# ucsdmanorlab/bootstrapper

Measured on AMD Instinct MI355X. Metric: Mvoxels/s predict+segment, 1024^3 vol in 128^3 blocks, higher is better.
Workload: dtype bf16x3

## Files before the change

bootstrapper_amd/_lib.py:

```python
import ctypes as C
import os

import torch

_HERE = os.path.dirname(os.path.abspath(__file__))
LIB_PATH = os.environ.get("BSMI_LIB") or os.path.join(_HERE, "libbsmi.so")

MAX_LEVELS, MAX_CONVS, MAX_HEADS, NAME_LEN = 8, 4, 4, 32
PREC_F32, PREC_BF16, PREC_BF16X3 = 0, 1, 2
RAW_U8, RAW_F32, RAW_U8_UNIT = 0, 1, 2
ERR_INVALID, ERR_HIP, ERR_STATE, ERR_MISSING, ERR_OVERFLOW = -1, -2, -3, -4, -5


class UNetConfig(C.Structure):
    _fields_ = [
        ("in_channels", C.c_int32),
        ("num_fmaps", C.c_int32),
        ("fmap_inc_factor", C.c_int32),
        ("num_levels", C.c_int32),
        ("downsample_factors", (C.c_int32 * 3) * MAX_LEVELS),
        ("n_convs_down", C.c_int32 * MAX_LEVELS),
        ("kernel_size_down", ((C.c_int32 * 3) * MAX_CONVS) * MAX_LEVELS),
        ("n_convs_up", C.c_int32 * MAX_LEVELS),
        ("kernel_size_up", ((C.c_int32 * 3) * MAX_CONVS) * MAX_LEVELS),
        ("num_heads", C.c_int32),
        ("head_name", (C.c_char * NAME_LEN) * MAX_HEADS),
        ("head_dims", C.c_int32 * MAX_HEADS),
        ("num_fmaps_out", C.c_int32),
    ]


class StepInfo(C.Structure):
    _fields_ = [("type", C.c_int32), ("materialised", C.c_int32), ("shape", C.c_int32 * 4), ("conv_index", C.c_int32),
                ("form", C.c_int32), ("flags", C.c_int32), ("bn", C.c_int32), ("ksteps", C.c_int32), ("head", C.c_int32),
                ("factor", C.c_int32 * 3), ("offset", C.c_int32 * 3), ("prefix", C.c_char * 64)]


STEP_TYPES = ("input", "conv", "pool", "up", "head")
CONV_FORMS = ("gather", "raster-halo", "box-halo", "halo-resident", "first-pass", "winograd F(2x2)", "winograd F(4x4)")
STEP_FLAGS = {1: "fused-up", 2: "res-low", 4: "split-k"}


class Codec(C.Structure):
    _fields_ = [("id", C.c_int32), ("level", C.c_int32), ("cname", C.c_int32), ("shuffle", C.c_int32),
                ("typesize", C.c_int32), ("blocksize", C.c_int32)]


class ChunkCopy(C.Structure):
    _fields_ = [("path", C.c_char_p), ("base", C.c_void_p), ("start", C.c_int64 * 4), ("extent", C.c_int64 * 4),
                ("stride", C.c_int64 * 4), ("read_modify_write", C.c_int32), ("reserved", C.c_int32)]


CODEC_RAW, CODEC_ZLIB, CODEC_GZIP, CODEC_ZSTD, CODEC_LZ4, CODEC_BLOSC = range(6)
BLOSC_LZ4, BLOSC_ZLIB, BLOSC_ZSTD = 1, 3, 4
CHUNK_MISSING = 1
MORPH_DILATE, MORPH_ERODE = 0, 1
RESCALE_DOWN, RESCALE_UP = 0, 1


class BsmiError(RuntimeError):
    def __init__(self, code, msg):
        super().__init__(f"libbsmi error {code}: {msg}")
        self.code = code
        self.msg = msg


def _load():
    if not os.path.exists(LIB_PATH):
        raise ImportError(
            f"{LIB_PATH} not found: build it with `python -c 'import __graft_entry__ as g; g.build()'` "
            "(or `make -C bootstrapper_amd/csrc`).  There is no CPU fallback.")
    lib = C.CDLL(LIB_PATH)
    p, i32, i64p, vp = C.c_void_p, C.c_int, C.POINTER(C.c_int64), C.c_void_p
    sigs = {
        "bsmi_last_error": (C.c_char_p, []),
        "bsmi_version": (i32, []),
        "bsmi_unet_create": (i32, [C.POINTER(UNetConfig), i32, C.POINTER(p)]),
        "bsmi_unet_destroy": (i32, [p]),
        "bsmi_unet_load_weight": (i32, [p, C.c_char_p, vp, i64p, i32]),
        "bsmi_unet_finalize": (i32, [p, i32]),
        "bsmi_unet_output_shape": (i32, [p, i64p, i64p]),
        "bsmi_unet_flops": (i32, [p, i64p, C.POINTER(C.c_double)]),
        "bsmi_unet_forward": (i32, [p, i32, vp, i32, i64p, C.POINTER(vp), C.POINTER(vp), vp]),
        "bsmi_unet_debug_activation": (i32, [p, i32, i32, i64p, vp, C.c_uint64]),
        "bsmi_unet_debug_step_info": (i32, [p, i32, C.POINTER(StepInfo), C.POINTER(i32)]),
        "bsmi_unet_profile_enable": (i32, [p, i32]),
        "bsmi_unet_profile_read": (i32, [p, i32, C.POINTER(i32), C.POINTER(C.c_int32), C.POINTER(C.c_double),
                                         C.POINTER(C.c_double)]),
        "bsmi_unet_profile_totals": (i32, [p, C.POINTER(C.c_double), C.POINTER(C.c_double), i64p, i32]),
        "bsmi_extract_block_reflect_u8": (i32, [vp, i64p, i64p, i64p, vp, vp]),
        "bsmi_seg_create": (i32, [i32, i64p, C.POINTER(p)]),
        "bsmi_seg_destroy": (i32, [p]),
        "bsmi_ws_fragments_u8": (i32, [p, vp, i64p, i32, i32, vp, vp, vp]),
        "bsmi_ws_fragments_seeds_u8": (i32, [p, vp, i64p, i32, i32, vp, vp, vp, vp]),
        "bsmi_rag_agglomerate_u8": (i32, [p, vp, vp, i64p, C.c_float, C.c_int, vp]),
        "bsmi_rag_edge_stats": (i32, [p, vp, vp, C.c_uint64, vp]),
        "bsmi_agglomerate_mean_u8": (i32, [p, vp, vp, i64p, C.POINTER(C.c_float), i32, vp, vp]),
        "bsmi_agglomerate_hist_u8": (i32, [p, vp, vp, i64p, C.POINTER(C.c_float), i32, i32, i32, vp, vp]),
        "bsmi_agglomerate_hist_graph": (i32, [C.c_uint32, C.c_uint32, vp, vp, vp, i32, i32, C.POINTER(C.c_float), i32, vp]),
        "bsmi_frag_postprocess_u8": (i32, [p, vp, vp, i64p, C.c_double, C.c_int64, i64p, i64p, C.c_uint64, vp, vp, vp]),
        "bsmi_label_stats": (i32, [p, vp, i64p, C.c_uint64, C.c_uint64, vp, vp, vp]),
        "bsmi_rag_merge_scores_u8": (i32, [p, vp, vp, i64p, C.c_float, C.c_int, vp, vp, C.c_uint64, vp, vp, vp, vp]),
        "bsmi_lut_relabel": (i32, [C.c_int, vp, C.c_uint64, vp, vp, C.c_uint64, vp, vp]),
        "bsmi_lut_relabel_multi": (i32, [i32, vp, C.c_uint64, vp, vp, C.c_uint64, i32, vp, vp]),
        "bsmi_connected_components": (i32, [vp, C.c_uint64, vp, vp, C.c_uint64, C.c_float, vp]),
        "bsmi_connected_components_multi": (i32, [vp, C.c_uint64, vp, vp, C.c_uint64, vp, C.c_int, vp]),
        "bsmi_cc_affs_u8": (i32, [p, vp, i64p, C.c_int, C.c_int64, vp, vp, vp, vp]),
        "bsmi_mws_agglom_f64": (i32, [C.c_int, vp, C.c_int, vp, vp, C.c_uint32, i64p, vp, vp]),
        "bsmi_mws_cluster": (i32, [C.c_uint64, vp, vp, C.c_uint64, vp]),
        "bsmi_frag_pair_affinity_u8": (i32, [C.c_int, vp, C.c_int, vp, vp, i64p, C.c_uint64, vp, vp, vp, vp, vp]),
        "bsmi_label_table_u64": (i32, [p, vp, i64p, C.c_int64, vp, vp, vp, vp, C.c_uint64, vp, vp]),
        "bsmi_seg_status": (i32, [p, vp]),
        "bsmi_seg_set_host_flood": (i32, [p, i32]),
        "bsmi_rag_graph_u8": (i32, [p, vp, vp, i64p, vp, vp, vp, C.c_uint64, vp, vp]),
        "bsmi_rag_merge_scores_host": (i32, [i32, vp, vp, vp, vp, C.c_float, i32, vp, i32]),
        "bsmi_rag_merge_scores_host_rule": (i32, [i32, vp, vp, vp, vp, C.c_float, i32, i32, vp, i32]),
        "bsmi_unet_train_set_arithmetic": (i32, [p, i32]),
        "bsmi_unet_train_set_deterministic": (i32, [p, i32]),
        "bsmi_unet_train_begin": (i32, [p, i64p]),
        "bsmi_unet_train_forward_backward": (i32, [p, vp, C.POINTER(C.c_void_p), C.POINTER(C.c_void_p), C.POINTER(C.c_float), vp]),
        "bsmi_unet_train_num_params": (i32, [p, C.POINTER(C.c_uint64)]),
        "bsmi_unet_train_buffers": (i32, [p, C.POINTER(C.c_void_p), C.POINTER(C.c_void_p)]),
        "bsmi_unet_train_param_info": (i32, [p, C.c_char_p, C.POINTER(C.c_uint64), C.POINTER(C.c_uint64)]),
        "bsmi_unet_train_adam_step": (i32, [p, C.c_float, C.c_float, C.c_float, C.c_float, C.c_float, vp]),
        "bsmi_unet_train_read_param": (i32, [p, C.c_char_p, C.c_int, vp]),
        "bsmi_unet_train_last_loss": (i32, [p, C.POINTER(C.c_float), vp]),
        "bsmi_unet_train_prediction": (i32, [p, i32, C.POINTER(C.c_void_p), C.POINTER(C.c_uint64)]),
        "bsmi_unet_train_grad_groups": (i32, [p, i32, C.POINTER(i32), C.POINTER(C.c_uint64), C.POINTER(C.c_uint64)]),
        "bsmi_unet_train_wait_grad_group": (i32, [p, i32, vp]),
        "bsmi_unet_train_write_param": (i32, [p, C.c_char_p, C.c_int, vp]),
        "bsmi_unet_train_step_count": (i32, [p, C.c_int, C.POINTER(C.c_int)]),
        "bsmi_unet_train_end": (i32, [p]),
        "bsmi_train_affinity_targets": (i32, [C.c_int, vp, vp, i64p, C.POINTER(C.c_int32), C.c_int, C.c_int, C.c_int, C.c_float,
                                              C.c_float, vp, vp, vp]),
        "bsmi_train_lsd_targets": (i32, [C.c_int, vp, vp, i64p, i64p, i64p, C.POINTER(C.c_float), C.POINTER(C.c_float), C.c_int, vp, vp, vp]),
        "bsmi_train_lsd2d_targets": (i32, [C.c_int, vp, vp, C.c_int, i64p, i64p, i64p, C.POINTER(C.c_float), C.POINTER(C.c_float), C.c_int,
                                           vp, vp, vp]),
        "bsmi_train_affinity_targets_roi": (i32, [C.c_int, vp, vp, C.c_int, i64p, i64p, i64p, C.POINTER(C.c_int32), C.c_int, C.c_int,
                                                  C.c_int, C.c_float, C.c_float, vp, vp, vp]),
        "bsmi_train_mask_sat": (i32, [C.c_int, vp, C.c_int, C.c_int, C.c_int, vp, vp]),
        "bsmi_unet_set_persistent_grid": (i32, [p, C.c_int]),
        "bsmi_unet_profile_executed": (i32, [p, C.POINTER(C.c_double), C.c_int]),
        "bsmi_debug_lds_canary": (i32, [i32, i32, i32, vp, vp]),
        "bsmi_debug_check_guards": (i32, []),
        "bsmi_stream_create_cu_mask": (i32, [C.c_int, vp, C.c_int, C.POINTER(C.c_void_p)]),
        "bsmi_stream_destroy": (i32, [C.c_int, vp]),
        "bsmi_eval_create": (i32, [i32, C.c_uint64, C.POINTER(p)]),
        "bsmi_eval_destroy": (i32, [p]),
        "bsmi_eval_aff_errors_u8": (i32, [p, vp, i64p, i64p, vp, i32, i64p, vp, C.POINTER(C.c_int32), i64p, C.c_float, C.c_float,
                                          C.c_int64, vp, vp, vp, vp]),
        "bsmi_eval_lsd_errors_u8": (i32, [p, vp, i64p, i64p, vp, vp, i64p, i64p, i64p, i64p, C.POINTER(C.c_float), C.POINTER(C.c_float),
                                          i32, C.c_float, C.c_float, C.c_int64, C.c_uint64, vp, vp, vp, vp, vp, vp, vp, vp]),
        "bsmi_eval_pairs_u64": (i32, [p, vp, vp, vp, i64p, i32, vp]),
        "bsmi_eval_pairs_read": (i32, [p, vp, vp, vp, C.c_uint64, vp, vp]),
        "bsmi_eval_status": (i32, [p, vp]),
        "bsmi_label_morph_u64": (i32, [i32, vp, i64p, i32, i32, i32, vp, vp, vp]),
        "bsmi_label_fill_holes_scratch_bytes": (C.c_size_t, [i64p, C.c_uint64]),
        "bsmi_label_fill_holes_u64": (i32, [i32, vp, i64p, i32, vp, vp, C.c_size_t, C.c_uint64, C.POINTER(C.c_uint64), vp]),
        "bsmi_mask_closing_work_bytes": (C.c_size_t, [i64p, i32]),
        "bsmi_mask_closing_disk_u8": (i32, [i32, vp, i64p, i32, vp, vp, C.c_size_t, vp]),
        "bsmi_downscale_mean": (i32, [i32, vp, i32, i64p, C.POINTER(C.c_int32), C.POINTER(C.c_int32), vp, i64p, vp]),
        "bsmi_rescale_sample": (i32, [i32, vp, i32, i64p, C.POINTER(C.c_int32), C.POINTER(C.c_int32), i32, vp, i64p, vp]),
        "bsmi_nonzero_bbox": (i32, [i32, vp, i32, i64p, i64p, vp, vp]),
        "bsmi_synth_create": (i32, [i32, i64p, C.POINTER(p)]),
        "bsmi_synth_destroy": (i32, [p]),
        "bsmi_synth_dilate_points": (i32, [p, i64p, vp, i32, vp, vp, vp, vp, vp]),
        "bsmi_synth_label_i32": (i32, [p, vp, i64p, vp, C.POINTER(C.c_uint64), vp]),
        "bsmi_synth_expand_i32": (i32, [p, vp, i64p, i32, C.c_int32, vp, vp]),
        "bsmi_synth_tubes_i32": (i32, [p, vp, i64p, vp, C.POINTER(C.c_uint64), vp]),
        "bsmi_synth_gaussian_f32": (i32, [p, vp, i64p, vp, i32, vp, vp]),
        "bsmi_synth_argmax_filter_f32": (i32, [p, vp, i64p, i32, vp, vp]),
        "bsmi_synth_basins_f32": (i32, [p, vp, vp, vp, i64p, vp, C.POINTER(C.c_uint64), vp]),
        "bsmi_synth_finish_i32": (i32, [p, vp, i64p, i32, i32, i32, vp, vp]),
        "bsmi_synth_grow_boundary_i64": (i32, [i32, vp, i64p, C.c_uint64, i32, vp, vp]),
        "bsmi_synth_merge_i64": (i32, [i32, vp, i64p, C.POINTER(C.c_int32), i32, C.c_int64, C.c_int64, vp]),
        "bsmi_synth_stamp_i64": (i32, [i32, vp, i64p, i32, i32, i32, vp, i32, i32, C.c_int64, vp]),
        "bsmi_synth_present_i64": (i32, [p, vp, C.c_uint64, vp, C.c_uint32, C.POINTER(C.c_uint32), vp]),
        "bsmi_synth_split_i64": (i32, [p, vp, i64p, C.c_int64, i32, C.POINTER(C.c_int32), i32, C.c_int64, C.POINTER(C.c_uint64), vp]),
        "bsmi_codec_bound": (C.c_size_t, [C.POINTER(Codec), C.c_size_t]),
        "bsmi_codec_decode": (i32, [C.POINTER(Codec), vp, C.c_size_t, vp, C.c_size_t, C.POINTER(C.c_size_t)]),
        "bsmi_codec_encode": (i32, [C.POINTER(Codec), vp, C.c_size_t, vp, C.c_size_t, C.POINTER(C.c_size_t)]),
        "bsmi_chunks_read": (i32, [C.POINTER(Codec), i32, C.POINTER(C.c_char_p), C.POINTER(vp), C.POINTER(C.c_size_t),
                                   C.POINTER(C.c_size_t), C.POINTER(i32), i32]),
        "bsmi_chunks_write": (i32, [C.POINTER(Codec), i32, C.POINTER(C.c_char_p), C.POINTER(vp), C.POINTER(C.c_size_t),
                                    C.POINTER(i32), i32]),
        "bsmi_blosc_dev_frame_bound": (C.c_size_t, [C.c_size_t]),
        "bsmi_blosc_dev_scratch_bytes": (C.c_size_t, [i32, C.c_size_t]),
        "bsmi_blosc_encode_dev_u64": (i32, [i32, vp, C.c_int64, C.c_int64, i32, i64p, i64p, i64p, vp, C.c_size_t, vp, C.c_size_t, vp, vp]),
        "bsmi_rag_write_sqlite": (i32, [C.c_char_p, C.c_uint64, vp, vp, vp, C.c_uint64, vp, vp]),
        "bsmi_chunks_read_into": (i32, [C.POINTER(Codec), i32, C.POINTER(ChunkCopy), i64p, i32, vp, C.POINTER(i32), i32]),
        "bsmi_chunks_write_from": (i32, [C.POINTER(Codec), i32, C.POINTER(ChunkCopy), i64p, i32, vp, C.POINTER(i32), i32]),
    }
    for name, (res, args) in sigs.items():
        fn = getattr(lib, name)
        fn.restype = res
        fn.argtypes = args
# ... 14 lines not shown
```

bootstrapper_amd/csrc/seg.hip:

```cpp
#include <atomic>
#include <chrono>
#include <thread>

#include "seg_internal.h"

#include "dev_guard.h"

namespace bsmi {

__global__ __launch_bounds__(256) void fill_list_kernel(FillList L) {
  const size_t stride = (size_t)gridDim.x * blockDim.x, t0 = (size_t)blockIdx.x * blockDim.x + threadIdx.x;
  for (int j = 0; j < L.n; ++j) {
    uint32_t* p = L.p[j];
    const size_t w = L.words[j];
    const uint32_t v = L.value[j];
    size_t head = (size_t)((0 - (uintptr_t)p) >> 2) & 3;
    head = head < w ? head : w;
    if (t0 < head) p[t0] = v;
    uint4* q = (uint4*)(p + head);
    const size_t nv = (w - head) >> 2;
    for (size_t i = t0; i < nv; i += stride) q[i] = make_uint4(v, v, v, v);
    const size_t done = head + 4 * nv;
    if (t0 < w - done) p[done + t0] = v;
  }
}
void Fills::launch(hipStream_t s) const {
  const unsigned grid = (unsigned)std::min<size_t>((most + 255) / 256 + 1, 2048);
  hipLaunchKernelGGL(fill_list_kernel, dim3(grid), dim3(256), 0, s, L);
}

template <typename T>
static int dalloc(bsmi_seg* h, T** p, size_t count) {
  void* q = nullptr;
  BSMI_HIP(hipMalloc(&q, count * sizeof(T) + 16));
  h->allocs.push_back(q);
  *p = (T*)q;
  return BSMI_OK;
}
static uint32_t next_pow2(uint64_t v) {
  uint32_t p = 1;
  while (p < v) p <<= 1;
  return p;
}

int check_seg_shape(bsmi_seg* h, const int64_t shape[3]) {
  if (!h || !shape) BSMI_FAIL(BSMI_ERR_INVALID, "null argument");
  for (int d = 0; d < 3; ++d)
    if (shape[d] < 1) BSMI_FAIL(BSMI_ERR_INVALID, "bad shape");
  if ((size_t)shape[0] * shape[1] * shape[2] > h->max_vox || shape[0] > h->max_shape[0] ||
      shape[1] * shape[2] > h->max_shape[1] * h->max_shape[2])
    BSMI_FAIL(BSMI_ERR_INVALID, "shape (%lld,%lld,%lld) exceeds the handle's max_shape (%lld,%lld,%lld)",
              (long long)shape[0], (long long)shape[1], (long long)shape[2], (long long)h->max_shape[0],
              (long long)h->max_shape[1], (long long)h->max_shape[2]);
  return BSMI_OK;
}

}

using namespace bsmi;

extern "C" {

int bsmi_seg_create(int device, const int64_t max_shape[3], bsmi_seg** out) {
  if (!max_shape || !out) BSMI_FAIL(BSMI_ERR_INVALID, "null argument");
  for (int d = 0; d < 3; ++d)
    if (max_shape[d] < 1 || max_shape[d] > 4096) BSMI_FAIL(BSMI_ERR_INVALID, "bad max_shape");
  BSMI_HIP(hipSetDevice(device));
  bsmi_seg* h = new bsmi_seg;
  h->device = device;
  for (int d = 0; d < 3; ++d) h->max_shape[d] = max_shape[d];
  const size_t nv = (size_t)max_shape[0] * max_shape[1] * max_shape[2];
  const size_t ns = (size_t)max_shape[1] * max_shape[2];
  h->max_vox = nv;
  int rc = 0;
#define A(ptr, cnt) if (!rc) rc = dalloc(h, &(ptr), (cnt))
  A(h->ws.mask, nv); A(h->ws.g, nv); A(h->ws.d2, nv); A(h->ws.mf, nv); A(h->ws.par, nv); A(h->ws.lab, nv);
  A(h->ws.nseeds, (size_t)max_shape[0]); A(h->ws.offs, (size_t)max_shape[0]);
  h->ws.seedlab = nullptr;
  h->flood_spill_stride = ns;
  A(h->flood_spill, nv);
  if (ns >= ((size_t)1 << 20)) A(h->flood_spill_idx, nv);
  AggWs& g = h->agg;
  static std::atomic<int> next_xcd{0};
  g.xcd_hint = next_xcd.fetch_add(1) & 7;
  g.id_cap = (uint32_t)std::min<size_t>(nv + 2, (size_t)1 << 27);
  g.node_cap = (uint32_t)std::min<size_t>(nv / 8 + 1024, (size_t)1 << 24);
  g.hcap = next_pow2(std::max<size_t>(nv / 2, 1024));
  g.edge_cap = g.hcap / 2;
  A(g.rank_of_id, (size_t)g.id_cap); A(g.ids, (size_t)g.node_cap); A(g.counters, 8);
  A(g.hkeys, (size_t)g.hcap); A(g.hvals, (size_t)g.hcap); A(g.hsum, (size_t)g.hcap); A(g.hcnt, (size_t)g.hcap);
  A(g.eu, (size_t)g.edge_cap); A(g.ev, (size_t)g.edge_cap); A(g.ekey0, (size_t)g.edge_cap);
  A(g.esum, (size_t)g.edge_cap); A(g.ecnt, (size_t)g.edge_cap); A(g.enextu, (size_t)g.edge_cap);
  A(g.enextv, (size_t)g.edge_cap); A(g.eflags, (size_t)g.edge_cap);
  A(g.head, (size_t)g.node_cap); A(g.parent, (size_t)g.node_cap);
  A(g.roots, (size_t)g.node_cap * kMaxThresholds); A(g.heap_spill, (size_t)g.edge_cap); A(g.maxid, 1);
  A(g.sticky, 1);
  A(g.escore, (size_t)g.edge_cap); A(g.etime, (size_t)g.edge_cap); A(g.ntime, (size_t)g.node_cap);
  A(h->thr_dev, kMaxThresholds); A(h->status_dev, 4);
  FragWs& f = h->frag;
  f.id_cap = (uint32_t)std::min<size_t>(nv + 2, (size_t)1 << 27);
  A(f.lsum, (size_t)f.id_cap); A(f.lcnt, (size_t)f.id_cap); A(f.rank, nv); A(f.blk, nv / 1024 + 2); A(f.flags, 4);
  f.par = h->ws.par;
  A(h->crop_tmp, nv);
  g.icap = next_pow2((size_t)g.node_cap * 2);
  A(g.idkeys, (size_t)g.icap); A(g.idvals, (size_t)g.icap); A(g.idu, (size_t)g.node_cap);
  A(g.skeys, (size_t)g.hcap); A(g.sslot, (size_t)g.hcap); A(g.iota, (size_t)g.hcap); A(g.qnext, (size_t)g.edge_cap);
  A(g.tnext, (size_t)g.node_cap * 2); A(g.tscore, (size_t)g.node_cap * 2); A(g.cur, (size_t)g.node_cap);
  A(g.ha, (size_t)g.node_cap); A(g.hb, (size_t)g.node_cap); A(h->rag_counts, 4);
  A(g.tcount, (size_t)g.icap); A(g.tzmin, (size_t)g.icap); A(g.tzmax, (size_t)g.icap);
  if (!rc) {
    size_t b = 0;
// ... 136 lines not shown
```

bootstrapper_amd/csrc/seg_graph.hip:

```cpp
#include <new>

#include "seg_internal.h"

#include "dev_guard.h"

namespace bsmi {
void host_agglomerate_hist(uint32_t nn, uint32_t ne, const uint32_t* eu, const uint32_t* ev, uint32_t* hist, int quantile,
                           int init_with_max, const float* thresholds, int nthr, uint32_t* roots_out);

constexpr int AGG_LDS_HEAP = 12288;

__global__ void agg_maxid_kernel(const uint64_t* __restrict__ frags, size_t n, AggWs w) {
  unsigned long long m = 0;
  for (size_t i = (size_t)blockIdx.x * blockDim.x + threadIdx.x; i < n; i += (size_t)gridDim.x * blockDim.x)
    m = frags[i] > m ? frags[i] : m;
  for (int o = 32; o > 0; o >>= 1) {
    const unsigned long long t = __shfl_down(m, o);
    m = t > m ? t : m;
  }
  if ((threadIdx.x & 63) == 0 && m) atomicMax((unsigned long long*)w.maxid, m);
}

__global__ void agg_mark_kernel(const uint64_t* __restrict__ frags, size_t n, AggWs w) {
  const uint64_t maxid = *w.maxid;
  if (maxid >= w.id_cap) {
    if (blockIdx.x == 0 && threadIdx.x == 0) atomicOr(&w.counters[3], 1u);
    return;
  }
  for (size_t i = (size_t)blockIdx.x * blockDim.x + threadIdx.x; i < n; i += (size_t)gridDim.x * blockDim.x) {
    const uint64_t f = frags[i];
    if (f) w.rank_of_id[f] = 1u;
  }
}

__global__ __launch_bounds__(1024) void agg_rank_kernel(AggWs w) {
  __shared__ uint32_t sh[1024];
  if (w.counters[3]) return;
  const uint64_t maxid = *w.maxid;
  const uint32_t n = (uint32_t)maxid + 1;
  const uint32_t chunk = (n + 1023) / 1024;
  const uint32_t c0 = threadIdx.x * chunk, c1 = min(n, c0 + chunk);
  uint32_t cnt = 0;
  for (uint32_t i = c0; i < c1 && i < n; ++i) cnt += w.rank_of_id[i] == 1u;
  sh[threadIdx.x] = cnt;
  __syncthreads();
  if (threadIdx.x == 0) {
    uint32_t acc = 0;
    for (int t = 0; t < 1024; ++t) { const uint32_t c = sh[t]; sh[t] = acc; acc += c; }
    w.counters[0] = acc;
    if (acc > w.node_cap) atomicOr(&w.counters[3], 2u);
  }
  __syncthreads();
  if (w.counters[3]) return;
  uint32_t r = sh[threadIdx.x];
  for (uint32_t i = c0; i < c1 && i < n; ++i) {
    if (w.rank_of_id[i] == 1u) {
      w.rank_of_id[i] = r;
      w.ids[r] = i;
      w.head[r] = NOEDGE;
      w.parent[r] = r;
      ++r;
    } else {
      w.rank_of_id[i] = 0xffffffffu;
    }
  }
}

template <bool HASH>
__device__ __forceinline__ uint32_t agg_rank(const AggWs& w, uint64_t f) {
  if constexpr (!HASH) return w.rank_of_id[f];
  uint32_t s = (uint32_t)mix64(f) & (w.icap - 1);
  for (uint32_t probe = 0; probe < w.icap; ++probe) {
    const uint64_t k = w.idkeys[s];
    if (k == f) return w.idvals[s];
    if (k == HEMPTY) break;
    s = (s + 1) & (w.icap - 1);
  }
  return 0;
}

template <bool HASH>
__global__ void agg_edges_kernel(const uint8_t* __restrict__ affs, const uint64_t* __restrict__ frags, int D, int H,
                                 int W, AggWs w) {
  if (w.counters[3]) return;
  const size_t n = (size_t)D * H * W;
  const size_t hw = (size_t)H * W;
  for (size_t p = (size_t)blockIdx.x * blockDim.x + threadIdx.x; p < n; p += (size_t)gridDim.x * blockDim.x) {
    const uint64_t f1 = frags[p];
    if (!f1) continue;
    const int x = (int)(p % W);
    const int y = (int)((p / W) % H);
    const int z = (int)(p / hw);
    const uint32_t r1 = agg_rank<HASH>(w, f1);
    const bool ok[3] = {z > 0, y > 0, x > 0};
    const size_t st[3] = {hw, (size_t)W, 1};
#pragma unroll
    for (int d = 0; d < 3; ++d) {
      if (!ok[d]) continue;
      const uint64_t f2 = frags[p - st[d]];
      if (!f2 || f2 == f1) continue;
      const uint32_t r2 = agg_rank<HASH>(w, f2);
      const uint32_t u = r1 < r2 ? r1 : r2, v = r1 < r2 ? r2 : r1;
      const uint64_t key = ((uint64_t)u << 32) | v;
      uint32_t slot = (uint32_t)mix64(key) & (w.hcap - 1);
      bool placed = false;
      for (uint32_t probe = 0; probe < w.hcap; ++probe) {
        const unsigned long long old = atomicCAS((unsigned long long*)&w.hkeys[slot], HEMPTY, key);
        if (old == HEMPTY || old == key) { placed = true; break; }
        slot = (slot + 1) & (w.hcap - 1);
      }
      if (!placed) { atomicOr(&w.counters[3], 4u); return; }
      atomicAdd(&w.hsum[slot], (unsigned long long)affs[(size_t)d * n + p]);
      atomicAdd(&w.hcnt[slot], 1u);
    }
  }
}

__global__ void agg_compact_kernel(AggWs w) {
  if (w.counters[3]) return;
  for (uint32_t s = blockIdx.x * blockDim.x + threadIdx.x; s < w.hcap; s += gridDim.x * blockDim.x) {
    const uint64_t key = w.hkeys[s];
    if (key == HEMPTY) continue;
    const uint32_t e = atomicAdd(&w.counters[1], 1u);
    if (e >= w.edge_cap) { atomicOr(&w.counters[3], 8u); continue; }
    const uint32_t u = (uint32_t)(key >> 32), v = (uint32_t)key;
    w.eu[e] = u; w.ev[e] = v; w.ekey0[e] = key;
    w.esum[e] = w.hsum[s]; w.ecnt[e] = w.hcnt[s];
    w.eflags[e] = 0;
    w.hvals[s] = e;
    w.enextu[e] = atomicExch(&w.head[u], e);
    w.enextv[e] = atomicExch(&w.head[v], e);
  }
}

__global__ void agg_hist_kernel(const uint8_t* __restrict__ affs, const uint64_t* __restrict__ frags, int D, int H, int W, AggWs w,
                                uint32_t* __restrict__ hist) {
  if (w.counters[3]) return;
  const size_t n = (size_t)D * H * W;
  const size_t hw = (size_t)H * W;
  for (size_t p = (size_t)blockIdx.x * blockDim.x + threadIdx.x; p < n; p += (size_t)gridDim.x * blockDim.x) {
    const uint64_t f1 = frags[p];
    if (!f1) continue;
    const int x = (int)(p % W);
    const int y = (int)((p / W) % H);
    const int z = (int)(p / hw);
    const uint32_t r1 = w.rank_of_id[f1];
    const bool ok[3] = {z > 0, y > 0, x > 0};
    const size_t st[3] = {hw, (size_t)W, 1};
#pragma unroll
    for (int d = 0; d < 3; ++d) {
      if (!ok[d]) continue;
      const uint64_t f2 = frags[p - st[d]];
      if (!f2 || f2 == f1) continue;
      const uint32_t r2 = w.rank_of_id[f2];
      const uint32_t u = r1 < r2 ? r1 : r2, v = r1 < r2 ? r2 : r1;
      const uint64_t key = ((uint64_t)u << 32) | v;
      uint32_t slot = (uint32_t)mix64(key) & (w.hcap - 1);
      while (w.hkeys[slot] != key) slot = (slot + 1) & (w.hcap - 1);
      atomicAdd(&hist[(size_t)w.hvals[slot] * 256 + affs[(size_t)d * n + p]], 1u);
    }
  }
}

constexpr uint32_t kRankMax = AGG_LDS_HEAP;
__global__ __launch_bounds__(1024) void agg_edge_rank_kernel(AggWs w) {
  extern __shared__ uint64_t rank_keys[];
  if (w.counters[3]) return;
  const uint32_t ne = w.counters[1];
  if (ne > kRankMax || ne > w.edge_cap) return;
  for (uint32_t e = threadIdx.x; e < ne; e += blockDim.x) rank_keys[e] = w.ekey0[e];
  __syncthreads();
  for (uint32_t e = threadIdx.x; e < ne; e += blockDim.x) {
    const uint64_t k = rank_keys[e];
    uint32_t r = 0;
    for (uint32_t j = 0; j < ne; ++j) r += rank_keys[j] < k ? 1u : 0u;
    w.qnext[e] = r;
  }
  if (threadIdx.x == 0) w.counters[7] = 1;
}

__device__ __forceinline__ float agg_score(unsigned long long sum, uint32_t cnt) {
  return 1.0f - (float)((double)sum / (255.0 * (double)cnt));
}

__device__ __forceinline__ bool xcd_claim(uint32_t* claim, int target) {
  __shared__ int sh_run;
  if (threadIdx.x == 0) {
    unsigned xcc;
    asm volatile("s_getreg_b32 %0, hwreg(HW_REG_XCC_ID)" : "=s"(xcc));
    bool run = false;
    if ((int)(xcc & 7) == target) run = atomicCAS(&claim[0], 0u, 1u) == 0u;
    const unsigned arrived = atomicAdd(&claim[1], 1u);
    if (!run && arrived == gridDim.x - 1) run = atomicCAS(&claim[0], 0u, 1u) == 0u;
    sh_run = run ? 1 : 0;
  }
  __syncthreads();
  return sh_run != 0;
}
// ... 152 lines not shown
            bool move_f = true;
            if (gs >= 0) {
              const uint32_t g = w.hvals[gs];
              const unsigned long long sum_f = w.esum[f], sum_g = w.esum[g];
              const uint32_t cnt_f = w.ecnt[f], cnt_g = w.ecnt[g];
              const float st_f = w.escore[f], st_g = w.escore[g];
              const uint8_t gfl = fget(g);
              if (st_f > st_g) {
                w.esum[g] = sum_g + sum_f;
                w.ecnt[g] = cnt_g + cnt_f;
                fset(g, gfl | 2);
                fset(f, ffl | 1);
                move_f = false;
              } else {
                w.esum[f] = sum_f + sum_g;
                w.ecnt[f] = cnt_f + cnt_g;
                fset(g, gfl | 1);
                w.hvals[gs] = f;
              }
            }
            if (move_f) {
              const uint32_t ha = w.head[a];
              if (b_in_u) { w.eu[f] = a; w.enextu[f] = ha; } else { w.ev[f] = a; w.enextv[f] = ha; }
              w.head[a] = f;
              fset(f, ffl | 2);
              if (gs < 0) hput(gkey, f);
            }
          }
          f = nxt;
        }
        if (fail) break;
        {
          const int64_t es = hfind(norm_key(eu, evv));
          if (es >= 0) w.hkeys[es] = HTOMB;
        }
        fset(e, fget(e) | 1);
        w.parent[b] = a;
      }
      sh_dummy = items;
      if (fail) atomicOr(&w.counters[3], 16u);
    }
    __syncthreads();
    for (uint32_t i = lane; i < nn; i += 64) {
      uint32_t r = i;
      for (;;) {
        const uint32_t p = __hip_atomic_load(&w.parent[r], __ATOMIC_RELAXED, __HIP_MEMORY_SCOPE_WORKGROUP);
        if (p == r) break;
        r = p;
      }
      w.roots[(size_t)t * w.node_cap + i] = r;
    }
    __syncthreads();
  }
}

__global__ __launch_bounds__(64) void agg_merge_kernel(AggWs w, const AggThresholds thr_arg, int nthr) {
  __shared__ uint64_t hl[AGG_LDS_HEAP];
  __shared__ uint8_t fl_lds[AGG_LDS_HEAP];
  __shared__ int sh_dummy;
  static_assert(AGG_LDS_HEAP <= 65536, "FAST entries hold 16-bit ranks and edges");
  if (!xcd_claim(&w.counters[5], w.xcd_hint)) return;
  if (w.counters[3]) return;
  const uint32_t nn = w.counters[0];
  const uint32_t ne = min(w.counters[1], w.edge_cap);
  if (ne <= (uint32_t)AGG_LDS_HEAP && w.counters[7] != 0) agg_merge_body<true>(w, thr_arg, nthr, hl, fl_lds, &sh_dummy, nn, ne);
  else agg_merge_body<false>(w, thr_arg, nthr, hl, fl_lds, &sh_dummy, nn, ne);
}

__global__ void agg_relabel_kernel(const uint64_t* __restrict__ frags, size_t n, int nthr, AggWs w,
                                   uint64_t* __restrict__ segs) {
  keep_overflow(w);
  if (w.counters[3]) return;
  for (size_t p = (size_t)blockIdx.x * blockDim.x + threadIdx.x; p < n; p += (size_t)gridDim.x * blockDim.x) {
    const uint64_t f = frags[p];
    if (!f) {
      for (int t = 0; t < nthr; ++t) segs[(size_t)t * n + p] = 0;
      continue;
    }
    const uint32_t r = w.rank_of_id[f];
    for (int t = 0; t < nthr; ++t) segs[(size_t)t * n + p] = w.ids[w.roots[(size_t)t * w.node_cap + r]];
  }
}

__global__ void rag_ids_kernel(const uint64_t* __restrict__ frags, size_t n, int W, AggWs w) {
  for (size_t p = (size_t)blockIdx.x * blockDim.x + threadIdx.x; p < n; p += (size_t)gridDim.x * blockDim.x) {
    const uint64_t f = frags[p];
    if (!f) continue;
    if (p % W != 0 && frags[p - 1] == f) continue;
    if (f >= HTOMB) { atomicOr(&w.counters[3], 1u); continue; }
    uint32_t s = (uint32_t)mix64(f) & (w.icap - 1);
    bool done = false;
    for (uint32_t probe = 0; probe < w.icap; ++probe) {
      const unsigned long long old = atomicCAS((unsigned long long*)&w.idkeys[s], HEMPTY, f);
      if (old == HEMPTY) {
        const uint32_t i = atomicAdd(&w.counters[0], 1u);
        if (i < w.node_cap) {
          w.idu[i] = f;
          w.idvals[s] = i;
        } else {
          atomicOr(&w.counters[3], 2u);
        }
        done = true;
        break;
      }
      if (old == f) { done = true; break; }
      s = (s + 1) & (w.icap - 1);
    }
    if (!done) atomicOr(&w.counters[3], 2u);
  }
}

__global__ void rag_pad_kernel(AggWs w) {
  const uint32_t nn = min(w.counters[0], w.node_cap);
  for (uint32_t i = blockIdx.x * blockDim.x + threadIdx.x; i < w.node_cap; i += gridDim.x * blockDim.x)
    if (i >= nn) w.idu[i] = HEMPTY;
}

__global__ void rag_rank_kernel(AggWs w) {
  if (w.counters[3]) return;
  const uint32_t nn = w.counters[0];
  for (uint32_t r = blockIdx.x * blockDim.x + threadIdx.x; r < nn; r += gridDim.x * blockDim.x) {
    const uint64_t f = w.ids[r];
    uint32_t s = (uint32_t)mix64(f) & (w.icap - 1);
    while (w.idkeys[s] != f) s = (s + 1) & (w.icap - 1);
    w.idvals[s] = r;
    w.head[r] = NOEDGE;
    w.parent[r] = r;
    w.cur[r] = r;
    w.tnext[r] = NOEDGE;
    w.ntime[r] = 0;
  }
}

__global__ void rag_iota_kernel(AggWs w) {
  for (uint32_t i = blockIdx.x * blockDim.x + threadIdx.x; i < w.hcap; i += gridDim.x * blockDim.x) w.iota[i] = i;
}

__global__ void rag_compact_kernel(AggWs w) {
  if (w.counters[3]) return;
  for (uint32_t i = blockIdx.x * blockDim.x + threadIdx.x; i < w.hcap; i += gridDim.x * blockDim.x) {
    const uint64_t key = w.skeys[i];
    if (key == HEMPTY) continue;
    if (i >= w.edge_cap) { atomicOr(&w.counters[3], 8u); continue; }
    const uint32_t e = i, slot = w.sslot[i];
    const uint32_t u = (uint32_t)(key >> 32), v = (uint32_t)key;
    w.eu[e] = u; w.ev[e] = v; w.ekey0[e] = key;
    w.esum[e] = w.hsum[slot]; w.ecnt[e] = w.hcnt[slot];
    w.eflags[e] = 0;
    w.hvals[slot] = e;
    w.enextu[e] = atomicExch(&w.head[u], e);
    w.enextv[e] = atomicExch(&w.head[v], e);
    atomicMax(&w.counters[1], i + 1);
  }
}

__device__ __forceinline__ int64_t agg_hfind(const AggWs& w, uint64_t key) {
  uint32_t s = (uint32_t)mix64(key) & (w.hcap - 1);
  for (uint32_t probe = 0; probe < w.hcap; ++probe) {
    const uint64_t k = w.hkeys[s];
    if (k == key) return (int64_t)s;
    if (k == HEMPTY) return -1;
    s = (s + 1) & (w.hcap - 1);
  }
  return -1;
}

__device__ __forceinline__ bool agg_hput(const AggWs& w, uint64_t key, uint32_t val) {
  uint32_t s = (uint32_t)mix64(key) & (w.hcap - 1);
  uint32_t probe = 0;
  for (; probe < w.hcap; ++probe) {
    const uint64_t k = w.hkeys[s];
    if (k == HEMPTY || k == HTOMB || k == key) break;
    s = (s + 1) & (w.hcap - 1);
  }
  if (probe == w.hcap) return false;
  w.hkeys[s] = key;
  w.hvals[s] = val;
  return true;
}

__device__ __forceinline__ uint64_t agg_norm_key(uint32_t x, uint32_t y) {
  return x < y ? (((uint64_t)x << 32) | y) : (((uint64_t)y << 32) | x);
}

constexpr int kRagFastEdges = 6144, kRagFastNodes = 6144;
template <bool FAST>
struct RagMem {
  const AggWs& w;
  uint16_t *eu16, *ev16, *qn16, *et16, *nt16;
  uint8_t* fl8;
  uint32_t *sum32, *cnt32;
  float* sc32;
// ... 230 lines not shown
    if (e == NOEDGE) break;
    uint32_t a, b;
    if (!agg_contract_wave<FAST>(M, e, lst, sh, a, b)) {
      if (lane == 0) atomicOr(&w.counters[3], 16u);
      break;
    }
    if (lane == 0) {
      const float sc = M.score(e);
      M.set_ntime(a, ++clock);
      const uint32_t t = nn + nm;
      w.tnext[w.cur[a]] = t;
      w.tnext[w.cur[b]] = t;
      w.cur[a] = t;
      w.tnext[t] = NOEDGE;
      w.tscore[t] = sc;
      w.ha[nm] = a;
      w.hb[nm] = b;
      ++nm;
    }
  }
  if (lane == 0) w.counters[4] = nm;
}

__global__ __launch_bounds__(64) void rag_merge_kernel(AggWs w, float threshold, int nbins, int allow_fast) {
  __shared__ uint32_t bhead[kMaxQueueBins], btail[kMaxQueueBins];
  __shared__ uint32_t lst[kSweepCap];
  __shared__ int sh[4];
  __shared__ uint16_t l_eu[kRagFastEdges], l_ev[kRagFastEdges], l_qn[kRagFastEdges], l_et[kRagFastEdges], l_nt[kRagFastNodes];
  __shared__ uint8_t l_fl[kRagFastEdges];
  __shared__ uint32_t l_sum[kRagFastEdges], l_cnt[kRagFastEdges];
  __shared__ float l_sc[kRagFastEdges];
  if (!xcd_claim(&w.counters[5], w.xcd_hint)) return;
  if (w.counters[3]) return;
  for (int b = threadIdx.x; b < nbins; b += 64) bhead[b] = btail[b] = NOEDGE;
  __syncthreads();
  const uint32_t nn = w.counters[0];
  const uint32_t ne = min(w.counters[1], w.edge_cap);
  if (allow_fast && ne <= (uint32_t)kRagFastEdges && nn <= (uint32_t)kRagFastNodes) {
    const RagMem<true> M{w, l_eu, l_ev, l_qn, l_et, l_nt, l_fl, l_sum, l_cnt, l_sc};
    rag_merge_body<true>(M, threshold, nbins, nn, ne, bhead, btail, lst, sh);
  } else {
    const RagMem<false> M{w, nullptr, nullptr, nullptr, nullptr, nullptr, nullptr, nullptr, nullptr, nullptr};
    rag_merge_body<false>(M, threshold, nbins, nn, ne, bhead, btail, lst, sh);
  }
}

__global__ void rag_scores_kernel(AggWs w, uint64_t* __restrict__ edges, float* __restrict__ scores, uint64_t cap,
                                  uint64_t* __restrict__ merges, float* __restrict__ mscores, uint64_t* __restrict__ counts) {
  keep_overflow(w);
  if (w.counters[3]) return;
  const uint32_t nn = w.counters[0];
  const uint32_t ne = min(w.counters[1], w.edge_cap);
  const uint32_t nm = w.counters[4];
  if (ne > cap) {
    if (blockIdx.x == 0 && threadIdx.x == 0) {
      atomicOr(&w.counters[3], 32u);
      atomicOr(w.sticky, 32u);
      counts[0] = ne; counts[1] = nm; counts[2] = nn;
    }
    return;
  }
  if (blockIdx.x == 0 && threadIdx.x == 0) { counts[0] = ne; counts[1] = nm; counts[2] = nn; }
  for (uint32_t e = blockIdx.x * blockDim.x + threadIdx.x; e < ne; e += gridDim.x * blockDim.x) {
    const uint64_t key = w.ekey0[e];
    uint32_t x = (uint32_t)(key >> 32), y = (uint32_t)key;
    edges[2 * (size_t)e] = w.ids[x];
    edges[2 * (size_t)e + 1] = w.ids[y];
    float sc = __uint_as_float(0x7fc00000u);
    for (;;) {
      if (x == y) { sc = w.tscore[x]; break; }
      if (x < y) { const uint32_t nx = w.tnext[x]; if (nx == NOEDGE) break; x = nx; }
      else { const uint32_t ny = w.tnext[y]; if (ny == NOEDGE) break; y = ny; }
    }
    scores[e] = sc;
  }
  if (merges)
    for (uint32_t i = blockIdx.x * blockDim.x + threadIdx.x; i < nm; i += gridDim.x * blockDim.x) {
      merges[2 * (size_t)i] = w.ids[w.ha[i]];
      merges[2 * (size_t)i + 1] = w.ids[w.hb[i]];
      if (mscores) mscores[i] = w.tscore[nn + i];
    }
}

__global__ void rag_graph_hash_out_kernel(AggWs w, uint64_t* __restrict__ edges, uint64_t* __restrict__ sums, uint32_t* __restrict__ cnts,
                                          uint64_t cap, uint64_t* __restrict__ counts) {
  keep_overflow(w);
  if (w.counters[3]) return;
  if (blockIdx.x == 0 && threadIdx.x == 0) counts[2] = w.counters[0];
  for (uint32_t sl = blockIdx.x * blockDim.x + threadIdx.x; sl < w.hcap; sl += gridDim.x * blockDim.x) {
    const uint64_t key = w.hkeys[sl];
    if (key == HEMPTY) continue;
    const unsigned long long e = atomicAdd((unsigned long long*)&counts[0], 1ull);
    if (e >= cap) {
      atomicOr(w.sticky, 32u);
      continue;
    }
    const uint64_t a = w.idu[(uint32_t)(key >> 32)], b = w.idu[(uint32_t)key];
    edges[2 * (size_t)e] = a < b ? a : b;
    edges[2 * (size_t)e + 1] = a < b ? b : a;
    sums[e] = w.hsum[sl];
    cnts[e] = w.hcnt[sl];
  }
}

__global__ void rag_relabel_kernel(uint64_t* __restrict__ frags, size_t n, AggWs w) {
  keep_overflow(w);
  if (w.counters[3]) return;
  for (size_t p = (size_t)blockIdx.x * blockDim.x + threadIdx.x; p < n; p += (size_t)gridDim.x * blockDim.x) {
    const uint64_t f = frags[p];
    if (!f) continue;
    uint32_t r = agg_rank<true>(w, f);
    for (;;) {
      const uint32_t q = w.parent[r];
      if (q == r) break;
      r = q;
    }
    frags[p] = w.ids[r];
  }
}

__global__ void rag_edge_stats_kernel(AggWs w, uint64_t* __restrict__ sums, uint64_t* __restrict__ counts, uint64_t cap) {
  if (w.counters[3]) return;
  const uint32_t ne = min(w.counters[1], w.edge_cap);
  for (uint32_t e = blockIdx.x * blockDim.x + threadIdx.x; e < ne && e < cap; e += gridDim.x * blockDim.x) {
    const uint32_t slot = w.sslot[e];
    sums[e] = w.hsum[slot];
    counts[e] = w.hcnt[slot];
  }
}

__global__ void seg_clear_kernel(AggWs w) {
  const size_t stride = (size_t)gridDim.x * blockDim.x, t0 = (size_t)blockIdx.x * blockDim.x + threadIdx.x;
  for (size_t i = t0; i < w.id_cap; i += stride) w.rank_of_id[i] = 0;
  for (size_t i = t0; i < w.hcap; i += stride) {
    w.hkeys[i] = HEMPTY;
    w.hsum[i] = 0;
    w.hcnt[i] = 0;
  }
}

int seg_scan_grid() {
  static const int g = [] { const char* e = getenv("BSMI_SEG_SCAN_GRID"); const int v = e ? atoi(e) : 32; return v < 1 ? 1 : v; }();
  return g;
}

}

using namespace bsmi;

extern "C" {

static bool agg_fast_enabled() {
  static const bool fast = [] { const char* e = getenv("BSMI_AGG_FAST"); return !(e && e[0] == '0'); }();
  return fast;
}

int bsmi_agglomerate_mean_u8(bsmi_seg* h, const uint8_t* affs_dev, const uint64_t* frags_dev, const int64_t shape[3],
                             const float* thresholds_host, int n_thresholds, uint64_t* segs_dev, void* stream) {
  int rc = check_seg_shape(h, shape);
  if (rc) return rc;
  if (!affs_dev || !frags_dev || !thresholds_host || !segs_dev) BSMI_FAIL(BSMI_ERR_INVALID, "null argument");
  if (n_thresholds < 1 || n_thresholds > kMaxThresholds) BSMI_FAIL(BSMI_ERR_INVALID, "1..%d thresholds supported", kMaxThresholds);
  for (int i = 0; i < n_thresholds; ++i) {
    if (!(thresholds_host[i] >= 0.f)) BSMI_FAIL(BSMI_ERR_INVALID, "thresholds must be >= 0");
    if (i && thresholds_host[i] < thresholds_host[i - 1]) BSMI_FAIL(BSMI_ERR_INVALID, "thresholds must be ascending");
  }
  BSMI_HIP(hipSetDevice(h->device));
  hipStream_t s = (hipStream_t)stream;
  const int D = (int)shape[0], H = (int)shape[1], W = (int)shape[2];
  const size_t n = (size_t)D * H * W;
  AggWs& g = h->agg;
  AggThresholds thr;
  static_assert(kMaxThresholds <= 16, "AggThresholds holds 16 values");
  for (int i = 0; i < 16; ++i) thr.v[i] = i < n_thresholds ? thresholds_host[i] : 0.f;
  BSMI_HIP(hipMemsetAsync(g.counters, 0, 8 * sizeof(uint32_t), s));
  BSMI_HIP(hipMemsetAsync(g.maxid, 0, sizeof(uint64_t), s));
  const int bs = 1024;
  const int grid = (int)std::min<size_t>((n + bs - 1) / bs, (size_t)seg_scan_grid());
  hipLaunchKernelGGL(seg_clear_kernel, dim3(grid), dim3(bs), 0, s, g);
  hipLaunchKernelGGL(agg_maxid_kernel, dim3(grid), dim3(bs), 0, s, frags_dev, n, g);
  hipLaunchKernelGGL(agg_mark_kernel, dim3(grid), dim3(bs), 0, s, frags_dev, n, g);
  hipLaunchKernelGGL(agg_rank_kernel, dim3(1), dim3(1024), 0, s, g);
  hipLaunchKernelGGL(agg_edges_kernel<false>, dim3(grid), dim3(bs), 0, s, affs_dev, frags_dev, D, H, W, g);
  hipLaunchKernelGGL(agg_compact_kernel, dim3(grid), dim3(bs), 0, s, g);
  {
    static DeviceOnce once;
    const bool attr_set = once.run([&]() -> int {
      BSMI_HIP(hipFuncSetAttribute((const void*)agg_edge_rank_kernel, hipFuncAttributeMaxDynamicSharedMemorySize, (int)(kRankMax * sizeof(uint64_t))));
      return BSMI_OK;
    }) == BSMI_OK;
    if (attr_set && agg_fast_enabled()) hipLaunchKernelGGL(agg_edge_rank_kernel, dim3(1), dim3(1024), kRankMax * sizeof(uint64_t), s, g);
  }
  hipLaunchKernelGGL(agg_merge_kernel, dim3(8), dim3(64), 0, s, g, thr, n_thresholds);
  hipLaunchKernelGGL(agg_relabel_kernel, dim3(grid), dim3(bs), 0, s, frags_dev, n, n_thresholds, g, segs_dev);
  BSMI_HIP(hipGetLastError());
  return BSMI_OK;
}

int bsmi_agglomerate_hist_u8(bsmi_seg* h, const uint8_t* affs_dev, const uint64_t* frags_dev, const int64_t shape[3],
                             const float* thresholds_host, int n_thresholds, int quantile, int init_with_max, uint64_t* segs_dev,
                             void* stream) {
  int rc = check_seg_shape(h, shape);
  if (rc) return rc;
  if (!affs_dev || !frags_dev || !thresholds_host || !segs_dev) BSMI_FAIL(BSMI_ERR_INVALID, "null argument");
  if (n_thresholds < 1 || n_thresholds > kMaxThresholds) BSMI_FAIL(BSMI_ERR_INVALID, "1..%d thresholds supported", kMaxThresholds);
  if (quantile < 0 || quantile > 100) BSMI_FAIL(BSMI_ERR_INVALID, "quantile %d outside 0..100", quantile);
  for (int i = 0; i < n_thresholds; ++i) {
    if (!(thresholds_host[i] >= 0.f)) BSMI_FAIL(BSMI_ERR_INVALID, "thresholds must be >= 0");
    if (i && thresholds_host[i] < thresholds_host[i - 1]) BSMI_FAIL(BSMI_ERR_INVALID, "thresholds must be ascending");
  }
  BSMI_HIP(hipSetDevice(h->device));
  hipStream_t s = (hipStream_t)stream;
  const int D = (int)shape[0], H = (int)shape[1], W = (int)shape[2];
  const size_t n = (size_t)D * H * W;
  AggWs& g = h->agg;
  BSMI_HIP(hipMemsetAsync(g.counters, 0, 8 * sizeof(uint32_t), s));
  BSMI_HIP(hipMemsetAsync(g.maxid, 0, sizeof(uint64_t), s));
  const int bs = 1024;
  const int grid = (int)std::min<size_t>((n + bs - 1) / bs, (size_t)seg_scan_grid());
  hipLaunchKernelGGL(seg_clear_kernel, dim3(grid), dim3(bs), 0, s, g);
  hipLaunchKernelGGL(agg_maxid_kernel, dim3(grid), dim3(bs), 0, s, frags_dev, n, g);
// ... 153 lines not shown
```

bootstrapper_amd/csrc/seg_internal.h:

```cpp
#pragma once
#include <vector>

#include "common.h"
#include "u64_table.h"

namespace bsmi {

constexpr uint64_t HEMPTY = 0xffffffffffffffffull;
constexpr uint64_t HTOMB = 0xfffffffffffffffeull;
constexpr uint32_t NOEDGE = 0xffffffffu;
constexpr int kMaxThresholds = 16;

__device__ __forceinline__ int reflect_dup(int i, int n) {
  const int p = 2 * n;
  i %= p;
  if (i < 0) i += p;
  return i < n ? i : p - 1 - i;
}
__device__ __forceinline__ int reflect_near(int i, int n) { return i < 0 ? -i - 1 : (i >= n ? 2 * n - 1 - i : i); }

struct WsScratch {
  uint8_t* mask;
  int32_t* g;
  int32_t* d2;
// ... 20 lines not shown
  uint32_t* eu; uint32_t* ev; uint64_t* ekey0; unsigned long long* esum; uint32_t* ecnt;
  uint32_t* enextu; uint32_t* enextv; uint8_t* eflags;
  uint32_t edge_cap;
  uint32_t* head;
  uint32_t* parent;
  uint32_t* roots;
  uint64_t* heap_spill;
  uint64_t* maxid;
  uint64_t* idkeys;
  uint32_t* idvals;
  uint32_t icap;
  uint64_t* idu;
  uint64_t* skeys;
  uint32_t* sslot;
  uint32_t* iota;
  uint32_t* qnext;
  uint32_t* tnext;
  float* tscore;
  uint32_t* cur;
  uint32_t* ha; uint32_t* hb;
  float* escore;
  uint32_t* etime;
  uint32_t* ntime;
  int xcd_hint;
  unsigned long long* tcount;
  int* tzmin; int* tzmax;
};

__device__ __forceinline__ void keep_overflow(const AggWs& w) {
  if (blockIdx.x == 0 && threadIdx.x == 0) {
    const uint32_t f = w.counters[3];
    if (f) atomicOr(w.sticky, f);
  }
}

struct FragWs {
  unsigned long long* lsum;
  uint32_t* lcnt;
  uint32_t id_cap;
  int32_t* par;
  int32_t* rank;
  uint32_t* blk;
  uint32_t* flags;
};

__device__ __forceinline__ int cc_find(int32_t* par, int a) {
  int p = __hip_atomic_load(&par[a], __ATOMIC_RELAXED, __HIP_MEMORY_SCOPE_AGENT);
  while (p != a) {
    a = p;
    p = __hip_atomic_load(&par[a], __ATOMIC_RELAXED, __HIP_MEMORY_SCOPE_AGENT);
  }
  return a;
}
__device__ __forceinline__ void cc_unite(int32_t* par, int a, int b) {
  for (;;) {
    a = cc_find(par, a);
    b = cc_find(par, b);
    if (a == b) break;
    const int hi = a < b ? b : a, lo = a < b ? a : b;
    const int old = atomicMin(&par[hi], lo);
    if (old == hi) break;
    a = old;
    b = lo;
  }
}

constexpr int kMaxFills = 6;
struct FillList {
  uint32_t* p[kMaxFills];
  size_t words[kMaxFills];
  uint32_t value[kMaxFills];
  int n;
};
struct Fills {
  FillList L{};
  size_t most = 0;
  void add(void* p, size_t bytes, uint32_t value = 0) {
    L.p[L.n] = (uint32_t*)p; L.words[L.n] = bytes / 4; L.value[L.n] = value; ++L.n;
    most = std::max(most, bytes / 16);
  }
  void launch(hipStream_t s) const;
};

}

struct bsmi_seg {
  int device = 0;
  int64_t max_shape[3] = {0, 0, 0};
  size_t max_vox = 0;
  std::vector<void*> allocs;
  bsmi::WsScratch ws{};
  uint64_t* flood_spill = nullptr;
  size_t flood_spill_stride = 0;
  uint32_t* flood_spill_idx = nullptr;
  bsmi::AggWs agg{};
  bsmi::FragWs frag{};
  uint64_t* crop_tmp = nullptr;
  void* sort_tmp = nullptr;
  size_t sort_tmp_bytes = 0;
  int32_t* seedlab = nullptr;
  uint64_t* rag_counts = nullptr;
  float* thr_dev = nullptr;
  int* status_dev = nullptr;
  bool host_flood3 = false;
};

namespace bsmi {

int check_seg_shape(bsmi_seg* h, const int64_t shape[3]);

int fragments_3d(bsmi_seg* h, const uint8_t* affs_dev, int D, int H, int W, int min_seed_distance, uint64_t* frags_dev,
                 uint64_t* max_id_dev, uint64_t* seeds_dev, hipStream_t s);

void cc_rank_roots(size_t n, const FragWs& f, uint64_t* num_out, hipStream_t s);

hipError_t seg_sort_tmp_bytes(int n_keys, int n_pairs, size_t* bytes);
hipError_t seg_sort_keys_u64(void* tmp, size_t tmp_bytes, const uint64_t* keys_in, uint64_t* keys_out, int n, hipStream_t s);
hipError_t seg_sort_pairs_u64_u32(void* tmp, size_t tmp_bytes, const uint64_t* keys_in, uint64_t* keys_out, const uint32_t* vals_in,
                                  uint32_t* vals_out, int n, hipStream_t s);

}
```

bootstrapper_amd/csrc/seg_labels.hip:

```cpp
#include "seg_internal.h"

#include "dev_guard.h"

namespace bsmi {

__global__ void lut_relabel_kernel(const uint64_t* __restrict__ in, size_t n, const uint64_t* __restrict__ keys,
                                   const uint64_t* __restrict__ vals, uint64_t m, uint64_t* __restrict__ out) {
  for (size_t p = (size_t)blockIdx.x * blockDim.x + threadIdx.x; p < n; p += (size_t)gridDim.x * blockDim.x) {
    const uint64_t f = in[p];
    uint64_t r = f;
    if (f && m) {
      uint64_t lo = 0, hi = m;
      while (lo < hi) {
        const uint64_t mid = (lo + hi) >> 1;
        if (keys[mid] < f) lo = mid + 1; else hi = mid;
      }
      if (lo < m && keys[lo] == f) r = vals[lo];
    }
    out[p] = r;
  }
}

constexpr int kLutMaxColumns = 8;
struct LutColumns {
  const uint64_t* vals[kLutMaxColumns];
  uint64_t* out[kLutMaxColumns];
};
__global__ void lut_relabel_multi_kernel(const uint64_t* __restrict__ in, size_t n, const uint64_t* __restrict__ keys, uint64_t m, int T,
                                         LutColumns c) {
  constexpr int RUN = 8;
  const size_t nruns = (n + RUN - 1) / RUN;
  for (size_t r0 = (size_t)blockIdx.x * blockDim.x + threadIdx.x; r0 < nruns; r0 += (size_t)gridDim.x * blockDim.x) {
    uint64_t last = 0, idx = m;
    const size_t p0 = r0 * RUN, p1 = p0 + RUN < n ? p0 + RUN : n;
    for (size_t p = p0; p < p1; ++p) {
      const uint64_t f = in[p];
      if (f != last) {
        last = f;
        idx = m;
        if (f && m) {
          uint64_t lo = 0, hi = m;
          while (lo < hi) {
            const uint64_t mid = (lo + hi) >> 1;
            if (keys[mid] < f) lo = mid + 1; else hi = mid;
          }
          if (lo < m && keys[lo] == f) idx = lo;
        }
      }
      for (int t = 0; t < T; ++t) c.out[t][p] = idx < m ? c.vals[t][idx] : f;
    }
  }
}

__global__ void frag_stats_kernel(const uint8_t* __restrict__ affs, const uint64_t* __restrict__ frags, size_t n, FragWs w) {
  for (size_t p = (size_t)blockIdx.x * blockDim.x + threadIdx.x; p < n; p += (size_t)gridDim.x * blockDim.x) {
    const uint64_t f = frags[p];
    if (!f) continue;
    if (f >= w.id_cap) { atomicOr(w.flags, 1u); continue; }
    atomicAdd(&w.lsum[f], (unsigned long long)((uint32_t)affs[p] + affs[n + p] + affs[2 * n + p]));
    atomicAdd(&w.lcnt[f], 1u);
  }
}

__global__ void frag_decide_kernel(const uint8_t* __restrict__ affs, const uint64_t* __restrict__ frags, size_t n, FragWs w,
                                   double filter_value, long long min_size) {
  for (uint32_t f = blockIdx.x * blockDim.x + threadIdx.x; f < w.id_cap; f += gridDim.x * blockDim.x) {
    const uint32_t c = w.lcnt[f];
    if (!c || !f) continue;
    bool drop = false;
    if (filter_value > 0.0) {
      double mean = (double)w.lsum[f] / (765.0 * (double)c);
      if (fabs(mean - filter_value) <= 1e-9) {
        double sum = 0.0;
        for (size_t p = 0; p < n; ++p)
          if (frags[p] == f)
            sum += (((double)affs[p] / 255.0 + (double)affs[n + p] / 255.0) + (double)affs[2 * n + p] / 255.0) / 3.0;
        mean = sum / (double)c;
      }
      drop = mean < filter_value;
    }
    if (min_size > 0) drop = drop || (long long)c < min_size;
    if (drop) w.lcnt[f] = c | 0x80000000u;
  }
}

__global__ void frag_filter_kernel(uint64_t* __restrict__ frags, size_t n, FragWs w) {
  for (size_t p = (size_t)blockIdx.x * blockDim.x + threadIdx.x; p < n; p += (size_t)gridDim.x * blockDim.x) {
    const uint64_t f = frags[p];
    if (!f || f >= w.id_cap) continue;
    if (w.lcnt[f] & 0x80000000u) frags[p] = 0;
  }
}

__global__ void crop_u64_kernel(const uint64_t* __restrict__ in, int H, int W, int oz, int oy, int ox, int cd, int ch,
                                int cw, uint64_t* __restrict__ out) {
  const size_t n = (size_t)cd * ch * cw;
  for (size_t i = (size_t)blockIdx.x * blockDim.x + threadIdx.x; i < n; i += (size_t)gridDim.x * blockDim.x) {
    const int x = (int)(i % cw);
    const int y = (int)((i / cw) % ch);
    const int z = (int)(i / ((size_t)cw * ch));
    out[i] = in[((size_t)(z + oz) * H + (y + oy)) * W + (x + ox)];
  }
}

__global__ void cc26_init_kernel(const uint64_t* __restrict__ x, size_t n, FragWs w) {
  for (size_t p = (size_t)blockIdx.x * blockDim.x + threadIdx.x; p < n; p += (size_t)gridDim.x * blockDim.x)
    w.par[p] = x[p] ? (int32_t)p : -1;
}

__global__ void cc26_union_kernel(const uint64_t* __restrict__ x, int D, int H, int W, FragWs w) {
  const size_t n = (size_t)D * H * W;
  for (size_t p = (size_t)blockIdx.x * blockDim.x + threadIdx.x; p < n; p += (size_t)gridDim.x * blockDim.x) {
    const uint64_t v = x[p];
    if (!v) continue;
    const int xx = (int)(p % W);
    const int y = (int)((p / W) % H);
    const int z = (int)(p / ((size_t)W * H));
    for (int dz = -1; dz <= 0; ++dz)
      for (int dy = -1; dy <= 1; ++dy)
        for (int dx = -1; dx <= 1; ++dx) {
          if (dz == 0 && (dy > 0 || (dy == 0 && dx >= 0))) continue;
          const int zz = z + dz, yy = y + dy, x2 = xx + dx;
          if (zz < 0 || yy < 0 || yy >= H || x2 < 0 || x2 >= W) continue;
          const size_t q = ((size_t)zz * H + yy) * W + x2;
          if (x[q] != v) continue;
          cc_unite(w.par, (int)p, (int)q);
        }
  }
}

__global__ __launch_bounds__(1024) void cc26_count_kernel(size_t n, FragWs w) {
  __shared__ uint32_t cnt;
  if (threadIdx.x == 0) cnt = 0;
  __syncthreads();
  const size_t p = (size_t)blockIdx.x * 1024 + threadIdx.x;
  if (p < n && w.par[p] == (int32_t)p) atomicAdd(&cnt, 1u);
  __syncthreads();
  if (threadIdx.x == 0) w.blk[blockIdx.x] = cnt;
}

__global__ __launch_bounds__(1024) void cc26_scan_kernel(uint32_t nblk, FragWs w, uint64_t* num_out) {
  __shared__ uint32_t sh[1024];
  const uint32_t chunk = (nblk + 1023) / 1024;
  const uint32_t c0 = threadIdx.x * chunk, c1 = min(nblk, c0 + chunk);
  uint32_t s = 0;
  for (uint32_t i = c0; i < c1; ++i) s += w.blk[i];
  sh[threadIdx.x] = s;
  __syncthreads();
  if (threadIdx.x == 0) {
    uint32_t acc = 0;
    for (int t = 0; t < 1024; ++t) { const uint32_t c = sh[t]; sh[t] = acc; acc += c; }
    *num_out = acc;
  }
  __syncthreads();
  uint32_t acc = sh[threadIdx.x];
  for (uint32_t i = c0; i < c1; ++i) { const uint32_t c = w.blk[i]; w.blk[i] = acc; acc += c; }
}

__global__ __launch_bounds__(1024) void cc26_rank_kernel(size_t n, FragWs w) {
  __shared__ uint32_t sh[1024];
  const size_t p = (size_t)blockIdx.x * 1024 + threadIdx.x;
  const uint32_t flag = (p < n && w.par[p] == (int32_t)p) ? 1u : 0u;
  sh[threadIdx.x] = flag;
  __syncthreads();
  for (int o = 1; o < 1024; o <<= 1) {
    const uint32_t v = threadIdx.x >= (unsigned)o ? sh[threadIdx.x - o] : 0u;
    __syncthreads();
    sh[threadIdx.x] += v;
    __syncthreads();
  }
  if (flag) w.rank[p] = (int32_t)(w.blk[blockIdx.x] + sh[threadIdx.x]);
}

void cc_rank_roots(size_t n, const FragWs& f, uint64_t* num_out, hipStream_t s) {
  const uint32_t nblk = (uint32_t)((n + 1023) / 1024);
  hipLaunchKernelGGL(cc26_count_kernel, dim3(nblk), dim3(1024), 0, s, n, f);
  hipLaunchKernelGGL(cc26_scan_kernel, dim3(1), dim3(1024), 0, s, nblk, f, num_out);
  hipLaunchKernelGGL(cc26_rank_kernel, dim3(nblk), dim3(1024), 0, s, n, f);
}

__global__ void cc26_write_kernel(const uint64_t* __restrict__ x, size_t n, FragWs w, uint64_t id_offset, uint64_t* __restrict__ out) {
  for (size_t p = (size_t)blockIdx.x * blockDim.x + threadIdx.x; p < n; p += (size_t)gridDim.x * blockDim.x) {
    if (!x[p]) { out[p] = 0; continue; }
    out[p] = id_offset + (uint64_t)w.rank[cc_find(w.par, (int)p)];
  }
}

__global__ void ccaff_init_kernel(size_t n, FragWs w, uint64_t* __restrict__ touched) {
  for (size_t p = (size_t)blockIdx.x * blockDim.x + threadIdx.x; p < n; p += (size_t)gridDim.x * blockDim.x) {
    w.par[p] = (int32_t)p;
    touched[p] = 0;
  }
}

__global__ void ccaff_union_kernel(const uint8_t* __restrict__ affs, int D, int H, int W, int cut, FragWs w, uint64_t* __restrict__ touched) {
  const size_t n = (size_t)D * H * W, hw = (size_t)H * W;
  for (size_t p = (size_t)blockIdx.x * blockDim.x + threadIdx.x; p < n; p += (size_t)gridDim.x * blockDim.x) {
    const int x = (int)(p % W), y = (int)((p / W) % H), z = (int)(p / hw);
    const bool ok[3] = {z + 1 < D, y + 1 < H, x + 1 < W};
    const size_t st[3] = {hw, (size_t)W, 1};
#pragma unroll
    for (int d = 0; d < 3; ++d) {
      if ((int)affs[(size_t)d * n + p] <= cut) continue;
      touched[p] = 1;
      if (!ok[d]) continue;
      const size_t q = p + st[d];
      touched[q] = 1;
      cc_unite(w.par, (int)p, (int)q);
    }
  }
}

__global__ void ccaff_finalize_kernel(size_t n, FragWs w, const uint64_t* __restrict__ touched) {
  for (size_t p = (size_t)blockIdx.x * blockDim.x + threadIdx.x; p < n; p += (size_t)gridDim.x * blockDim.x)
    if (!touched[p]) w.par[p] = -1;
}

__global__ void ltab_clear_kernel(AggWs w) {
  for (size_t i = (size_t)blockIdx.x * blockDim.x + threadIdx.x; i < w.icap; i += (size_t)gridDim.x * blockDim.x) {
    w.idkeys[i] = HEMPTY;
    w.tcount[i] = 0;
    w.tzmin[i] = 0x7fffffff;
    w.tzmax[i] = -0x7fffffff;
  }
}

__global__ void ltab_scan_kernel(const uint64_t* __restrict__ lab, int D, int H, int W, int z0, AggWs w) {
  const size_t nrows = (size_t)D * H;
  for (size_t row = (size_t)blockIdx.x * blockDim.x + threadIdx.x; row < nrows; row += (size_t)gridDim.x * blockDim.x) {
    const int z = (int)(row / H);
    const uint64_t* p = lab + row * W;
    int x = 0;
    while (x < W) {
      const uint64_t f = p[x];
      int len = 1;
      while (x + len < W && p[x + len] == f) ++len;
      x += len;
      if (!f) continue;
      if (f >= HTOMB) { atomicOr(&w.counters[3], 1u); continue; }
      uint32_t s = (uint32_t)mix64(f) & (w.icap - 1);
      bool ok = false;
      for (uint32_t probe = 0; probe < w.icap; ++probe) {
        const unsigned long long old = atomicCAS((unsigned long long*)&w.idkeys[s], HEMPTY, f);
        if (old == HEMPTY) {
          if (atomicAdd(&w.counters[0], 1u) >= w.node_cap) atomicOr(&w.counters[3], 2u);
          ok = true;
          break;
        }
        if (old == f) { ok = true; break; }
        s = (s + 1) & (w.icap - 1);
      }
      if (!ok) { atomicOr(&w.counters[3], 2u); continue; }
      atomicAdd(&w.tcount[s], (unsigned long long)len);
      atomicMin(&w.tzmin[s], z0 + z);
      atomicMax(&w.tzmax[s], z0 + z);
    }
  }
}

__global__ void ltab_compact_kernel(AggWs w) {
  if (w.counters[3]) return;
  for (uint32_t s = blockIdx.x * blockDim.x + threadIdx.x; s < w.icap; s += gridDim.x * blockDim.x) {
    if (w.idkeys[s] == HEMPTY) continue;
    const uint32_t i = atomicAdd(&w.counters[1], 1u);
    if (i < w.node_cap) {
      w.idu[i] = w.idkeys[s];
      w.ha[i] = s;
    }
  }
}

__global__ void ltab_pad_kernel(AggWs w) {
  const uint32_t nn = min(w.counters[0], w.node_cap);
  for (uint32_t i = blockIdx.x * blockDim.x + threadIdx.x; i < w.node_cap; i += gridDim.x * blockDim.x)
    if (i >= nn) { w.idu[i] = HEMPTY; w.ha[i] = 0; }
}

__global__ void ltab_gather_kernel(AggWs w, uint64_t* __restrict__ ids, uint64_t* __restrict__ counts, int32_t* __restrict__ zmin,
                                   int32_t* __restrict__ zmax, uint64_t cap, uint64_t* __restrict__ n_out) {
  keep_overflow(w);
  if (w.counters[3]) return;
  const uint32_t nn = w.counters[0];
  if (nn > cap) {
    if (blockIdx.x == 0 && threadIdx.x == 0) { atomicOr(&w.counters[3], 32u); atomicOr(w.sticky, 32u); }
    return;
  }
  if (blockIdx.x == 0 && threadIdx.x == 0) *n_out = nn;
  for (uint32_t i = blockIdx.x * blockDim.x + threadIdx.x; i < nn; i += gridDim.x * blockDim.x) {
    const uint32_t s = w.hb[i];
    ids[i] = w.ids[i];
    counts[i] = w.tcount[s];
    zmin[i] = w.tzmin[s];
    zmax[i] = w.tzmax[s];
  }
}

__global__ void label_stats_kernel(const uint64_t* __restrict__ lab, int D, int H, int W, uint64_t id_offset, uint64_t num,
                                   unsigned long long* __restrict__ size, unsigned long long* __restrict__ sums) {
  const size_t n = (size_t)D * H * W;
  for (size_t p = (size_t)blockIdx.x * blockDim.x + threadIdx.x; p < n; p += (size_t)gridDim.x * blockDim.x) {
    const uint64_t l = lab[p];
    if (l <= id_offset || l - id_offset > num) continue;
    const uint64_t k = l - id_offset - 1;
    atomicAdd(&size[k], 1ull);
    atomicAdd(&sums[3 * k + 0], (unsigned long long)(p / ((size_t)W * H)));
    atomicAdd(&sums[3 * k + 1], (unsigned long long)((p / W) % H));
    atomicAdd(&sums[3 * k + 2], (unsigned long long)(p % W));
  }
}

}

using namespace bsmi;

extern "C" {

int bsmi_frag_postprocess_u8(bsmi_seg* h, const uint8_t* affs_dev, uint64_t* frags_dev, const int64_t shape[3],
                             double filter_value, int64_t min_size, const int64_t crop_offset[3],
                             const int64_t crop_shape[3], uint64_t id_offset, uint64_t* out_dev, uint64_t* num_labels_dev,
                             void* stream) {
  int rc = check_seg_shape(h, shape);
  if (rc) return rc;
  if (!affs_dev || !frags_dev || !crop_offset || !crop_shape || !out_dev || !num_labels_dev) BSMI_FAIL(BSMI_ERR_INVALID, "null argument");
  for (int d = 0; d < 3; ++d)
    if (crop_offset[d] < 0 || crop_shape[d] < 1 || crop_offset[d] + crop_shape[d] > shape[d])
      BSMI_FAIL(BSMI_ERR_INVALID, "crop outside the fragment volume");
  BSMI_HIP(hipSetDevice(h->device));
  hipStream_t s = (hipStream_t)stream;
  const size_t n = (size_t)shape[0] * shape[1] * shape[2];
  const size_t nc = (size_t)crop_shape[0] * crop_shape[1] * crop_shape[2];
  FragWs& f = h->frag;
  const int bs = 256;
  const int grid = (int)std::min<size_t>((n + bs - 1) / bs, 4096);
  const int gridc = (int)std::min<size_t>((nc + bs - 1) / bs, 4096);
  {
    Fills fl;
    fl.add(f.flags, 4 * sizeof(uint32_t));
    if (filter_value > 0.0 || min_size > 0) {
      fl.add(f.lsum, (size_t)f.id_cap * sizeof(unsigned long long));
      fl.add(f.lcnt, (size_t)f.id_cap * sizeof(uint32_t));
    }
    fl.launch(s);
  }
  if (filter_value > 0.0 || min_size > 0) {
    hipLaunchKernelGGL(frag_stats_kernel, dim3(grid), dim3(bs), 0, s, affs_dev, (const uint64_t*)frags_dev, n, f);
    hipLaunchKernelGGL(frag_decide_kernel, dim3(grid), dim3(bs), 0, s, affs_dev, (const uint64_t*)frags_dev, n, f, filter_value,
                       (long long)min_size);
    hipLaunchKernelGGL(frag_filter_kernel, dim3(grid), dim3(bs), 0, s, frags_dev, n, f);
  }
  hipLaunchKernelGGL(crop_u64_kernel, dim3(gridc), dim3(bs), 0, s, (const uint64_t*)frags_dev, (int)shape[1], (int)shape[2],
                     (int)crop_offset[0], (int)crop_offset[1], (int)crop_offset[2], (int)crop_shape[0], (int)crop_shape[1],
                     (int)crop_shape[2], h->crop_tmp);
  hipLaunchKernelGGL(cc26_init_kernel, dim3(gridc), dim3(bs), 0, s, (const uint64_t*)h->crop_tmp, nc, f);
  hipLaunchKernelGGL(cc26_union_kernel, dim3(gridc), dim3(bs), 0, s, (const uint64_t*)h->crop_tmp, (int)crop_shape[0],
                     (int)crop_shape[1], (int)crop_shape[2], f);
  cc_rank_roots(nc, f, num_labels_dev, s);
  hipLaunchKernelGGL(cc26_write_kernel, dim3(gridc), dim3(bs), 0, s, (const uint64_t*)h->crop_tmp, nc, f, id_offset, out_dev);
  BSMI_HIP(hipGetLastError());
  return BSMI_OK;
}

int bsmi_label_stats(bsmi_seg* h, const uint64_t* labels_dev, const int64_t shape[3], uint64_t id_offset, uint64_t num,
                     uint64_t* size_dev, uint64_t* sums_dev, void* stream) {
  int rc = check_seg_shape(h, shape);
  if (rc) return rc;
  if (!labels_dev || !size_dev || !sums_dev) BSMI_FAIL(BSMI_ERR_INVALID, "null argument");
  BSMI_HIP(hipSetDevice(h->device));
  hipStream_t s = (hipStream_t)stream;
  const size_t n = (size_t)shape[0] * shape[1] * shape[2];
  {
    Fills fl;
    fl.add(size_dev, num * sizeof(uint64_t));
    fl.add(sums_dev, 3 * num * sizeof(uint64_t));
    fl.launch(s);
  }
  const int bs = 256;
  hipLaunchKernelGGL(label_stats_kernel, dim3((int)std::min<size_t>((n + bs - 1) / bs, 4096)), dim3(bs), 0, s, labels_dev,
                     (int)shape[0], (int)shape[1], (int)shape[2], id_offset, num, (unsigned long long*)size_dev,
                     (unsigned long long*)sums_dev);
  BSMI_HIP(hipGetLastError());
  return BSMI_OK;
}

int bsmi_lut_relabel(int device, const uint64_t* in_dev, uint64_t n, const uint64_t* keys_dev, const uint64_t* vals_dev, uint64_t m,
                     uint64_t* out_dev, void* stream) {
  if (!in_dev || !out_dev || (m && (!keys_dev || !vals_dev))) BSMI_FAIL(BSMI_ERR_INVALID, "null argument");
  BSMI_HIP(hipSetDevice(device));
  if (!n) return BSMI_OK;
  const int bs = 256;
  hipLaunchKernelGGL(lut_relabel_kernel, dim3((int)std::min<uint64_t>((n + bs - 1) / bs, 8192)), dim3(bs), 0, (hipStream_t)stream,
                     in_dev, (size_t)n, keys_dev, vals_dev, m, out_dev);
// ... 79 lines not shown
```

bootstrapper_amd/csrc/seg_ws.hip:

```cpp
#include "seg_internal.h"

#include "dev_guard.h"

namespace bsmi {

constexpr int WS_T = 1024;
#ifndef BSMI_FLOOD_WAVES
#define BSMI_FLOOD_WAVES 8
#endif
constexpr int FLOOD_WAVES = BSMI_FLOOD_WAVES;
constexpr int FLOOD_LDS_HEAP = 1024;

template <bool LDS>
__global__ __launch_bounds__(WS_T) void ws_seeds_kernel(const uint8_t* __restrict__ affs, int D, int H, int W,
                                                        int msd, WsScratch s, int compact) {
  extern __shared__ __attribute__((aligned(16))) char ws_smem[];
  const int z = blockIdx.x;
  const int n = H * W;
  const size_t vol = (size_t)D * n;
  const uint8_t* ay = affs + vol + (size_t)z * n;
  const uint8_t* ax = affs + 2 * vol + (size_t)z * n;
  uint8_t* mask = s.mask + (size_t)z * n;
  int32_t* g = s.g + (size_t)z * n;
  int32_t* d2 = s.d2 + (size_t)z * n;
  int32_t* mf = s.mf + (size_t)z * n;
  int32_t* par = s.par + (size_t)z * n;
  int32_t* lab = s.lab + (size_t)z * n;
  const int tid = threadIdx.x;
  __shared__ int sh_any_bg;
  __shared__ int sh_wave[WS_T / 64];
  const bool near = msd <= H && msd <= W;
  if (tid == 0) sh_any_bg = 0;
  __syncthreads();
  uint8_t* smask = nullptr;
  uint8_t* sflag = nullptr;
  const uint16_t* sd2_lds = nullptr;
  if constexpr (!LDS) compact = 0;
  if constexpr (LDS) {
    const size_t o_sd2 = ((size_t)H * (W + 2) * 2 + 15) & ~(size_t)15;
    sd2_lds = (const uint16_t*)(ws_smem + o_sd2);
    const size_t o_mask = (o_sd2 + (size_t)n * 2 + 15) & ~(size_t)15;
    smask = (uint8_t*)(ws_smem + o_mask);
    sflag = smask + (((size_t)n + 15) & ~(size_t)15);
  }
  int bg = 0;
  for (int i = tid; i < n; i += WS_T) {
    const int m = (int)ay[i] + (int)ax[i] >= 256;
    if (!compact) mask[i] = (uint8_t)m;
    if constexpr (LDS) smask[i] = (uint8_t)m;
    bg |= !m;
  }
  if (bg) sh_any_bg = 1;
  __syncthreads();
  const int any_bg = sh_any_bg;
  constexpr int INF = 1 << 28;
  if constexpr (LDS) {
    const int Wp = W + 2;
    uint16_t* sg = (uint16_t*)ws_smem;
    uint16_t* sd2 = (uint16_t*)(ws_smem + (((size_t)H * Wp * 2 + 15) & ~(size_t)15));
    constexpr int GINF = 0xffff;
    if (any_bg) {
      for (int y = tid; y < H; y += WS_T) {
        int last = -INF;
        for (int x = 0; x < W; ++x) {
          if (!smask[y * W + x]) last = x;
          sg[y * Wp + x] = (uint16_t)(last <= -INF ? GINF : x - last);
        }
        last = INF;
        for (int x = W - 1; x >= 0; --x) {
          if (!smask[y * W + x]) last = x;
          const int d = last >= INF ? GINF : last - x;
          if (d < (int)sg[y * Wp + x]) sg[y * Wp + x] = (uint16_t)d;
        }
      }
      __syncthreads();
      for (int i = tid; i < n; i += WS_T) {
        const int y = i / W, x = i - y * W;
        const int g0 = sg[y * Wp + x];
        int best = g0 == GINF ? INF : g0 * g0;
        for (int k = 1; k < H && k * k < best; ++k) {
          if (y - k >= 0) {
            const int gg = sg[(y - k) * Wp + x];
            const int v = gg == GINF ? INF : gg * gg + k * k;
            best = v < best ? v : best;
          }
          if (y + k < H) {
            const int gg = sg[(y + k) * Wp + x];
            const int v = gg == GINF ? INF : gg * gg + k * k;
            best = v < best ? v : best;
          }
        }
        sd2[i] = (uint16_t)best;
        if (!compact) d2[i] = best;
      }
    } else {
      for (int i = tid; i < n; i += WS_T) {
        const int y = i / W, x = i - y * W;
        const int v = (y + 1) * (y + 1) + x * x;
// ... 117 lines not shown
      }
    }
  }
  __syncthreads();
  auto find = [&](int a) {
    int p = par[a];
    while (p != a) {
      a = p;
      p = __hip_atomic_load(&par[a], __ATOMIC_RELAXED, __HIP_MEMORY_SCOPE_WORKGROUP);
    }
    return a;
  };
  auto unite = [&](int a, int b) {
    for (;;) {
      a = find(a);
      b = find(b);
      if (a == b) return;
      if (a < b) { const int t = a; a = b; b = t; }
      const int old = atomicMin(&par[a], b);
      if (old == a) return;
      a = old;
    }
  };
  for (int i = tid; i < n; i += WS_T) {
    if (i < W || par[i] < 0 || par[i - W] < 0) continue;
    const int x = i % W;
    if (x > 0 && par[i - 1] >= 0 && par[i - W - 1] >= 0) continue;
    unite(i, i - W);
  }
  __syncthreads();
  if constexpr (LDS) {
    for (int i = tid; i < n; i += WS_T) sflag[i] = (uint8_t)(par[i] == i);
    __syncthreads();
  }
  const int chunk = (n + WS_T - 1) / WS_T;
  const int c0 = tid * chunk, c1 = min(n, c0 + chunk);
  int cnt = 0;
  for (int i = c0; i < c1; ++i) {
    if constexpr (LDS) cnt += sflag[i];
    else cnt += (par[i] == i);
  }
  const int lane = tid & 63, wave = tid >> 6;
  int incl = cnt;
  for (int o = 1; o < 64; o <<= 1) {
    const int t = __shfl_up(incl, o);
    if (lane >= o) incl += t;
  }
  if (lane == 63) sh_wave[wave] = incl;
  __syncthreads();
  if (wave == 0) {
    int w = lane < WS_T / 64 ? sh_wave[lane] : 0;
    for (int o = 1; o < WS_T / 64; o <<= 1) {
      const int t = __shfl_up(w, o);
      if (lane >= o) w += t;
    }
    if (lane < WS_T / 64) sh_wave[lane] = w;
  }
  __syncthreads();
  int id = (wave ? sh_wave[wave - 1] : 0) + incl - cnt;
  if (tid == WS_T - 1) s.nseeds[z] = id + cnt;
  for (int i = c0; i < c1; ++i) {
    bool root;
    if constexpr (LDS) root = sflag[i] != 0;
    else root = par[i] == i;
    if (root) g[i] = ++id;
  }
  __syncthreads();
  for (int i = tid; i < n; i += WS_T) {
    int l = 0;
    if (par[i] >= 0) {
      const int sl = g[find(i)];
      if (s.seedlab) s.seedlab[(size_t)z * n + i] = sl;
      bool inside;
      if constexpr (LDS) inside = smask[i] != 0;
      else inside = mask[i] != 0;
      if (inside) l = sl;
    } else if (s.seedlab) {
      s.seedlab[(size_t)z * n + i] = 0;
    }
    if (compact) ((uint32_t*)lab)[i] = (uint32_t)l | ((uint32_t)sd2_lds[i] << 16);
    else lab[i] = l;
  }
}

__global__ void ws_offsets_kernel(int D, WsScratch s, uint64_t* max_id) {
  if (threadIdx.x == 0 && blockIdx.x == 0) {
    uint64_t acc = 0;
    for (int z = 0; z < D; ++z) { s.offs[z] = acc; acc += (uint64_t)s.nseeds[z]; }
    *max_id = acc;
  }
}

__device__ __forceinline__ uint64_t bcast0(uint64_t v) {
  const uint32_t lo = __builtin_amdgcn_readfirstlane((uint32_t)v), hi = __builtin_amdgcn_readfirstlane((uint32_t)(v >> 32));
  return ((uint64_t)hi << 32) | lo;
}

__device__ __forceinline__ bool flood_smaller(uint64_t a, uint64_t b) { return (int64_t)((a >> 20) - (b >> 20)) < 0; }

template <bool COMPACT>
__global__ __launch_bounds__(64 * FLOOD_WAVES) void ws_flood_kernel(int D, int H, int W, WsScratch s, uint64_t* heap_spill,
                                                     size_t spill_stride, uint64_t* __restrict__ frags, int* status) {
  __shared__ uint64_t hl_all[FLOOD_WAVES][FLOOD_LDS_HEAP];
  const int lane = threadIdx.x & 63;
  const int wave = __builtin_amdgcn_readfirstlane(threadIdx.x >> 6);
  const int z = blockIdx.x * FLOOD_WAVES + wave;
  if (z >= D) return;
  uint64_t* hl = hl_all[wave];
  const int n = H * W;
  const uint8_t* mask = s.mask + (size_t)z * n;
  const int32_t* d2 = s.d2 + (size_t)z * n;
  int32_t* lab = s.lab + (size_t)z * n;
  uint64_t* hg = heap_spill + (size_t)z * spill_stride;
  {
    constexpr uint64_t MAXD2 = (1u << 24) - 1;
    auto uni = [](int v) { return __builtin_amdgcn_readfirstlane(v); };
    auto entry = [](uint64_t dd, uint32_t age_, uint64_t q_, uint32_t lbl_) -> uint64_t {
      return COMPACT ? ((65535ull - dd) << 48) | ((uint64_t)age_ << 32) | ((uint64_t)lbl_ << 16) | q_
                     : ((MAXD2 - dd) << 40) | ((uint64_t)age_ << 20) | q_;
    };
    auto smaller = [](uint64_t a_, uint64_t b_) -> bool {
      if constexpr (COMPACT) return (uint32_t)(a_ >> 32) < (uint32_t)(b_ >> 32);
      else return flood_smaller(a_, b_);
    };
    int items = 0;
    auto hget = [&](int i) -> uint64_t {
      if (i < FLOOD_LDS_HEAP) return hl[i];
      uint64_t v = 0;
      if (lane == 0) v = hg[i - FLOOD_LDS_HEAP];
      return bcast0(v);
    };
    auto hset = [&](int i, uint64_t v) {
      if (lane == 0) {
        if (i < FLOOD_LDS_HEAP) hl[i] = v; else hg[i - FLOOD_LDS_HEAP] = v;
      }
    };
    auto push = [&](uint64_t it) {
      int c = uni(items++);
      if constexpr (COMPACT) {
        if (c < FLOOD_LDS_HEAP) {
          const uint32_t ik = (uint32_t)(it >> 32), ix = (uint32_t)it;
          while (c > 0) {
            const int p = (c - 1) >> 1;
            const uint64_t pr = hl[p];
            const uint32_t pk = (uint32_t)(pr >> 32), px = (uint32_t)pr;
            if (!(ik < pk)) break;
            hl[c] = ((uint64_t)pk << 32) | px;
            c = p;
          }
          hl[c] = ((uint64_t)ik << 32) | ix;
          return;
        }
      }
      if (c < FLOOD_LDS_HEAP) {
        while (c > 0) {
          const int p = (c - 1) >> 1;
          const uint64_t pv = hl[p];
          if (!smaller(it, pv)) break;
          hl[c] = pv;
          c = p;
        }
        hl[c] = it;
        return;
      }
      while (c > 0) {
        const int p = (c + 1) / 2 - 1;
        const uint64_t pv = hget(p);
        if (smaller(it, pv)) { hset(c, pv); c = uni(p); } else break;
      }
      hset(c, it);
    };
    uint32_t* rec = (uint32_t*)lab;
    for (int i0 = 0; i0 < n; i0 += 64) {
      const int i = i0 + lane;
      const int li = i < n ? (COMPACT ? (int)(rec[i] & 0xffffu) : lab[i]) : 0;
      unsigned long long seeds = __ballot(li != 0);
      while (seeds) {
        const int k = __ffsll(seeds) - 1;
        seeds &= seeds - 1;
        const int j = i0 + k;
        const uint32_t rj = COMPACT ? (uint32_t)uni((int)rec[j]) : 0u;
        const uint64_t dj = COMPACT ? (uint64_t)(rj >> 16) : (uint64_t)(uint32_t)uni(d2[j]);
        push(entry(dj, 0u, (uint64_t)j, rj & 0xffffu));
      }
    }
// ... 19 lines not shown
          dk = (int)(rk >> 16);
          mk = dk != 0;
        } else {
          lme = lab[idx];
          mk = mask[qk];
          lk = lab[qk];
          dk = d2[qk];
        }
      }
      if (items > 0) {
        const uint64_t last = hget(items);
        int i = 0;
        const int lim = items < FLOOD_LDS_HEAP ? items : FLOOD_LDS_HEAP;
        bool placed = false;
        if constexpr (COMPACT) {
          const uint32_t lk = (uint32_t)(last >> 32);
          while (2 * i + 2 < lim) {
            const int c1 = 2 * i + 1;
            const uint64_t r1 = hl[c1], r2 = hl[c1 + 1];
            const uint32_t k1 = (uint32_t)(r1 >> 32), k2 = (uint32_t)(r2 >> 32);
            const uint32_t x1 = (uint32_t)r1, x2 = (uint32_t)r2;
            const bool right = k2 < k1;
            const uint32_t ck = right ? k2 : k1, cx = right ? x2 : x1;
            if (!(ck < lk)) { placed = true; break; }
            hl[i] = ((uint64_t)ck << 32) | cx;
            i = c1 + (right ? 1 : 0);
          }
        }
        while (!COMPACT && 2 * i + 2 < lim) {
          const int c1 = 2 * i + 1;
          const uint64_t r1 = hl[c1], r2 = hl[c1 + 1];
          const uint64_t v1 = r1, v2 = r2;
          const bool right = smaller(v2, v1);
          const uint64_t cv = right ? v2 : v1;
          if (!smaller(cv, last)) { placed = true; break; }
          hl[i] = cv;
          i = c1 + (right ? 1 : 0);
        }
        for (; !placed;) {
          const int c1 = 2 * i + 1, c2 = c1 + 1;
          if (c1 >= items) break;
          uint64_t v1, v2;
          if (c2 < FLOOD_LDS_HEAP) {
            const uint64_t r1 = hl[c1], r2 = hl[c2];
            v1 = r1;
            v2 = r2;
          } else {
            v1 = hget(c1);
            v2 = c2 < items ? hget(c2) : 0;
          }
          int sm = i;
          uint64_t smv = last;
          if (smaller(v1, smv)) { sm = c1; smv = v1; }
          if (c2 < items && smaller(v2, smv)) { sm = c2; smv = v2; }
          if (sm == i) break;
          hset(i, smv);
          i = uni(sm);
        }
        hset(i, last);
      }
      const int l = uni(lme);
      const bool cand = okk && mk && lk == 0;
      for (uint32_t m = (uint32_t)__ballot(cand) & 0xfu; m; m &= m - 1) {
        const int k = __ffs((int)m) - 1;
        const int q = __builtin_amdgcn_readlane(qk, k);
        const uint64_t dd = (uint64_t)(uint32_t)__builtin_amdgcn_readlane(dk, k);
        ++age;
        if constexpr (COMPACT) rec[q] = (uint32_t)l | ((uint32_t)dd << 16);
        else lab[q] = l;
        push(entry(dd, age, (uint64_t)q, (uint32_t)l));
      }
    }
  }
  __builtin_amdgcn_fence(__ATOMIC_RELEASE, "workgroup");
  __builtin_amdgcn_wave_barrier();
  __builtin_amdgcn_fence(__ATOMIC_ACQUIRE, "workgroup");
  const uint64_t off = s.offs[z];
  uint64_t* out = frags + (size_t)z * n;
  for (int i = lane; i < n; i += 64) {
    const int l = COMPACT ? (int)(((const uint32_t*)lab)[i] & 0xffffu) : lab[i];
    out[i] = l ? (uint64_t)l + off : 0ull;
  }
  (void)status;
}

constexpr int FLOOD_WIDE_LDS_LEVELS = 13;
constexpr int FLOOD_WIDE_LDS_HEAP = (1 << FLOOD_WIDE_LDS_LEVELS) - 1;

__device__ __forceinline__ int flood_wide_owner(uint32_t i) {
  const int d = 31 - __builtin_clz(i + 1);
  const int k = (d - FLOOD_WIDE_LDS_LEVELS) % 5 + 1;
  return (1 << k) - 2 + (int)((i + 1) & ((1u << k) - 1));
}

#ifdef BSMI_FLOOD_STATS
__device__ unsigned long long g_flood_stats[16];
extern "C" int bsmi_debug_flood_stats(unsigned long long* out, int reset) {
  if (hipMemcpyFromSymbol(out, HIP_SYMBOL(g_flood_stats), sizeof(unsigned long long) * 16) != hipSuccess) return -1;
  if (reset) {
    unsigned long long zero[16] = {0};
    if (hipMemcpyToSymbol(HIP_SYMBOL(g_flood_stats), zero, sizeof zero) != hipSuccess) return -1;
  }
  return 0;
}
#define FW_STAT(i, v) (st[i] += (v))
#else
#define FW_STAT(i, v) ((void)0)
#endif

__global__ __launch_bounds__(64) void ws_flood_wide_kernel(int D, int H, int W, WsScratch s, uint64_t* spill_key, uint32_t* spill_idx,
                                                           size_t spill_stride, uint64_t* __restrict__ frags) {
  constexpr int LH = FLOOD_WIDE_LDS_HEAP;
  __shared__ uint64_t hk[LH];
  __shared__ uint32_t hx[LH];
  const int lane = threadIdx.x;
  const int z = blockIdx.x;
  if (z >= D) return;
  const int n = H * W;
  const uint8_t* mask = s.mask + (size_t)z * n;
  const int32_t* d2 = s.d2 + (size_t)z * n;
  int32_t* lab = s.lab + (size_t)z * n;
  uint64_t* gk = spill_key + (size_t)z * spill_stride;
  uint32_t* gx = spill_idx + (size_t)z * spill_stride;
  {
    constexpr uint64_t MAXD2 = 0x7fffffffull;
    auto uni = [](int v) { return __builtin_amdgcn_readfirstlane(v); };
    auto rl64 = [](uint64_t v, int l) -> uint64_t {
      const uint32_t lo = __builtin_amdgcn_readlane((int)(uint32_t)v, l), hi = __builtin_amdgcn_readlane((int)(uint32_t)(v >> 32), l);
      return ((uint64_t)hi << 32) | lo;
    };
    auto smaller = [](uint64_t a_, uint64_t b_) -> bool { return (int64_t)(a_ - b_) < 0; };
    int items = 0;
#ifdef BSMI_FLOOD_STATS
    uint64_t st[11] = {};
    bool popping = false;
    uint64_t t0 = 0;
#endif
    struct Ent { uint64_t k; uint32_t x; };
    auto hget = [gk, gx, lane, rl64](int i) -> Ent {
      if (i < LH) return {hk[i], hx[i]};
      const int o = flood_wide_owner((uint32_t)i);
      uint64_t kv = 0;
      uint32_t xv = 0;
      if (lane == o) { kv = gk[i - LH]; xv = gx[i - LH]; }
      return {rl64(kv, o), (uint32_t)__builtin_amdgcn_readlane((int)xv, o)};
    };
    auto hset = [gk, gx, lane](int i, uint64_t k_, uint32_t x_) {
      if (i < LH) { hk[i] = k_; hx[i] = x_; return; }
      if (lane == flood_wide_owner((uint32_t)i)) { gk[i - LH] = k_; gx[i - LH] = x_; }
    };
    auto push = [&](uint64_t ik, uint32_t ix) {
      int c = uni(items++);
#ifdef BSMI_FLOOD_STATS
      if (popping) FW_STAT(4, 1);
      if ((uint64_t)items > st[8]) st[8] = items;
#endif
      while (c > 0) {
        const int p = (c - 1) >> 1;
        const Ent pe = hget(p);
#ifdef BSMI_FLOOD_STATS
        if (popping && p >= LH) FW_STAT(6, 1);
#endif
        if (!smaller(ik, pe.k)) break;
        hset(c, pe.k, pe.x);
#ifdef BSMI_FLOOD_STATS
        if (popping) FW_STAT(5, 1);
// ... 48 lines not shown
          const uint64_t v1 = hk[c1], v2 = hk[c2];
          int sm = i;
          uint64_t smv = lastk;
          if (smaller(v1, smv)) { sm = c1; smv = v1; }
          if (c2 < items && smaller(v2, smv)) { sm = c2; smv = v2; }
          if (sm == i) { placed = true; break; }
          hk[i] = smv;
          hx[i] = hx[sm];
          FW_STAT(1, 1);
          i = sm;
        }
        while (!placed) {
          uint64_t wk = 0;
          uint32_t wx = 0;
          {
            const uint32_t q = ((uint32_t)(i + 1) << wl_k) - 1 + (uint32_t)wl_j;
            if (lane < 62 && q < (uint32_t)items) { wk = gk[q - LH]; wx = gx[q - LH]; }
          }
          FW_STAT(2, 1);
          int wj = 0;
          int kk = 0;
          for (; kk < 5; ++kk) {
            const int c1 = 2 * i + 1, c2 = c1 + 1;
            if (c1 >= items) { placed = true; break; }
            const int l1 = (2 << kk) - 2 + 2 * wj;
            const uint64_t v1 = rl64(wk, l1), v2 = rl64(wk, l1 + 1);
            int sm = i, sl = 0;
            uint64_t smv = lastk;
            if (smaller(v1, smv)) { sm = c1; smv = v1; sl = l1; }
            if (c2 < items && smaller(v2, smv)) { sm = c2; smv = v2; sl = l1 + 1; }
            if (sm == i) { placed = true; break; }
            hset(i, smv, (uint32_t)__builtin_amdgcn_readlane((int)wx, sl));
            FW_STAT(3, 1);
            wj = 2 * wj + (sm == c2 ? 1 : 0);
            i = uni(sm);
          }
        }
        hset(i, lastk, lastx);
      }
      const int l = uni(lme);
      const bool cand = okk && mk && lk == 0;
      for (uint32_t m = (uint32_t)__ballot(cand) & 0xfu; m; m &= m - 1) {
        const int k = __ffs((int)m) - 1;
        const int q = __builtin_amdgcn_readlane(qk, k);
        const uint64_t dd = (uint64_t)(uint32_t)__builtin_amdgcn_readlane(dk, k);
        ++age;
        lab[q] = l;
        push(((MAXD2 - dd) << 32) | age, (uint32_t)q);
      }
    }
#ifdef BSMI_FLOOD_STATS
    st[9] = __builtin_amdgcn_s_memrealtime() - t0;
    st[10] = 1;
    if (lane == 0) {
      for (int k = 0; k < 11; ++k)
        if (k == 8) atomicMax(&g_flood_stats[k], (unsigned long long)st[k]);
        else atomicAdd(&g_flood_stats[k], (unsigned long long)st[k]);
    }
#endif
  }
  __builtin_amdgcn_fence(__ATOMIC_RELEASE, "workgroup");
  __builtin_amdgcn_wave_barrier();
  __builtin_amdgcn_fence(__ATOMIC_ACQUIRE, "workgroup");
  const uint64_t off = s.offs[z];
  uint64_t* out = frags + (size_t)z * n;
  for (int i = lane; i < n; i += 64) {
    const int l = lab[i];
    out[i] = l ? (uint64_t)l + off : 0ull;
  }
}

__global__ void ws_seeds_out_kernel(int D, size_t n, WsScratch s, uint64_t* __restrict__ seeds) {
  const size_t total = (size_t)D * n;
  for (size_t p = (size_t)blockIdx.x * blockDim.x + threadIdx.x; p < total; p += (size_t)gridDim.x * blockDim.x) {
    const int l = s.seedlab[p];
    seeds[p] = l ? (uint64_t)l + s.offs[p / n] : 0ull;
  }
}

}

using namespace bsmi;

static int fragments_xy(bsmi_seg* h, const uint8_t* affs_dev, int D, int H, int W, int min_seed_distance, uint64_t* frags_dev,
                        uint64_t* max_id_dev, uint64_t* seeds_dev, hipStream_t s) {
  if ((size_t)H * W >= ((size_t)1 << 20) && (H > 4096 || W > 4096))
    BSMI_FAIL(BSMI_ERR_INVALID, "slices of 2^20 voxels or more must have H, W <= 4096 (got %d x %d)", H, W);
  WsScratch wsx = h->ws;
  bool compact = false;
  wsx.seedlab = nullptr;
  if (seeds_dev) {
    if (!h->seedlab) {
      void* q = nullptr;
      BSMI_HIP(hipMalloc(&q, h->max_vox * sizeof(int32_t)));
      h->allocs.push_back(q);
      h->seedlab = (int32_t*)q;
    }
    wsx.seedlab = h->seedlab;
  }
  {
    const size_t hw16 = ((size_t)H * W + 15) & ~(size_t)15;
    const size_t lds = (((size_t)H * (W + 2) * 2 + 15) & ~(size_t)15) + (((size_t)H * W * 2 + 15) & ~(size_t)15) + 2 * hw16;
    const bool use_lds = lds <= 158 * 1024 && (size_t)H * H + (size_t)W * W < 65535 && (H + 1) * (H + 1) + W * W < 65535;
    static const bool compact_ok = [] { const char* e = getenv("BSMI_FLOOD_COMPACT"); return !(e && e[0] == '0'); }();
    compact = use_lds && compact_ok;
    if (use_lds) {
      static DeviceOnce once;
      const int rc_once = once.run([&]() -> int {
        BSMI_HIP(hipFuncSetAttribute((const void*)ws_seeds_kernel<true>, hipFuncAttributeMaxDynamicSharedMemorySize, 158 * 1024));
        return BSMI_OK;
      });
      if (rc_once) return rc_once;
      hipLaunchKernelGGL(ws_seeds_kernel<true>, dim3(D), dim3(WS_T), lds, s, affs_dev, D, H, W, min_seed_distance, wsx, compact ? 1 : 0);
    } else {
      hipLaunchKernelGGL(ws_seeds_kernel<false>, dim3(D), dim3(WS_T), 0, s, affs_dev, D, H, W, min_seed_distance, wsx, 0);
    }
  }
  hipLaunchKernelGGL(ws_offsets_kernel, dim3(1), dim3(64), 0, s, D, h->ws, max_id_dev);
  if (seeds_dev)
    hipLaunchKernelGGL(ws_seeds_out_kernel, dim3((unsigned)std::min<size_t>(((size_t)D * H * W + 255) / 256, 4096)), dim3(256), 0, s, D,
                       (size_t)H * W, wsx, seeds_dev);
  if ((size_t)H * W >= ((size_t)1 << 20)) {
    if (!h->flood_spill_idx) BSMI_FAIL(BSMI_ERR_STATE, "wide flood without its spill");
    hipLaunchKernelGGL(ws_flood_wide_kernel, dim3(D), dim3(64), 0, s, D, H, W, h->ws, h->flood_spill, h->flood_spill_idx,
                       h->flood_spill_stride, frags_dev);
  } else if (compact)
    hipLaunchKernelGGL(ws_flood_kernel<true>, dim3((D + FLOOD_WAVES - 1) / FLOOD_WAVES), dim3(64 * FLOOD_WAVES), 0, s, D, H, W, h->ws, h->flood_spill,
                       h->flood_spill_stride, frags_dev, h->status_dev);
  else
    hipLaunchKernelGGL(ws_flood_kernel<false>, dim3((D + FLOOD_WAVES - 1) / FLOOD_WAVES), dim3(64 * FLOOD_WAVES), 0, s, D, H, W, h->ws, h->flood_spill,
                       h->flood_spill_stride, frags_dev, h->status_dev);
  BSMI_HIP(hipGetLastError());
  return BSMI_OK;
}

extern "C" {

int bsmi_ws_fragments_u8(bsmi_seg* h, const uint8_t* affs_dev, const int64_t shape[3], int fragments_in_xy,
                         int min_seed_distance, uint64_t* frags_dev, uint64_t* max_id_dev, void* stream) {
  return bsmi_ws_fragments_seeds_u8(h, affs_dev, shape, fragments_in_xy, min_seed_distance, frags_dev, max_id_dev, nullptr, stream);
}

int bsmi_ws_fragments_seeds_u8(bsmi_seg* h, const uint8_t* affs_dev, const int64_t shape[3], int fragments_in_xy,
                               int min_seed_distance, uint64_t* frags_dev, uint64_t* max_id_dev, uint64_t* seeds_dev, void* stream) {
  int rc = check_seg_shape(h, shape);
  if (rc) return rc;
  if (!affs_dev || !frags_dev || !max_id_dev) BSMI_FAIL(BSMI_ERR_INVALID, "null argument");
  if (min_seed_distance < 1 || min_seed_distance > 64) BSMI_FAIL(BSMI_ERR_INVALID, "min_seed_distance out of range");
  BSMI_HIP(hipSetDevice(h->device));
  hipStream_t s = (hipStream_t)stream;
  const int D = (int)shape[0], H = (int)shape[1], W = (int)shape[2];
  if (!fragments_in_xy) return fragments_3d(h, affs_dev, D, H, W, min_seed_distance, frags_dev, max_id_dev, seeds_dev, s);
  return fragments_xy(h, affs_dev, D, H, W, min_seed_distance, frags_dev, max_id_dev, seeds_dev, s);
}

}
```

bootstrapper_amd/post/engine.py:

```python
import ctypes as C

import torch

from .. import _lib
from .._lib import lib, check


def _affs3(affs_u8, contiguous=False):
    if affs_u8.dtype != torch.uint8 or not affs_u8.is_cuda or affs_u8.dim() != 4 or affs_u8.shape[0] != 3 or (contiguous and not affs_u8.is_contiguous()):
        raise ValueError(f"affs must be a {'contiguous ' if contiguous else ''}uint8 CUDA tensor of shape (3, D, H, W)")


def _frags_like(frags, affs_u8, contiguous=False):
    if frags.dtype != torch.int64 or tuple(frags.shape) != tuple(affs_u8.shape[1:]) or (contiguous and not frags.is_contiguous()):
        raise ValueError(f"fragments must be {'a contiguous' if contiguous else 'an'} int64 tensor of shape (D, H, W)")


class SegEngine:
    def __init__(self, max_shape, device=0, host_flood=True):
        self.device = int(device)
        self.max_shape = tuple(int(s) for s in max_shape)
        self._h = C.c_void_p()
        check(lib.bsmi_seg_create(self.device, _lib.i64x3(self.max_shape), C.byref(self._h)))
        check(lib.bsmi_seg_set_host_flood(self._h, 1 if host_flood else 0))
# ... 94 lines not shown
                                           float(threshold), int(discretize_queue), C.c_void_p(edges.data_ptr()),
                                           C.c_void_p(scores.data_ptr()), cap,
                                           C.c_void_p(merges.data_ptr()) if return_merges else None,
                                           C.c_void_p(mscores.data_ptr()) if return_merges else None,
                                           C.c_void_p(counts.data_ptr()), self._stream()))
        self.status()
        ne, nm = int(counts[0]), int(counts[1])
        if return_merges:
            return edges[:ne], scores[:ne], merges[:nm], mscores[:nm]
        return edges[:ne], scores[:ne]

    def rag_agglomerate(self, affs_u8, frags, threshold, discretize_queue=256):
        _affs3(affs_u8, contiguous=True)
        _frags_like(frags, affs_u8, contiguous=True)
        check(lib.bsmi_rag_agglomerate_u8(self._h, C.c_void_p(affs_u8.data_ptr()), C.c_void_p(frags.data_ptr()), _lib.i64x3(frags.shape),
                                          float(threshold), int(discretize_queue), self._stream()))
        return frags

    def rag_edge_stats(self, n_edges):
        dev = torch.device("cuda", self.device)
        sums = torch.zeros(max(1, n_edges), dtype=torch.int64, device=dev)
        counts = torch.zeros(max(1, n_edges), dtype=torch.int64, device=dev)
        check(lib.bsmi_rag_edge_stats(self._h, C.c_void_p(sums.data_ptr()), C.c_void_p(counts.data_ptr()), int(n_edges), self._stream()))
        self.status()
        return sums[:n_edges].cpu().numpy(), counts[:n_edges].cpu().numpy()

    def rag_merge_scores_async(self, affs_u8, frags, threshold, discretize_queue, edges, scores, counts, merges=None,
                               merge_scores=None):
        _affs3(affs_u8, contiguous=True)
        _frags_like(frags, affs_u8, contiguous=True)
        if not (edges.is_contiguous() and scores.is_contiguous() and counts.is_contiguous()) or edges.shape[0] != scores.shape[0]:
            raise ValueError("edges / scores / counts must be contiguous and of one capacity")
        check(lib.bsmi_rag_merge_scores_u8(self._h, C.c_void_p(affs_u8.data_ptr()), C.c_void_p(frags.data_ptr()),
                                           _lib.i64x3(frags.shape), float(threshold), int(discretize_queue),
                                           C.c_void_p(edges.data_ptr()), C.c_void_p(scores.data_ptr()), int(edges.shape[0]),
                                           C.c_void_p(merges.data_ptr()) if merges is not None else None,
                                           C.c_void_p(merge_scores.data_ptr()) if merge_scores is not None else None,
                                           C.c_void_p(counts.data_ptr()), self._stream()))

    def rag_graph_async(self, affs_u8, frags, edges, sums, pair_counts, counts):
        _affs3(affs_u8, contiguous=True)
        _frags_like(frags, affs_u8, contiguous=True)
        if (edges.dtype != torch.int64 or sums.dtype != torch.int64 or pair_counts.dtype != torch.int32 or counts.dtype != torch.int64
                or not (edges.is_contiguous() and sums.is_contiguous() and pair_counts.is_contiguous() and counts.is_contiguous())
                or not edges.shape[0] == sums.shape[0] == pair_counts.shape[0]):
            raise ValueError("edges int64 [cap][2], sums int64 [cap], pair_counts int32 [cap], counts int64: contiguous, one capacity")
        check(lib.bsmi_rag_graph_u8(self._h, C.c_void_p(affs_u8.data_ptr()), C.c_void_p(frags.data_ptr()), _lib.i64x3(frags.shape),
                                    C.c_void_p(edges.data_ptr()), C.c_void_p(sums.data_ptr()), C.c_void_p(pair_counts.data_ptr()),
                                    int(edges.shape[0]), C.c_void_p(counts.data_ptr()), self._stream()))

    def cc_affs(self, affs_u8, threshold=0.5, remove_debris=0):
        _affs3(affs_u8)
        a = affs_u8.contiguous()
        shape = tuple(a.shape[1:])
        frags = torch.empty(shape, dtype=torch.int64, device=a.device)
        seg = torch.empty(shape, dtype=torch.int64, device=a.device)
        num = torch.zeros(1, dtype=torch.int64, device=a.device)
        check(lib.bsmi_cc_affs_u8(self._h, C.c_void_p(a.data_ptr()), _lib.i64x3(shape), threshold_to_cut(threshold), int(remove_debris),
                                  C.c_void_p(frags.data_ptr()), C.c_void_p(seg.data_ptr()), C.c_void_p(num.data_ptr()), self._stream()))
        return frags, seg, num

    def label_table(self, labels, z0=0):
        if labels.dtype != torch.int64 or labels.dim() != 3 or not labels.is_cuda:
            raise ValueError("labels must be an int64 CUDA tensor of shape (D, H, W)")
        lab = labels.contiguous()
        cap = max(1024, lab.numel() // 8 + 1024)
        dev = lab.device
        ids = torch.empty(cap, dtype=torch.int64, device=dev)
        counts = torch.empty(cap, dtype=torch.int64, device=dev)
        zmin = torch.empty(cap, dtype=torch.int32, device=dev)
        zmax = torch.empty(cap, dtype=torch.int32, device=dev)
        n = torch.zeros(1, dtype=torch.int64, device=dev)
        check(lib.bsmi_label_table_u64(self._h, C.c_void_p(lab.data_ptr()), _lib.i64x3(lab.shape), int(z0), C.c_void_p(ids.data_ptr()),
                                       C.c_void_p(counts.data_ptr()), C.c_void_p(zmin.data_ptr()), C.c_void_p(zmax.data_ptr()), cap,
                                       C.c_void_p(n.data_ptr()), self._stream()))
        self.status()
        k = int(n.item())
        return (ids[:k].cpu().numpy().view("uint64"), counts[:k].cpu().numpy(), zmin[:k].cpu().numpy(), zmax[:k].cpu().numpy())

    def status(self):
        check(lib.bsmi_seg_status(self._h, self._stream()))


QUEUE_BINS_FORMULAS = {"n_minus_1": 0, "n": 1}


def rag_merge_scores_host(n_edges, edges, sums, pair_counts, threshold=1.0, discretize_queue=256, threads=0, bins_formula="n_minus_1"):
    import numpy as np
    ne = np.ascontiguousarray(n_edges, dtype=np.uint64)
    G = int(ne.shape[0])
    for a in (edges, sums, pair_counts):
        if not (isinstance(a, np.ndarray) and a.flags.c_contiguous and a.flags.writeable):
            raise ValueError("edges, sums and pair_counts must be C-contiguous writable numpy arrays (they are sorted in place)")
    e = edges.view(np.uint64)
    s = sums.view(np.uint64)
    c = pair_counts.view(np.uint32)
    if e.shape[:1] != (G,) or e.ndim != 3 or e.shape[2] != 2 or s.shape != e.shape[:2] or c.shape != e.shape[:2] or int(ne.max(initial=0)) > e.shape[1]:
        raise ValueError("edges [G][cap][2], sums [G][cap], pair_counts [G][cap], n_edges [G] <= cap")
    scores = np.full(e.shape[:2], np.nan, dtype=np.float32)
    ptrs = lambda a, stride: (C.c_void_p * G)(*[a.ctypes.data + g * stride for g in range(G)])
    if bins_formula not in QUEUE_BINS_FORMULAS:
        raise ValueError(f"queue_bins_formula {bins_formula!r}: one of {sorted(QUEUE_BINS_FORMULAS)}")
    check(lib.bsmi_rag_merge_scores_host_rule(G, ne.ctypes.data_as(C.c_void_p), ptrs(e, e.strides[0]), ptrs(s, s.strides[0]), ptrs(c, c.strides[0]),
                                              float(threshold), int(discretize_queue), QUEUE_BINS_FORMULAS[bins_formula],
                                              ptrs(scores, scores.strides[0]), int(threads)))
    return scores


def lut_relabel(labels, keys, vals, out=None):
    if labels.dtype != torch.int64 or not labels.is_cuda:
        raise ValueError("labels must be an int64 CUDA tensor")
    lab = labels.contiguous()
    keys = keys.to(device=lab.device, dtype=torch.int64).contiguous()
    vals = vals.to(device=lab.device, dtype=torch.int64).contiguous()
    if keys.numel() != vals.numel():
        raise ValueError("keys and vals differ in length")
    out = torch.empty_like(lab) if out is None else out
    stream = C.c_void_p(torch.cuda.current_stream(lab.device).cuda_stream)
    check(lib.bsmi_lut_relabel(lab.device.index, C.c_void_p(lab.data_ptr()), lab.numel(), C.c_void_p(keys.data_ptr()),
                               C.c_void_p(vals.data_ptr()), keys.numel(), C.c_void_p(out.data_ptr()), stream))
    return out


def label_morph(labels, op, iterations=1, xy=False, out=None, tmp=None):
    if labels.dtype != torch.int64 or not labels.is_cuda or labels.dim() != 3 or not labels.is_contiguous():
        raise ValueError("labels must be a contiguous int64 CUDA tensor of shape (D, H, W)")
    out = torch.empty_like(labels) if out is None else out
    if tmp is None and iterations > 1:
        tmp = torch.empty_like(labels)
    for t in (out, tmp):
        if t is not None and (t.dtype != torch.int64 or t.device != labels.device or t.numel() < labels.numel() or not t.is_contiguous()):
            raise ValueError("out / tmp must be contiguous int64 tensors of the volume's size on its device")
    stream = C.c_void_p(torch.cuda.current_stream(labels.device).cuda_stream)
    check(lib.bsmi_label_morph_u64(labels.device.index, C.c_void_p(labels.data_ptr()), _lib.i64x3(labels.shape), int(op), int(iterations),
                                   1 if xy else 0, C.c_void_p(out.data_ptr()), C.c_void_p(tmp.data_ptr() if tmp is not None else None), stream))
    return out


def label_fill_holes(labels, xy=False, out=None, table_capacity=None):
    if labels.dtype != torch.int64 or not labels.is_cuda or labels.dim() != 3 or not labels.is_contiguous():
        raise ValueError("labels must be a contiguous int64 CUDA tensor of shape (D, H, W)")
    out = torch.empty_like(labels) if out is None else out
    shape = _lib.i64x3(labels.shape)
    cap = int(table_capacity) if table_capacity else max(1 << 16, 1 << max(0, (labels.numel() // 256 - 1).bit_length()))
    stream = C.c_void_p(torch.cuda.current_stream(labels.device).cuda_stream)
    filled = C.c_uint64(0)
    while True:
        nbytes = int(lib.bsmi_label_fill_holes_scratch_bytes(shape, cap))
        scratch = torch.empty(nbytes, dtype=torch.uint8, device=labels.device)
        rc = lib.bsmi_label_fill_holes_u64(labels.device.index, C.c_void_p(labels.data_ptr()), shape, 1 if xy else 0, C.c_void_p(out.data_ptr()),
                                           C.c_void_p(scratch.data_ptr()), nbytes, cap, C.byref(filled), stream)
        if rc == _lib.ERR_OVERFLOW and cap < (1 << 31):
            del scratch
            cap *= 2
            continue
        check(rc)
        return out, int(filled.value)


def lut_relabel_multi(labels, keys, vals, out=None):
    if labels.dtype != torch.int64 or not labels.is_cuda:
        raise ValueError("labels must be an int64 CUDA tensor")
    lab = labels.contiguous()
    keys = keys.to(device=lab.device, dtype=torch.int64).contiguous()
    vals = vals.to(device=lab.device, dtype=torch.int64).contiguous()
    if vals.dim() != 2 or vals.shape[1] != keys.numel():
# ... 18 lines not shown
```

bootstrapper_amd/volume.py:

```python
import numpy as np
import torch

from . import _lib
from .post.blockwise import shrink_blocks
from .post.engine import SegEngine, lut_relabel


def slab_layers(n_layers, world):
    q, r = divmod(int(n_layers), int(world))
    counts = [q + (1 if i < r else 0) for i in range(world)]
    starts = [sum(counts[:i]) for i in range(world)]
    return starts, counts


def rank_grid(world, layers, rows):
    best = (1, 1)
    for rz in range(1, min(int(world), int(layers)) + 1):
        ry = min(int(world) // rz, int(rows))
        if (rz * ry, rz) > (best[0] * best[1], best[0]):
            best = (rz, ry)
    return best


def exchange_faces(low_out, high_out, low_in, high_in, lo_peer, hi_peer, group=None):
# ... 87 lines not shown

    def __init__(self, slab_shape, block, context, total_layers, layer0, thresholds=(0.2, 0.35, 0.5),
                 fragments_in_xy=True, min_seed_distance=10, filter_fragments=0.0, remove_debris=0, discretize_queue=256,
                 n_lanes=8, device=0, rank=0, world=1, group=None, edge_cap=1 << 17, label_cap=1 << 16, exchange_affs=True,
                 epsilon_agglomerate=0.0, sigma=None, noise_eps=None, bias=None, noise_seed=0, seed_eps=None,
                 grid=None, total_rows=None, row0=0, obj_group=None, host_scores=True, cc_inclusive=True, queue_bins_formula="n_minus_1",
                 lazy_outputs=False):
        self.host_scores = bool(host_scores)
        self.cc_inclusive = bool(cc_inclusive)
        self.queue_bins_formula = str(queue_bins_formula)
        from .post.engine import QUEUE_BINS_FORMULAS
        if self.queue_bins_formula not in QUEUE_BINS_FORMULAS:
            raise ValueError(f"queue_bins_formula {queue_bins_formula!r}: one of {sorted(QUEUE_BINS_FORMULAS)}")
        if self.queue_bins_formula != "n_minus_1" and not self.host_scores:
            raise NotImplementedError("the device merge loop (host_scores=False) implements the specified bin rule only")
        self.shape = tuple(int(s) for s in slab_shape)
        self.block = tuple(int(b) for b in block)
        self.ctx = tuple(int(c) for c in context)
        self.thresholds = [float(t) for t in thresholds]
        self.fragments_in_xy, self.msd = bool(fragments_in_xy), int(min_seed_distance)
        self.filter_fragments, self.remove_debris = float(filter_fragments), int(remove_debris)
        self.bins = int(discretize_queue)
        self.epsilon = float(epsilon_agglomerate or 0.0)
        self.shift = dict(sigma=sigma, noise_eps=noise_eps, bias=bias, seed_eps=seed_eps)
        self.noise_seed = int(noise_seed)
        self.rank, self.world, self.group = int(rank), int(world), group
        self.obj_group = obj_group if obj_group is not None else group
        self.grid = (int(world), 1) if grid is None else (int(grid[0]), int(grid[1]))
        if self.grid[0] * self.grid[1] != self.world:
            raise ValueError(f"rank grid {self.grid} for {self.world} ranks")
        self.rz, self.ry = divmod(self.rank, self.grid[1])
        self.peers = ((self.rank - self.grid[1] if self.rz > 0 else None, self.rank + self.grid[1] if self.rz < self.grid[0] - 1 else None),
                      (self.rank - 1 if self.ry > 0 else None, self.rank + 1 if self.ry < self.grid[1] - 1 else None))
        self.exchange_affs = bool(exchange_affs)
        self.dev = torch.device("cuda", int(device))
        self.boxes = shrink_blocks(self.shape, self.block)
        counts = self.counts = [-(-s // b) for s, b in zip(self.shape, self.block)]
        rows = counts[1] if total_rows is None else int(total_rows)
        self.block_ids = [((int(layer0) + iz) * rows + (int(row0) + iy)) * counts[2] + ix
                          for iz in range(counts[0]) for iy in range(counts[1]) for ix in range(counts[2])]
        self.total_blocks = int(total_layers) * rows * counts[2]
        self.nvb = int(np.prod(self.block))
        padded = tuple(s + 2 * c for s, c in zip(self.shape, self.ctx))
        K = len(self.boxes)
        read_vox = int(np.prod([min(b, s) + 2 * c for b, s, c in zip(self.block, self.shape, self.ctx)]))
        self.edge_cap = max(64, min(int(edge_cap), 3 * read_vox))
        self.label_cap = max(64, min(int(label_cap), self.nvb))
        need = self.hbm_bytes(self.shape, self.ctx, len(self.thresholds), K, self.label_cap, self.edge_cap)
        free, _total = torch.cuda.mem_get_info(self.dev)
        free += torch.cuda.memory_reserved(self.dev) - torch.cuda.memory_allocated(self.dev)
        if need > free:
            per_layer = need / max(1, self.counts[0])
            raise MemoryError(f"a slab of {self.shape} voxels needs {need / 2**30:.1f} GiB of HBM ({need / max(1, int(np.prod(self.shape))):.0f} B per voxel: "
                              f"affinities, fragments, {len(self.thresholds)} segmentations, per-block tables) and {free / 2**30:.1f} GiB are free on "
                              f"{self.dev}: give each rank at most {max(1, int(free // per_layer))} block layer(s), i.e. use more workers / GPUs")
        self.affs = torch.zeros((3,) + padded, dtype=torch.uint8, device=self.dev)
        self.frags = torch.zeros(padded, dtype=torch.int64, device=self.dev)
        self.segs = self._fr = self._one = None
        if not lazy_outputs:
            self.segs = torch.empty((len(self.thresholds),) + self.shape, dtype=torch.int64, device=self.dev)
            self._fr = torch.empty(self.shape, dtype=torch.int64, device=self.dev)
        self.nums = torch.zeros(K, dtype=torch.int64, device=self.dev)
        self.sizes = torch.zeros((K, self.label_cap), dtype=torch.int64, device=self.dev)
        self.sums = torch.zeros((K, self.label_cap, 3), dtype=torch.int64, device=self.dev)
        self.edges = torch.empty((K, self.edge_cap, 2), dtype=torch.int64, device=self.dev)
        self.scores = torch.empty((K, self.edge_cap), dtype=torch.float32, device=self.dev)
        self.esums = torch.empty((K, self.edge_cap), dtype=torch.int64, device=self.dev) if self.host_scores else None
        self.counts_dev = torch.zeros((K, 4), dtype=torch.int64, device=self.dev)
        self.frag_done = [None] * K
        read = tuple(min(b, s) + 2 * c for b, s, c in zip(self.block, self.shape, self.ctx))
        self.lanes = []
        import torch.distributed as dist
        import os
        dist_cap = int(os.environ.get("BSMI_DIST_LANES", "16"))
        if int(n_lanes) > dist_cap and dist.is_available() and dist.is_initialized() and "nccl" in str(dist.get_backend()):
            n_lanes = dist_cap
        for stream in lane_streams(self.dev, max(1, min(int(n_lanes), K))):
            self.lanes.append(dict(engine=SegEngine(read, self.dev.index), stream=stream,
                                   a=torch.empty((3,) + read, dtype=torch.uint8, device=self.dev),
                                   f=torch.empty(read, dtype=torch.int64, device=self.dev),
                                   lab=torch.empty(tuple(min(b, s) for b, s in zip(self.block, self.shape)), dtype=torch.int64,
                                                   device=self.dev)))
        torch.cuda.current_stream(self.dev).synchronize()
        self.nodes = None
        self.rag_edges = self.rag_scores = None
        self.luts = None
        self._lane_load = [0] * len(self.lanes)
        self._lane_of = {}
        self._lane_limit = len(self.lanes)
        self.overlap_lanes = 3
        self.timers = {"exchange": 0.0, "blocks": 0.0, "stitch": 0.0}

    @staticmethod
    def hbm_bytes(shape, ctx, n_thresholds, n_blocks, label_cap=1 << 16, edge_cap=1 << 17):
        vox = int(np.prod(shape))
        padded = int(np.prod([s + 2 * c for s, c in zip(shape, ctx)]))
        return 11 * padded + 8 * vox * (1 + n_thresholds) + n_blocks * (32 * label_cap + 28 * edge_cap + 40)

    def interior(self, t):
        sl = tuple(slice(c, c + s) for c, s in zip(self.ctx, self.shape))
        return t[(Ellipsis,) + sl]

    def write_view(self, k):
        b, e = self.boxes[k]
        return self.affs[(slice(None),) + tuple(slice(c + lo, c + hi) for c, lo, hi in zip(self.ctx, b, e))]

    def _read_slices(self, k):
        b, e = self.boxes[k]
        return tuple(slice(lo, hi + 2 * c) for c, lo, hi in zip(self.ctx, b, e))

    def _buf(self, t, shape, lead=()):
        n = int(np.prod(lead + shape))
        return t.reshape(-1)[:n].view(lead + shape)

    def _exchange(self, t):
        import time
        t_in = time.perf_counter()
        if self.world > 1 and (t is not self.affs or self.exchange_affs):
            c, Z = self.ctx[0], self.shape[0]
            if c > 0:
                exchange_faces(t[..., c:2 * c, :, :], t[..., Z:Z + c, :, :], t[..., 0:c, :, :], t[..., Z + c:Z + 2 * c, :, :],
                               self.peers[0][0], self.peers[0][1], self.group)
            c, Y = self.ctx[1], self.shape[1]
            if c > 0:
                exchange_faces(t[..., :, c:2 * c, :], t[..., :, Y:Y + c, :], t[..., :, 0:c, :], t[..., :, Y + c:Y + 2 * c, :],
                               self.peers[1][0], self.peers[1][1], self.group)
        ev = torch.cuda.Event()
        ev.record(torch.cuda.current_stream(self.dev))
        self.timers["exchange"] += time.perf_counter() - t_in
        return ev

    def _sync(self):
        err = None
        for lane in self.lanes:
            lane["stream"].synchronize()
            try:
                lane["engine"].status()
            except _lib.BsmiError as exc:
                if exc.code != _lib.ERR_OVERFLOW:
                    raise
                err = err or exc
        return err

    @staticmethod
    def _only_edge_buffer(err):
        import re
        m = re.search(r"flags 0x([0-9a-f]+)", str(err))
        return bool(m) and int(m.group(1), 16) == 32

    def _neighbours(self, k):
        cy, cx = self.counts[1], self.counts[2]
        iz, r = divmod(k, cy * cx)
        iy, ix = divmod(r, cx)
        out = []
        for dz in (-1, 0, 1):
            for dy in (-1, 0, 1):
                for dx in (-1, 0, 1):
                    z, y, x = iz + dz, iy + dy, ix + dx
                    if 0 <= z < self.counts[0] and 0 <= y < cy and 0 <= x < cx:
                        out.append((z * cy + y) * cx + x)
        return out

    def _on_face(self, k):
        iz, r = divmod(k, self.counts[1] * self.counts[2])
        iy = r // self.counts[2]
        (zlo, zhi), (ylo, yhi) = self.peers
        return ((self.ctx[0] > 0 and ((zlo is not None and iz == 0) or (zhi is not None and iz == self.counts[0] - 1))) or
                (self.ctx[1] > 0 and ((ylo is not None and iy == 0) or (yhi is not None and iy == self.counts[1] - 1))))

    def _take_lane(self, kind, k):
        i = min(range(min(len(self.lanes), self._lane_limit)), key=lambda j: (self._lane_load[j], j))
        self._lane_load[i] += 1
        self._lane_of[(kind, k)] = i
        return self.lanes[i]

    def lane_of(self, kind, k):
        return self.lanes[self._lane_of[(kind, k)]]

    def _launch_fragments(self, k, wait=()):
        b, e = self.boxes[k]
        lane = self._take_lane("f", k)
        wshape = tuple(hi - lo for lo, hi in zip(b, e))
        rshape = tuple(w + 2 * c for w, c in zip(wshape, self.ctx))
        with torch.cuda.stream(lane["stream"]):
            for ev in wait:
                lane["stream"].wait_event(ev)
            a = self._buf(lane["a"], rshape, (3,))
            a.copy_(self.affs[(slice(None),) + self._read_slices(k)])
            eng = lane["engine"]
            if any(v is not None for v in self.shift.values()):
                from .post.shifts import boundary_mask_affinities
                gen = torch.Generator(device=self.dev).manual_seed(self.noise_seed + self.block_ids[k])
                src = boundary_mask_affinities(a, self.fragments_in_xy, dtype=torch.float64, generator=gen, min_seed_distance=self.msd,
                                               **self.shift)
            else:
                src = a
            fr, _ = eng.ws_fragments(src, self.fragments_in_xy, self.msd)
            if self.epsilon > 0:
                eng.rag_agglomerate(a, fr, self.epsilon, 256)
            lab = self._buf(lane["lab"], wshape)
            eng.postprocess_fragments(a, fr, self.filter_fragments, self.remove_debris, self.ctx, wshape,
                                      self.block_ids[k] * self.nvb, out=lab, num=self.nums[k:k + 1])
            self.frags[tuple(slice(c + lo, c + hi) for c, lo, hi in zip(self.ctx, b, e))].copy_(lab)
            eng.label_stats(lab, self.block_ids[k] * self.nvb, self.label_cap, size=self.sizes[k], sums=self.sums[k])
            self.frag_done[k] = torch.cuda.Event()
            self.frag_done[k].record(lane["stream"])

    def _launch_scores(self, k, wait=()):
        b, e = self.boxes[k]
        lane = self._take_lane("s", k)
        rshape = tuple(hi - lo + 2 * c for lo, hi, c in zip(b, e, self.ctx))
        with torch.cuda.stream(lane["stream"]):
            for ev in wait:
                lane["stream"].wait_event(ev)
            a = self._buf(lane["a"], rshape, (3,))
            a.copy_(self.affs[(slice(None),) + self._read_slices(k)])
            f = self._buf(lane["f"], rshape)
            f.copy_(self.frags[self._read_slices(k)])
            if self.host_scores:
                lane["engine"].rag_graph_async(a, f, self.edges[k], self.esums[k], self.scores[k].view(torch.int32), self.counts_dev[k])
            else:
                lane["engine"].rag_merge_scores_async(a, f, 1.0, self.bins, self.edges[k], self.scores[k], self.counts_dev[k])

    def _collect(self):
        err = self._sync()
        nums = self.nums.cpu().numpy()
        if nums.max(initial=0) >= self.nvb:
            raise _lib.BsmiError(_lib.ERR_OVERFLOW, f"a block produced {int(nums.max())} fragments: not below its {self.nvb} voxels")
        n_edges = self.counts_dev[:, 0].cpu().numpy()
        if (err is None or self._only_edge_buffer(err)) and (nums.max(initial=0) > self.label_cap or n_edges.max(initial=0) > self.edge_cap):
            err = self._regrow(nums, n_edges)
        if err is not None:
            raise err
        self.block_nums = nums
        if self.host_scores:
            from .post.engine import rag_merge_scores_host
            m = int(n_edges.max(initial=0))
            if m == 0:
                self.rag_edges, self.rag_scores = np.zeros((0, 2), np.uint64), np.zeros(0, np.float32)
                return 0
            E = self.edges[:, :m].cpu().numpy().view(np.uint64)
            S = self.esums[:, :m].cpu().numpy()
            C = self.scores.view(torch.int32)[:, :m].cpu().numpy()
            sc = rag_merge_scores_host(n_edges, E, S, C, 1.0, self.bins, bins_formula=self.queue_bins_formula)
            es, ss = [], []
            for k in range(len(self.boxes)):
                first = np.uint64(self.block_ids[k]) * np.uint64(self.nvb) + np.uint64(1)
                lo, hi = np.searchsorted(E[k, :n_edges[k], 0], [first, first + np.uint64(self.nvb)])
                es.append(E[k, lo:hi])
                ss.append(sc[k, lo:hi])
            self.rag_edges = np.concatenate(es)
            self.rag_scores = np.concatenate(ss)
            return len(self.rag_scores)
        ne = self.counts_dev[:, 0]
        take = torch.arange(self.edge_cap, device=self.dev)[None, :] < ne[:, None]
        bid = torch.tensor(self.block_ids, dtype=torch.int64, device=self.dev)[:, None].expand(-1, self.edge_cap)
        own = take & (torch.div(self.edges[:, :, 0] - 1, self.nvb, rounding_mode="floor") == bid)
        self.rag_edges = self.edges[own].cpu().numpy().view(np.uint64)
        self.rag_scores = self.scores[own].cpu().numpy()
        return len(self.rag_scores)

    def _regrow(self, nums, n_edges):
        K = len(self.boxes)
        if nums.max(initial=0) > self.label_cap:
            old, self.label_cap = self.label_cap, min(self.nvb, int(nums.max()) * 5 // 4 + 64)
            sizes = torch.zeros((K, self.label_cap), dtype=torch.int64, device=self.dev)
            sums = torch.zeros((K, self.label_cap, 3), dtype=torch.int64, device=self.dev)
            sizes[:, :old].copy_(self.sizes)
            sums[:, :old].copy_(self.sums)
            self.sizes, self.sums = sizes, sums
            torch.cuda.current_stream(self.dev).synchronize()
            for k in np.nonzero(nums > old)[0]:
                b, e = self.boxes[k]
                lane = self._take_lane("n", int(k))
                with torch.cuda.stream(lane["stream"]):
                    lab = self.frags[tuple(slice(c + lo, c + hi) for c, lo, hi in zip(self.ctx, b, e))].contiguous()
                    lane["engine"].label_stats(lab, self.block_ids[k] * self.nvb, self.label_cap, size=self.sizes[k], sums=self.sums[k])
        if n_edges.max(initial=0) > self.edge_cap:
            old, self.edge_cap = self.edge_cap, int(n_edges.max()) * 5 // 4 + 64
            edges = torch.empty((K, self.edge_cap, 2), dtype=torch.int64, device=self.dev)
            scores = torch.empty((K, self.edge_cap), dtype=torch.float32, device=self.dev)
            edges[:, :old].copy_(self.edges)
            scores[:, :old].copy_(self.scores)
            self.edges, self.scores = edges, scores
            if self.host_scores:
                esums = torch.empty((K, self.edge_cap), dtype=torch.int64, device=self.dev)
                esums[:, :old].copy_(self.esums)
                self.esums = esums
            torch.cuda.current_stream(self.dev).synchronize()
            for k in np.nonzero(n_edges > old)[0]:
                self._launch_scores(int(k))
        return self._sync()

    def run_blocks(self, ready=None, overlap=False):
        K = len(self.boxes)
        self._lane_load = [0] * len(self.lanes)
        self._lane_of = {}
        self._lane_limit = len(self.lanes)
        last = [max(self._neighbours(k)) for k in range(K)]
        face = [k for k in range(K) if self._on_face(k)]
        inner = [k for k in range(K) if not self._on_face(k)]
        inner_set = set(inner)
        if ready is None:
            here = torch.cuda.Event()
            here.record(torch.cuda.current_stream(self.dev))
            ready = [here] * K
        nb = [self._neighbours(k) for k in range(K)]
        queued, scored = set(), set()

        def score_what_can_be(candidates, extra=()):
            for j in candidates:
                if j not in scored and all(i in queued for i in nb[j]):
                    self._launch_scores(j, list(extra) + [self.frag_done[i] for i in nb[j]])
                    scored.add(j)
        err = None

        def guarded(phase):
            nonlocal err
            if err is not None:
                return
            try:
                phase()
            except Exception as exc:
                from .blockwise import is_fatal
                if self.world == 1 or is_fatal(exc):
                    raise
                err = exc

        def launch_inner():
            for k in inner:
                self._launch_fragments(k, (ready[K - 1],))
                queued.add(k)
        def launch_overlapped():
            import time
            todo_f = list(inner)
            todo_s = [j for j in inner if all(i in inner_set for i in nb[j])]
            while todo_f or todo_s:
                moved = False
                self._lane_limit = len(self.lanes) if ready[K - 1].query() else max(1, min(self.overlap_lanes, len(self.lanes)))
                while todo_f and ready[last[todo_f[0]]].query():
                    k = todo_f.pop(0)
                    self._launch_fragments(k, ())
                    queued.add(k)
                    moved = True
                for j in list(todo_s):
                    if all(i in queued and self.frag_done[i].query() for i in nb[j]):
                        self._launch_scores(j, ())
                        scored.add(j)
                        todo_s.remove(j)
                        moved = True
                if not moved:
                    time.sleep(0.0002)
        if overlap:
            guarded(launch_overlapped)
            self._lane_limit = len(self.lanes)
        if not overlap:
            guarded(launch_inner)
        if face:
            guarded(lambda: ready[K - 1].synchronize())
            self._agree(err)
            got = self._exchange(self.affs)

            def launch_face():
                for k in face:
                    self._launch_fragments(k, (got,))
                    queued.add(k)
                    if overlap:
                        score_what_can_be([j for j in nb[k] if j in inner_set])
            guarded(launch_face)
        guarded(lambda: score_what_can_be(inner))
        if face:
            def await_outer():
                (zlo, zhi), (ylo, yhi) = self.peers
                for k in range(K):
                    iz, r = divmod(k, self.counts[1] * self.counts[2])
                    iy = r // self.counts[2]
                    if ((zlo is not None and iz == 0) or (zhi is not None and iz == self.counts[0] - 1) or
                            (ylo is not None and iy == 0) or (yhi is not None and iy == self.counts[1] - 1)):
                        self.frag_done[k].synchronize()
            guarded(await_outer)
            self._agree(err)
            got = self._exchange(self.frags)
            score_what_can_be(face, (got,))
        if err is not None:
            raise err
        return self._collect()

    def _agree(self, err):
        if self.world == 1:
            if err is not None:
                raise err
            return
        import torch.distributed as dist
        flag = torch.tensor([0 if err is None else 1], dtype=torch.int32,
                            device=self.dev if dist.get_backend(self.group) == "nccl" else "cpu")
        dist.all_reduce(flag, op=dist.ReduceOp.MAX, group=self.group)
        if int(flag.item()):
            raise err if err is not None else RuntimeError("another rank failed in front of a face exchange: leaving the stage with it")

    def run_blocks_accounted(self, max_retries=None):
        import torch.distributed as dist
        from .blockwise import MAX_RETRIES, TaskState, run_blocks
        max_retries = MAX_RETRIES if max_retries is None else max_retries
        K = len(self.boxes)
        failed = 0
        try:
            self.run_blocks()
        except Exception as exc:
            from .blockwise import is_fatal
            if is_fatal(exc):
                raise
            failed = 1
        if self.world > 1:
            flag = torch.tensor([failed], dtype=torch.int32, device=self.dev if dist.get_backend(self.group) == "nccl" else "cpu")
            dist.all_reduce(flag, op=dist.ReduceOp.MAX, group=self.group)
            failed = int(flag.item())
        names = ("WatershedFrags", "WaterzAgglom")
        if not failed:
            states = {}
            for n in names:
                states[n] = TaskState(n, K)
                states[n].completed_count = K
            return states

        def one(launch, kind):
            def run(k):
                launch(k)
                lane = self.lane_of(kind, k)
                lane["stream"].synchronize()
                lane["engine"].status()
            return run
        here = self._exchange(self.affs)
        here.synchronize()
        st_f = run_blocks(names[0], list(range(K)), one(self._launch_fragments, "f"), max_retries)
        for k in st_f.failed_blocks:
            b, e = self.boxes[k]
            self.frags[tuple(slice(c + lo, c + hi) for c, lo, hi in zip(self.ctx, b, e))].zero_()
            self.nums[k] = 0
        torch.cuda.synchronize(self.dev)
        self._exchange(self.frags).synchronize()
        self.counts_dev.zero_()
        torch.cuda.current_stream(self.dev).synchronize()
        st_s = run_blocks(names[1], list(range(K)), one(self._launch_scores, "s"), max_retries, upstream_failed=st_f.failed_blocks,
                          depends_on=self._neighbours)
        self._collect()
        return {names[0]: st_f, names[1]: st_s}

    def node_table(self):
        nums = np.asarray([int(n) for n in self.block_nums], dtype=np.int64)
        if nums.sum() == 0:
            return np.zeros(0, np.uint64), np.zeros((0, 3)), np.zeros(0, np.int64)
        used = torch.arange(self.label_cap, device=self.dev)[None, :] < torch.from_numpy(nums).to(self.dev)[:, None]
        sizes = self.sizes[used].cpu().numpy()
        sums = self.sums[used].cpu().numpy().astype(np.float64)
        first = np.repeat(np.asarray([b for b, _ in self.boxes], np.float64), nums, axis=0)
        ids = np.concatenate([np.arange(1, n + 1, dtype=np.uint64) + np.uint64(bid * self.nvb) for n, bid in zip(nums, self.block_ids) if n])
        return ids, first + sums / sizes[:, None], sizes

    def ensure_outputs(self, one=False):
        if self._fr is None:
            self._fr = torch.empty(self.shape, dtype=torch.int64, device=self.dev)
        if one and self._one is None:
            self._one = torch.empty(self.shape, dtype=torch.int64, device=self.dev)
        if not one and self.segs is None:
            self.segs = torch.empty((len(self.thresholds),) + self.shape, dtype=torch.int64, device=self.dev)

    def stitch(self, consume=None):
        nodes = np.concatenate([np.arange(1, int(n) + 1, dtype=np.uint64) + np.uint64(bid * self.nvb)
                                for n, bid in zip(self.block_nums, self.block_ids)] or [np.zeros(0, np.uint64)])
        thr = self.thresholds if self.cc_inclusive else [float(np.nextafter(np.float32(t), np.float32(-np.inf))) for t in self.thresholds]
        self.nodes, self.luts = gather_and_stitch(nodes, self.rag_edges, self.rag_scores, thr, self.rank, self.world, self.obj_group)
        self.ensure_outputs(one=consume is not None)
        fr = self._fr
        fr.copy_(self.interior(self.frags))
        keys = torch.from_numpy(self.nodes.view(np.int64)).to(self.dev)
        if consume is not None:
            for t, comp in enumerate(self.luts):
                lut_relabel(fr, keys, torch.from_numpy(comp.view(np.int64)).to(self.dev), out=self._one)
                torch.cuda.current_stream(self.dev).synchronize()
                consume(t, self._one)
            return None
        if 1 <= len(self.luts) <= 8:
            from .post.engine import lut_relabel_multi
            lut_relabel_multi(fr, keys, torch.from_numpy(np.stack([c.view(np.int64) for c in self.luts])).to(self.dev), out=self.segs)
        else:
            for t, comp in enumerate(self.luts):
                lut_relabel(fr, keys, torch.from_numpy(comp.view(np.int64)).to(self.dev), out=self.segs[t])
        torch.cuda.synchronize(self.dev)
        return self.segs

    def prime(self):
        self.prime_lanes()
        self._collect()
        return self.stitch()

    def prime_lanes(self):
        if len(self.boxes):
            for i in range(len(self.lanes)):
                self._lane_load = [1] * len(self.lanes)
                self._lane_load[i] = 0
                self._launch_fragments(0)
                self._lane_load = [1] * len(self.lanes)
                self._lane_load[i] = 0
                self._launch_scores(0)
            self._lane_load = [0] * len(self.lanes)
            for lane in self.lanes:
                lane["stream"].synchronize()

    def run(self, ready=None, overlap=False):
        if ready is not None and not overlap:
            ready[-1].synchronize()
        import time
        self.timers = {"exchange": 0.0, "blocks": 0.0, "stitch": 0.0}
        t0 = time.perf_counter()
        self.run_blocks(ready, overlap)
        t1 = time.perf_counter()
        segs = self.stitch()
        self.timers["blocks"], self.timers["stitch"] = t1 - t0, time.perf_counter() - t1
        return segs


class VolumePipeline:

    def __init__(self, model, out_block, net_context, job_blocks, seg_context=(16, 16, 16), thresholds=(0.2, 0.35, 0.5),
                 min_seed_distance=10, filter_fragments=0.0, remove_debris=0, n_lanes=20, device=0, rank=0, world=1,
                 group=None, job_origin=(0, 0, 0), segment=True, overlap=False, obj_group=None):
        self.models = list(model) if isinstance(model, (list, tuple)) else [model]
        model = self.model = self.models[0]
        self.out_block = tuple(int(b) for b in out_block)
        self.net_context = tuple(int(c) for c in net_context)
        self.in_block = tuple(o + 2 * c for o, c in zip(self.out_block, self.net_context))
        if model.output_shape(self.in_block) != self.out_block:
            raise ValueError(f"network maps {self.in_block} to {model.output_shape(self.in_block)}, not {self.out_block}")
        self.job_blocks = tuple(int(g) for g in job_blocks)
        self.rank, self.world = int(rank), int(world)
        self.dev = torch.device("cuda", int(device))
        slab = tuple(g * b for g, b in zip(self.job_blocks, self.out_block))
        self.origin = (int(job_origin[0]) + self.rank * slab[0], int(job_origin[1]), int(job_origin[2]))
        self.pred_stream = predict_stream(self.dev)
        self.pred_streams = [predict_stream(self.dev, i) for i in range(len(self.models))]
        self.seg = SlabSegmenter(slab, self.out_block, seg_context if segment else (0, 0, 0), self.job_blocks[0] * self.world,
                                 self.job_blocks[0] * self.rank, thresholds, True, min_seed_distance, filter_fragments,
                                 remove_debris, 256, n_lanes if segment else 1, device, rank, world, group, obj_group=obj_group)
        self.segment = bool(segment)
        self.overlap = bool(overlap)
        self.t_predict = 0.0

    def predict(self, volume_u8):
        from .unet import extract_block_reflect
        ready = []
        K = len(self.models)
        n = len(self.seg.boxes)
        self._t0 = torch.cuda.Event(enable_timing=True)
        self._t0.record(self.pred_stream)
        for lane in range(1, K):
            self.pred_streams[lane].wait_event(self._t0)
        for k, (b, _) in enumerate(self.seg.boxes):
            lane = k % K
            st = self.pred_streams[lane]
            with torch.cuda.stream(st):
                off = [o + lo - c for o, lo, c in zip(self.origin, b, self.net_context)]
                raw = extract_block_reflect(volume_u8, off, self.in_block)
                u8 = self.models[lane].predict_u8(raw)
                self.seg.write_view(k).copy_(u8[0][:3])
                last = k + 1 == n
                if last and K > 1:
                    for j in range(max(0, n - K), n - 1):
                        self.pred_stream.wait_event(ready[j])
                    done = torch.cuda.Event()
                    done.record(st)
                    self.pred_stream.wait_event(done)
                    st = self.pred_stream
                ev = torch.cuda.Event(enable_timing=last)
                ev.record(st)
                ready.append(ev)
        return ready

    def run(self, volume_u8):
        ready = self.predict(volume_u8)
        segs = self.seg.run(ready, self.overlap) if self.segment else None
        ready[-1].synchronize()
        self.t_predict = self._t0.elapsed_time(ready[-1]) * 1e-3
        return segs
```

include/bsmi.h:

```cpp
#ifndef BSMI_H
#define BSMI_H

#include <stddef.h>
#include <stdint.h>

#ifdef __cplusplus
extern "C" {
#endif

#define BSMI_MAX_LEVELS 8
#define BSMI_MAX_CONVS 4
#define BSMI_MAX_HEADS 4
#define BSMI_NAME_LEN 32

#define BSMI_OK 0
#define BSMI_ERR_INVALID (-1)
#define BSMI_ERR_HIP (-2)
#define BSMI_ERR_STATE (-3)
#define BSMI_ERR_MISSING (-4)
#define BSMI_ERR_OVERFLOW (-5)

#define BSMI_PREC_F32 0
#define BSMI_PREC_BF16 1
#define BSMI_PREC_BF16X3 2
// ... 142 lines not shown

int bsmi_ws_fragments_seeds_u8(bsmi_seg *h, const uint8_t *affs_dev, const int64_t shape[3],
                               int fragments_in_xy, int min_seed_distance, uint64_t *frags_dev,
                               uint64_t *max_id_dev, uint64_t *seeds_dev, void *stream);

int bsmi_agglomerate_mean_u8(bsmi_seg *h, const uint8_t *affs_dev, const uint64_t *frags_dev,
                             const int64_t shape[3], const float *thresholds_host,
                             int n_thresholds, uint64_t *segs_dev, void *stream);

int bsmi_agglomerate_hist_u8(bsmi_seg *h, const uint8_t *affs_dev, const uint64_t *frags_dev,
                             const int64_t shape[3], const float *thresholds_host, int n_thresholds,
                             int quantile, int init_with_max, uint64_t *segs_dev, void *stream);

int bsmi_agglomerate_hist_graph(uint32_t n_nodes, uint32_t n_edges, const uint32_t *edge_u, const uint32_t *edge_v,
                                uint32_t *hist, int quantile, int init_with_max, const float *thresholds,
                                int n_thresholds, uint32_t *roots_out);

int bsmi_frag_postprocess_u8(bsmi_seg *h, const uint8_t *affs_dev, uint64_t *frags_dev,
                             const int64_t shape[3], double filter_value, int64_t min_size,
                             const int64_t crop_offset[3], const int64_t crop_shape[3],
                             uint64_t id_offset, uint64_t *out_dev, uint64_t *num_labels_dev,
                             void *stream);

int bsmi_label_stats(bsmi_seg *h, const uint64_t *labels_dev, const int64_t shape[3], uint64_t id_offset,
                     uint64_t num, uint64_t *size_dev, uint64_t *sums_dev, void *stream);

int bsmi_rag_merge_scores_u8(bsmi_seg *h, const uint8_t *affs_dev, const uint64_t *frags_dev,
                             const int64_t shape[3], float threshold, int discretize_queue,
                             uint64_t *edges_dev, float *scores_dev, uint64_t edge_capacity,
                             uint64_t *merges_dev, float *merge_scores_dev, uint64_t *counts_dev,
                             void *stream);

int bsmi_rag_graph_u8(bsmi_seg *h, const uint8_t *affs_dev, const uint64_t *frags_dev, const int64_t shape[3],
                      uint64_t *edges_dev, uint64_t *sums_dev, uint32_t *pair_counts_dev, uint64_t edge_capacity,
                      uint64_t *counts_dev, void *stream);
int bsmi_rag_merge_scores_host(int n_graphs, const uint64_t *n_edges, uint64_t *const *edges, uint64_t *const *sums,
                               uint32_t *const *pair_counts, float threshold, int discretize_queue, float *const *scores,
                               int n_threads);
#define BSMI_QUEUE_BINS_N_MINUS_1 0
#define BSMI_QUEUE_BINS_N 1
int bsmi_rag_merge_scores_host_rule(int n_graphs, const uint64_t *n_edges, uint64_t *const *edges, uint64_t *const *sums,
                                    uint32_t *const *pair_counts, float threshold, int discretize_queue, int bin_rule,
                                    float *const *scores, int n_threads);

int bsmi_rag_agglomerate_u8(bsmi_seg *h, const uint8_t *affs_dev, uint64_t *frags_dev, const int64_t shape[3],
                            float threshold, int discretize_queue, void *stream);

int bsmi_rag_edge_stats(bsmi_seg *h, uint64_t *sums_dev, uint64_t *counts_dev, uint64_t capacity, void *stream);

int bsmi_lut_relabel(int device, const uint64_t *in_dev, uint64_t n, const uint64_t *keys_dev,
                     const uint64_t *vals_dev, uint64_t m, uint64_t *out_dev, void *stream);
int bsmi_lut_relabel_multi(int device, const uint64_t *in_dev, uint64_t n, const uint64_t *keys_dev,
                           const uint64_t *vals_dev, uint64_t m, int n_columns, uint64_t *out_dev, void *stream);

int bsmi_connected_components(const uint64_t *nodes, uint64_t n, const uint64_t *edges,
                              const float *scores, uint64_t m, float threshold, uint64_t *components);
int bsmi_connected_components_multi(const uint64_t *nodes, uint64_t n, const uint64_t *edges,
                                    const float *scores, uint64_t m, const float *thresholds,
                                    int n_thresholds, uint64_t *components);

int bsmi_cc_affs_u8(bsmi_seg *h, const uint8_t *affs_dev, const int64_t shape[3], int cut, int64_t min_size,
                    uint64_t *frags_dev, uint64_t *seg_dev, uint64_t *num_labels_dev, void *stream);

int bsmi_mws_agglom_f64(int device, const double *affs_dev, int n_offsets, const int32_t *offsets,
                        const int32_t *strides, uint32_t random_seed, const int64_t shape[3],
                        uint64_t *labels_dev, void *stream);

int bsmi_mws_cluster(uint64_t n_nodes, const uint64_t *edges, const double *scores, uint64_t m,
                     uint64_t *labels_out);

int bsmi_frag_pair_affinity_u8(int device, const uint8_t *affs_dev, int n_offsets, const int32_t *offsets,
                               const uint64_t *dense_dev, const int64_t shape[3], uint64_t capacity,
                               uint64_t *pairs_out, uint64_t *sums_out, uint64_t *counts_out,
                               uint64_t *n_pairs, void *stream);

int bsmi_label_table_u64(bsmi_seg *h, const uint64_t *labels_dev, const int64_t shape[3], int64_t z0,
                         uint64_t *ids_dev, uint64_t *counts_dev, int32_t *zmin_dev, int32_t *zmax_dev,
                         uint64_t capacity, uint64_t *n_dev, void *stream);

int bsmi_seg_set_host_flood(bsmi_seg *h, int on);

int bsmi_seg_status(bsmi_seg *h, void *stream);

typedef struct bsmi_eval bsmi_eval;
int bsmi_eval_create(int device, uint64_t pair_capacity, bsmi_eval **out);
int bsmi_eval_destroy(bsmi_eval *h);

int bsmi_eval_aff_errors_u8(bsmi_eval *h, const uint64_t *seg_dev, const int64_t seg_shape[3], const int64_t seg_origin[3],
                            const uint8_t *pred_dev, int n_channels, const int64_t tile_shape[3], const uint8_t *mask_dev,
                            const int32_t *offsets, const int64_t chunk_shape[3], float floor_, float ceil_, int64_t count_z_end,
                            uint8_t *error_map_dev, uint8_t *error_mask_dev, uint64_t *hist_dev, void *stream);

int bsmi_eval_lsd_errors_u8(bsmi_eval *h, const uint64_t *seg_dev, const int64_t seg_shape[3], const int64_t seg_origin[3],
                            const uint8_t *pred_dev, const uint8_t *mask_dev, const int64_t tile_shape[3],
                            const int64_t chunk_shape[3], const int64_t margin[3], const int64_t context[3], const float sigma[3],
                            const float voxel_size[3], int downsample, float floor_, float ceil_, int64_t count_z_end,
                            uint64_t scratch_limit_bytes, uint8_t *error_map_dev, uint8_t *error_mask_dev, uint64_t *hist_dev,
                            float *debug_desc_dev, float *debug_diff_dev, float *debug_max_dev, uint8_t *debug_raw_mask_dev,
                            void *stream);

int bsmi_eval_pairs_u64(bsmi_eval *h, const uint64_t *gt_dev, const uint64_t *seg_dev, const uint8_t *mask_dev,
                        const int64_t shape[3], int reset, void *stream);

int bsmi_eval_pairs_read(bsmi_eval *h, uint64_t *gt_out_dev, uint64_t *seg_out_dev, uint64_t *count_out_dev,
                         uint64_t out_capacity, uint64_t *n_dev, void *stream);

int bsmi_eval_status(bsmi_eval *h, void *stream);

#define BSMI_MORPH_DILATE 0
#define BSMI_MORPH_ERODE 1
int bsmi_label_morph_u64(int device, const uint64_t *in_dev, const int64_t shape[3], int op, int iterations, int xy,
                         uint64_t *out_dev, uint64_t *tmp_dev, void *stream);

#define BSMI_MORPH_MERGE_NUM 19ull
#define BSMI_MORPH_MERGE_DEN 20ull
size_t bsmi_label_fill_holes_scratch_bytes(const int64_t shape[3], uint64_t table_capacity);
int bsmi_label_fill_holes_u64(int device, const uint64_t *in_dev, const int64_t shape[3], int xy, uint64_t *out_dev,
                              void *scratch_dev, size_t scratch_bytes, uint64_t table_capacity, uint64_t *n_filled,
                              void *stream);

size_t bsmi_mask_closing_work_bytes(const int64_t shape[3], int radius);
int bsmi_mask_closing_disk_u8(int device, const uint8_t *in_dev, const int64_t shape[3], int radius, uint8_t *out_dev,
                              void *work_dev, size_t work_bytes, void *stream);

#define BSMI_RESCALE_DOWN 0
#define BSMI_RESCALE_UP 1
int bsmi_downscale_mean(int device, const void *in_dev, int itemsize, const int64_t in_shape[3], const int32_t factor[3],
                        const int32_t lead[3], void *out_dev, const int64_t out_shape[3], void *stream);
int bsmi_rescale_sample(int device, const void *in_dev, int itemsize, const int64_t in_shape[3], const int32_t factor[3],
                        const int32_t lead[3], int mode, void *out_dev, const int64_t out_shape[3], void *stream);

int bsmi_nonzero_bbox(int device, const void *in_dev, int itemsize, const int64_t shape[3], const int64_t origin[3],
                      int64_t *box_dev, void *stream);

typedef struct bsmi_synth bsmi_synth;
int bsmi_synth_create(int device, const int64_t max_shape[3], bsmi_synth **out);
int bsmi_synth_destroy(bsmi_synth *h);
int bsmi_synth_dilate_points(bsmi_synth *h, const int64_t shape[3], const int32_t *points, int n_points, const uint32_t *bitmaps,
                             const int32_t *bitmap_sizes, const int32_t *iterations, int32_t *out_dev, void *stream);
int bsmi_synth_label_i32(bsmi_synth *h, const int32_t *in_dev, const int64_t shape[3], int32_t *out_dev, uint64_t *num_host, void *stream);
int bsmi_synth_expand_i32(bsmi_synth *h, const int32_t *labels_dev, const int64_t shape[3], int depth, int32_t fill, int32_t *out_dev,
                          void *stream);
int bsmi_synth_tubes_i32(bsmi_synth *h, const int32_t *fg_dev, const int64_t shape[3], int32_t *out_dev, uint64_t *num_host, void *stream);
int bsmi_synth_gaussian_f32(bsmi_synth *h, const float *in_dev, const int64_t shape[3], const float *weights, int radius, float *out_dev,
                            void *stream);
int bsmi_synth_argmax_filter_f32(bsmi_synth *h, const float *field_dev, const int64_t shape[3], int window, int32_t *pos_dev, void *stream);
int bsmi_synth_basins_f32(bsmi_synth *h, const float *field_dev, const int32_t *pos_dev, const uint8_t *mask_dev, const int64_t shape[3],
                          int32_t *out_dev, uint64_t *num_host, void *stream);
int bsmi_synth_finish_i32(bsmi_synth *h, const int32_t *in_dev, const int64_t shape[3], int drop3, int drop5, int anisotropy, int64_t *out_dev,
                          void *stream);
int bsmi_synth_grow_boundary_i64(int device, const int64_t *in_dev, const int64_t shape[3], uint64_t seed, int max_steps, int64_t *out_dev,
                                 void *stream);
int bsmi_synth_merge_i64(int device, int64_t *labels_dev, const int64_t shape[3], const int32_t *sections, int n_sections, int64_t a, int64_t b,
                         void *stream);
int bsmi_synth_stamp_i64(int device, int64_t *labels_dev, const int64_t shape[3], int z, int y, int x, const uint32_t *bitmap, int bitmap_h,
                         int bitmap_w, int64_t value, void *stream);
int bsmi_synth_present_i64(bsmi_synth *h, const int64_t *labels_dev, uint64_t n_voxels, int64_t *ids_dev, uint32_t capacity, uint32_t *count_host,
                           void *stream);
int bsmi_synth_split_i64(bsmi_synth *h, int64_t *labels_dev, const int64_t shape[3], int64_t id, int window, const int32_t *sections,
                         int n_sections, int64_t scale, uint64_t *num_host, void *stream);

#ifdef __cplusplus
}
#endif
#endif
```

Baseline: 97.68.

## Batch per-block fragment and RAG-graph kernels across workspaces in one launch

Adds a batched segmentation API that runs fragment extraction and RAG graph construction for up to 32 blocks per launch. A device-side table of per-block workspaces is indexed by blockIdx.y, and the Python pipeline groups same-shaped blocks onto batcher streams. This replaces many small per-block kernel launches spread over lanes. The cost is more complex scheduling and event handling, with a fallback to per-lane launches when the batch path refuses a shape. The batched path is only used when overlap is disabled.

```diff
diff --git a/bootstrapper_amd/_lib.py b/bootstrapper_amd/_lib.py
--- a/bootstrapper_amd/_lib.py
+++ b/bootstrapper_amd/_lib.py
@@ -49,6 +49,16 @@
 class ChunkCopy(C.Structure):
     _fields_ = [("path", C.c_char_p), ("base", C.c_void_p), ("start", C.c_int64 * 4), ("extent", C.c_int64 * 4),
                 ("stride", C.c_int64 * 4), ("read_modify_write", C.c_int32), ("reserved", C.c_int32)]
+
+
+class BatchFragArgs(C.Structure):
+    _fields_ = [("affs_dev", C.c_void_p), ("frags_dev", C.c_void_p), ("max_id_dev", C.c_void_p), ("labels_dev", C.c_void_p),
+                ("num_labels_dev", C.c_void_p), ("id_offset", C.c_uint64), ("size_dev", C.c_void_p), ("sums_dev", C.c_void_p)]
+
+
+class BatchGraphArgs(C.Structure):
+    _fields_ = [("affs_dev", C.c_void_p), ("frags_dev", C.c_void_p), ("edges_dev", C.c_void_p), ("sums_dev", C.c_void_p),
+                ("pair_counts_dev", C.c_void_p), ("counts_dev", C.c_void_p), ("edge_capacity", C.c_uint64)]
 
 
 CODEC_RAW, CODEC_ZLIB, CODEC_GZIP, CODEC_ZSTD, CODEC_LZ4, CODEC_BLOSC = range(6)
@@ -112,6 +122,10 @@
         "bsmi_label_table_u64": (i32, [p, vp, i64p, C.c_int64, vp, vp, vp, vp, C.c_uint64, vp, vp]),
         "bsmi_seg_status": (i32, [p, vp]),
         "bsmi_seg_set_host_flood": (i32, [p, i32]),
+        "bsmi_seg_batch_create": (i32, [C.POINTER(p), i32, C.POINTER(p)]),
+        "bsmi_seg_batch_destroy": (i32, [p]),
+        "bsmi_seg_batch_fragments_u8": (i32, [p, i32, C.POINTER(BatchFragArgs), i64p, i32, i32, C.c_double, C.c_int64, i64p, i64p, C.c_uint64, vp]),
+        "bsmi_seg_batch_rag_graph_u8": (i32, [p, i32, C.POINTER(BatchGraphArgs), i64p, vp]),
         "bsmi_rag_graph_u8": (i32, [p, vp, vp, i64p, vp, vp, vp, C.c_uint64, vp, vp]),
         "bsmi_rag_merge_scores_host": (i32, [i32, vp, vp, vp, vp, C.c_float, i32, vp, i32]),
         "bsmi_rag_merge_scores_host_rule": (i32, [i32, vp, vp, vp, vp, C.c_float, i32, i32, vp, i32]),
diff --git a/bootstrapper_amd/csrc/seg.hip b/bootstrapper_amd/csrc/seg.hip
--- a/bootstrapper_amd/csrc/seg.hip
+++ b/bootstrapper_amd/csrc/seg.hip
@@ -8,7 +8,7 @@
 
 namespace bsmi {
 
-__global__ __launch_bounds__(256) void fill_list_kernel(FillList L) {
+__device__ __forceinline__ void fill_list_body(const FillList& L) {
   const size_t stride = (size_t)gridDim.x * blockDim.x, t0 = (size_t)blockIdx.x * blockDim.x + threadIdx.x;
   for (int j = 0; j < L.n; ++j) {
     uint32_t* p = L.p[j];
@@ -24,9 +24,15 @@
     if (t0 < w - done) p[done + t0] = v;
   }
 }
+__global__ __launch_bounds__(256) void fill_list_kernel(FillList L) { fill_list_body(L); }
+__global__ __launch_bounds__(256) void fill_list_batch_kernel(const BatchBlock* __restrict__ tab) { fill_list_body(tab[blockIdx.y].fills); }
 void Fills::launch(hipStream_t s) const {
   const unsigned grid = (unsigned)std::min<size_t>((most + 255) / 256 + 1, 2048);
   hipLaunchKernelGGL(fill_list_kernel, dim3(grid), dim3(256), 0, s, L);
+}
+void batch_fill_launch(const BatchBlock* tab, int N, size_t most, hipStream_t s) {
+  const unsigned grid = (unsigned)std::min<size_t>((most + 255) / 256 + 1, 2048);
+  hipLaunchKernelGGL(fill_list_batch_kernel, dim3(grid, N), dim3(256), 0, s, tab);
 }
 
 template <typename T>
diff --git a/bootstrapper_amd/csrc/seg_batch.hip b/bootstrapper_amd/csrc/seg_batch.hip
--- /dev/null
+++ b/bootstrapper_amd/csrc/seg_batch.hip
@@ -0,0 +1,178 @@
+#include "seg_internal.h"
+
+#include "dev_guard.h"
+
+struct bsmi_seg_batch {
+  int device = 0;
+  int n = 0;
+  std::vector<bsmi_seg*> handles;
+  bsmi::BatchBlock* tab = nullptr;
+  uint32_t max_frag_id_cap = 0, max_icap = 0, max_hcap = 0;
+};
+
+namespace bsmi {
+
+static_assert(sizeof(BatchFragArgs) == sizeof(bsmi_batch_frag_args) && sizeof(BatchGraphArgs) == sizeof(bsmi_batch_graph_args),
+              "include/bsmi.h and seg_internal.h disagree on the per-block arguments");
+
+struct BatchFragCall { BatchFragArgs a[kMaxBatch]; };
+struct BatchGraphCall { BatchGraphArgs a[kMaxBatch]; };
+
+__global__ __launch_bounds__(64) void batch_set_frag_kernel(BatchBlock* tab, BatchFragCall c, uint64_t stats_num, int with_filter) {
+  if (threadIdx.x != 0) return;
+  BatchBlock& b = tab[blockIdx.x];
+  const BatchFragArgs a = c.a[blockIdx.x];
+  b.f = a;
+  FillList L{};
+  L.p[0] = b.frag.flags; L.words[0] = 4;
+  L.p[1] = (uint32_t*)a.size; L.words[1] = 2 * (size_t)stats_num;
+  L.p[2] = (uint32_t*)a.sums; L.words[2] = 6 * (size_t)stats_num;
+  L.n = 3;
+  if (with_filter) {
+    L.p[3] = (uint32_t*)b.frag.lsum; L.words[3] = 2 * (size_t)b.frag.id_cap;
+    L.p[4] = b.frag.lcnt; L.words[4] = (size_t)b.frag.id_cap;
+    L.n = 5;
+  }
+  b.fills = L;
+}
+
+__global__ __launch_bounds__(64) void batch_set_graph_kernel(BatchBlock* tab, BatchGraphCall c) {
+  if (threadIdx.x != 0) return;
+  BatchBlock& b = tab[blockIdx.x];
+  const BatchGraphArgs a = c.a[blockIdx.x];
+  b.g = a;
+  FillList L{};
+  L.p[0] = b.agg.counters; L.words[0] = 8;
+  L.p[1] = (uint32_t*)a.counts; L.words[1] = 6;
+  L.p[2] = (uint32_t*)b.agg.idkeys; L.words[2] = 2 * (size_t)b.agg.icap; L.value[2] = 0xffffffffu;
+  L.p[3] = (uint32_t*)b.agg.hkeys; L.words[3] = 2 * (size_t)b.agg.hcap; L.value[3] = 0xffffffffu;
+  L.p[4] = (uint32_t*)b.agg.hsum; L.words[4] = 2 * (size_t)b.agg.hcap;
+  L.p[5] = b.agg.hcnt; L.words[5] = (size_t)b.agg.hcap;
+  L.n = 6;
+  b.fills = L;
+}
+
+static int batch_check(bsmi_seg_batch* b, int n_blocks, const void* args, const int64_t shape[3]) {
+  if (!b || !args || !shape) BSMI_FAIL(BSMI_ERR_INVALID, "null argument");
+  if (n_blocks < 1 || n_blocks > b->n) BSMI_FAIL(BSMI_ERR_INVALID, "%d blocks for a batch of %d workspaces", n_blocks, b->n);
+  for (int i = 0; i < n_blocks; ++i) {
+    const int rc = check_seg_shape(b->handles[i], shape);
+    if (rc) return rc;
+  }
+  if (shape[1] > 4096 || shape[2] > 4096 || !batch_ws_lds_bytes((int)shape[1], (int)shape[2]))
+    BSMI_FAIL(BSMI_ERR_INVALID, "slices of %lld x %lld are off the LDS / compact path: not served in batches", (long long)shape[1],
+              (long long)shape[2]);
+  return BSMI_OK;
+}
+
+}
+
+using namespace bsmi;
+
+extern "C" {
+
+int bsmi_seg_batch_create(bsmi_seg* const* handles, int n, bsmi_seg_batch** out) {
+  if (!handles || !out) BSMI_FAIL(BSMI_ERR_INVALID, "null argument");
+  if (n < 1 || n > kMaxBatch) BSMI_FAIL(BSMI_ERR_INVALID, "a batch takes 1 to %d workspaces (got %d)", kMaxBatch, n);
+  for (int i = 0; i < n; ++i) {
+    if (!handles[i]) BSMI_FAIL(BSMI_ERR_INVALID, "null handle");
+    if (handles[i]->device != handles[0]->device) BSMI_FAIL(BSMI_ERR_INVALID, "the workspaces of a batch must be on one device");
+    for (int j = 0; j < i; ++j)
+      if (handles[j] == handles[i]) BSMI_FAIL(BSMI_ERR_INVALID, "a workspace appears twice in the batch");
+  }
+  BSMI_HIP(hipSetDevice(handles[0]->device));
+  bsmi_seg_batch* b = new bsmi_seg_batch;
+  b->device = handles[0]->device;
+  b->n = n;
+  b->handles.assign(handles, handles + n);
+  std::vector<BatchBlock> rows(n);
+  for (int i = 0; i < n; ++i) {
+    const bsmi_seg* h = handles[i];
+    BatchBlock& r = rows[i];
+    r = BatchBlock{};
+    r.ws = h->ws;
+    r.ws.seedlab = nullptr;
+    r.flood_spill = h->flood_spill;
+    r.flood_spill_stride = h->flood_spill_stride;
+    r.status = h->status_dev;
+    r.frag = h->frag;
+    r.crop_tmp = h->crop_tmp;
+    r.agg = h->agg;
+    b->max_frag_id_cap = std::max(b->max_frag_id_cap, h->frag.id_cap);
+    b->max_icap = std::max(b->max_icap, h->agg.icap);
+    b->max_hcap = std::max(b->max_hcap, h->agg.hcap);
+  }
+  void* q = nullptr;
+  hipError_t err = hipMalloc(&q, sizeof(BatchBlock) * n);
+  if (err == hipSuccess) err = hipMemcpy(q, rows.data(), sizeof(BatchBlock) * n, hipMemcpyHostToDevice);
+  if (err == hipSuccess) err = hipDeviceSynchronize();
+  if (err != hipSuccess) {
+    if (q) (void)hipFree(q);
+    delete b;
+    BSMI_HIP(err);
+  }
+  b->tab = (BatchBlock*)q;
+  *out = b;
+  return BSMI_OK;
+}
+
+int bsmi_seg_batch_destroy(bsmi_seg_batch* b) {
+  if (!b) return BSMI_OK;
+  (void)hipSetDevice(b->device);
+  if (b->tab) (void)hipFree(b->tab);
+  delete b;
+  return BSMI_OK;
+}
+
+int bsmi_seg_batch_fragments_u8(bsmi_seg_batch* b, int n_blocks, const bsmi_batch_frag_args* args, const int64_t shape[3],
+                                int fragments_in_xy, int min_seed_distance, double filter_value, int64_t min_size,
+                                const int64_t crop_offset[3], const int64_t crop_shape[3], uint64_t stats_num, void* stream) {
+  int rc = batch_check(b, n_blocks, args, shape);
+  if (rc) return rc;
+  if (!fragments_in_xy) BSMI_FAIL(BSMI_ERR_INVALID, "the 3-D fragments mode is not served in batches");
+  if (min_seed_distance < 1 || min_seed_distance > 64) BSMI_FAIL(BSMI_ERR_INVALID, "min_seed_distance out of range");
+  if (!crop_offset || !crop_shape) BSMI_FAIL(BSMI_ERR_INVALID, "null argument");
+  for (int d = 0; d < 3; ++d)
+    if (crop_offset[d] < 0 || crop_shape[d] < 1 || crop_offset[d] + crop_shape[d] > shape[d])
+      BSMI_FAIL(BSMI_ERR_INVALID, "crop outside the fragment volume");
+  BatchFragCall call{};
+  for (int i = 0; i < n_blocks; ++i) {
+    const bsmi_batch_frag_args& a = args[i];
+    if (!a.affs_dev || !a.frags_dev || !a.max_id_dev || !a.labels_dev || !a.num_labels_dev || !a.size_dev || !a.sums_dev)
+      BSMI_FAIL(BSMI_ERR_INVALID, "null argument (block %d)", i);
+    call.a[i] = BatchFragArgs{a.affs_dev, a.frags_dev, a.max_id_dev, a.labels_dev, a.num_labels_dev, a.id_offset, a.size_dev, a.sums_dev};
+  }
+  BSMI_HIP(hipSetDevice(b->device));
+  hipStream_t s = (hipStream_t)stream;
+  const bool with_filter = filter_value > 0.0 || min_size > 0;
+  hipLaunchKernelGGL(batch_set_frag_kernel, dim3(n_blocks), dim3(64), 0, s, b->tab, call, stats_num, with_filter ? 1 : 0);
+  size_t most = (size_t)stats_num * 24 / 16;
+  if (with_filter) most = std::max(most, (size_t)b->max_frag_id_cap * 8 / 16);
+  batch_fill_launch(b->tab, n_blocks, most, s);
+  rc = batch_ws_launch(b->tab, n_blocks, (int)shape[0], (int)shape[1], (int)shape[2], min_seed_distance, s);
+  if (rc) return rc;
+  batch_post_launch(b->tab, n_blocks, shape, filter_value, min_size, crop_offset, crop_shape, stats_num, s);
+  BSMI_HIP(hipGetLastError());
+  return BSMI_OK;
+}
+
+int bsmi_seg_batch_rag_graph_u8(bsmi_seg_batch* b, int n_blocks, const bsmi_batch_graph_args* args, const int64_t shape[3], void* stream) {
+  int rc = batch_check(b, n_blocks, args, shape);
+  if (rc) return rc;
+  BatchGraphCall call{};
+  for (int i = 0; i < n_blocks; ++i) {
+    const bsmi_batch_graph_args& a = args[i];
+    if (!a.affs_dev || !a.frags_dev || !a.edges_dev || !a.sums_dev || !a.pair_counts_dev || !a.counts_dev)
+      BSMI_FAIL(BSMI_ERR_INVALID, "null argument (block %d)", i);
+    call.a[i] = BatchGraphArgs{a.affs_dev, a.frags_dev, a.edges_dev, a.sums_dev, a.pair_counts_dev, a.counts_dev, a.edge_capacity};
+  }
+  BSMI_HIP(hipSetDevice(b->device));
+  hipStream_t s = (hipStream_t)stream;
+  hipLaunchKernelGGL(batch_set_graph_kernel, dim3(n_blocks), dim3(64), 0, s, b->tab, call);
+  batch_fill_launch(b->tab, n_blocks, (size_t)std::max(b->max_icap, b->max_hcap) * 8 / 16, s);
+  batch_graph_launch(b->tab, n_blocks, shape, b->max_hcap, s);
+  BSMI_HIP(hipGetLastError());
+  return BSMI_OK;
+}
+
+}
diff --git a/bootstrapper_amd/csrc/seg_graph.hip b/bootstrapper_amd/csrc/seg_graph.hip
--- a/bootstrapper_amd/csrc/seg_graph.hip
+++ b/bootstrapper_amd/csrc/seg_graph.hip
@@ -80,8 +80,8 @@
 }
 
 template <bool HASH>
-__global__ void agg_edges_kernel(const uint8_t* __restrict__ affs, const uint64_t* __restrict__ frags, int D, int H,
-                                 int W, AggWs w) {
+__device__ __forceinline__ void agg_edges_body(const uint8_t* __restrict__ affs, const uint64_t* __restrict__ frags, int D, int H,
+                                 int W, const AggWs& w) {
   if (w.counters[3]) return;
   const size_t n = (size_t)D * H * W;
   const size_t hw = (size_t)H * W;
@@ -114,6 +114,15 @@
       atomicAdd(&w.hcnt[slot], 1u);
     }
   }
+}
+template <bool HASH>
+__global__ void agg_edges_kernel(const uint8_t* __restrict__ affs, const uint64_t* __restrict__ frags, int D, int H,
+                                 int W, AggWs w) {
+  agg_edges_body<HASH>(affs, frags, D, H, W, w);
+}
+__global__ void agg_edges_batch_kernel(const BatchBlock* __restrict__ tab, int D, int H, int W) {
+  const BatchBlock& b = tab[blockIdx.y];
+  agg_edges_body<true>(b.g.affs, b.g.frags, D, H, W, b.agg);
 }
 
 __global__ void agg_compact_kernel(AggWs w) {
@@ -432,7 +441,7 @@
   }
 }
 
-__global__ void rag_ids_kernel(const uint64_t* __restrict__ frags, size_t n, int W, AggWs w) {
+__device__ __forceinline__ void rag_ids_body(const uint64_t* __restrict__ frags, size_t n, int W, const AggWs& w) {
   for (size_t p = (size_t)blockIdx.x * blockDim.x + threadIdx.x; p < n; p += (size_t)gridDim.x * blockDim.x) {
     const uint64_t f = frags[p];
     if (!f) continue;
@@ -458,6 +467,11 @@
     }
     if (!done) atomicOr(&w.counters[3], 2u);
   }
+}
+__global__ void rag_ids_kernel(const uint64_t* __restrict__ frags, size_t n, int W, AggWs w) { rag_ids_body(frags, n, W, w); }
+__global__ void rag_ids_batch_kernel(const BatchBlock* __restrict__ tab, size_t n, int W) {
+  const BatchBlock& b = tab[blockIdx.y];
+  rag_ids_body(b.g.frags, n, W, b.agg);
 }
 
 __global__ void rag_pad_kernel(AggWs w) {
@@ -854,7 +868,7 @@
     }
 }
 
-__global__ void rag_graph_hash_out_kernel(AggWs w, uint64_t* __restrict__ edges, uint64_t* __restrict__ sums, uint32_t* __restrict__ cnts,
+__device__ __forceinline__ void rag_graph_hash_out_body(const AggWs& w, uint64_t* __restrict__ edges, uint64_t* __restrict__ sums, uint32_t* __restrict__ cnts,
                                           uint64_t cap, uint64_t* __restrict__ counts) {
   keep_overflow(w);
   if (w.counters[3]) return;
@@ -874,6 +888,12 @@
     cnts[e] = w.hcnt[sl];
   }
 }
+__global__ void rag_graph_hash_out_kernel(AggWs w, uint64_t* __restrict__ edges, uint64_t* __restrict__ sums, uint32_t* __restrict__ cnts,
+                                          uint64_t cap, uint64_t* __restrict__ counts) { rag_graph_hash_out_body(w, edges, sums, cnts, cap, counts); }
+__global__ void rag_graph_hash_out_batch_kernel(const BatchBlock* __restrict__ tab) {
+  const BatchBlock& b = tab[blockIdx.y];
+  rag_graph_hash_out_body(b.agg, b.g.edges, b.g.sums, b.g.pair_counts, b.g.edge_capacity, b.g.counts);
+}
 
 __global__ void rag_relabel_kernel(uint64_t* __restrict__ frags, size_t n, AggWs w) {
   keep_overflow(w);
@@ -909,6 +929,15 @@
     w.hsum[i] = 0;
     w.hcnt[i] = 0;
   }
+}
+
+void batch_graph_launch(const BatchBlock* tab, int N, const int64_t shape[3], uint32_t max_hcap, hipStream_t s) {
+  const size_t n = (size_t)shape[0] * shape[1] * shape[2];
+  const int bs = 256;
+  const dim3 grid((unsigned)std::min<size_t>((n + bs - 1) / bs, 4096), N);
+  hipLaunchKernelGGL(rag_ids_batch_kernel, grid, dim3(bs), 0, s, tab, n, (int)shape[2]);
+  hipLaunchKernelGGL(agg_edges_batch_kernel, grid, dim3(bs), 0, s, tab, (int)shape[0], (int)shape[1], (int)shape[2]);
+  hipLaunchKernelGGL(rag_graph_hash_out_batch_kernel, dim3(std::min<uint32_t>(max_hcap / bs, 2048u), N), dim3(bs), 0, s, tab);
 }
 
 int seg_scan_grid() {
diff --git a/bootstrapper_amd/csrc/seg_internal.h b/bootstrapper_amd/csrc/seg_internal.h
--- a/bootstrapper_amd/csrc/seg_internal.h
+++ b/bootstrapper_amd/csrc/seg_internal.h
@@ -126,6 +126,28 @@
   void launch(hipStream_t s) const;
 };
 
+constexpr int kMaxBatch = 32;
+struct BatchFragArgs {
+  const uint8_t* affs; uint64_t* frags; uint64_t* max_id; uint64_t* labels; uint64_t* num; uint64_t id_offset;
+  uint64_t* size; uint64_t* sums;
+};
+struct BatchGraphArgs {
+  const uint8_t* affs; const uint64_t* frags; uint64_t* edges; uint64_t* sums; uint32_t* pair_counts; uint64_t* counts;
+  uint64_t edge_capacity;
+};
+struct BatchBlock {
+  WsScratch ws;
+  uint64_t* flood_spill;
+  size_t flood_spill_stride;
+  int* status;
+  FragWs frag;
+  uint64_t* crop_tmp;
+  AggWs agg;
+  BatchFragArgs f;
+  BatchGraphArgs g;
+  FillList fills;
+};
+
 }
 
 struct bsmi_seg {
@@ -156,6 +178,13 @@
 int fragments_3d(bsmi_seg* h, const uint8_t* affs_dev, int D, int H, int W, int min_seed_distance, uint64_t* frags_dev,
                  uint64_t* max_id_dev, uint64_t* seeds_dev, hipStream_t s);
 
+void batch_fill_launch(const BatchBlock* tab, int N, size_t most, hipStream_t s);
+size_t batch_ws_lds_bytes(int H, int W);
+int batch_ws_launch(const BatchBlock* tab, int N, int D, int H, int W, int msd, hipStream_t s);
+void batch_post_launch(const BatchBlock* tab, int N, const int64_t shape[3], double filter_value, int64_t min_size, const int64_t crop_offset[3],
+                       const int64_t crop_shape[3], uint64_t stats_num, hipStream_t s);
+void batch_graph_launch(const BatchBlock* tab, int N, const int64_t shape[3], uint32_t max_hcap, hipStream_t s);
+
 void cc_rank_roots(size_t n, const FragWs& f, uint64_t* num_out, hipStream_t s);
 
 hipError_t seg_sort_tmp_bytes(int n_keys, int n_pairs, size_t* bytes);
diff --git a/bootstrapper_amd/csrc/seg_labels.hip b/bootstrapper_amd/csrc/seg_labels.hip
--- a/bootstrapper_amd/csrc/seg_labels.hip
+++ b/bootstrapper_amd/csrc/seg_labels.hip
@@ -52,7 +52,7 @@
   }
 }
 
-__global__ void frag_stats_kernel(const uint8_t* __restrict__ affs, const uint64_t* __restrict__ frags, size_t n, FragWs w) {
+__device__ __forceinline__ void frag_stats_body(const uint8_t* __restrict__ affs, const uint64_t* __restrict__ frags, size_t n, const FragWs& w) {
   for (size_t p = (size_t)blockIdx.x * blockDim.x + threadIdx.x; p < n; p += (size_t)gridDim.x * blockDim.x) {
     const uint64_t f = frags[p];
     if (!f) continue;
@@ -61,8 +61,13 @@
     atomicAdd(&w.lcnt[f], 1u);
   }
 }
-
-__global__ void frag_decide_kernel(const uint8_t* __restrict__ affs, const uint64_t* __restrict__ frags, size_t n, FragWs w,
+__global__ void frag_stats_kernel(const uint8_t* __restrict__ affs, const uint64_t* __restrict__ frags, size_t n, FragWs w) { frag_stats_body(affs, frags, n, w); }
+__global__ void frag_stats_batch_kernel(const BatchBlock* __restrict__ tab, size_t n) {
+  const BatchBlock& b = tab[blockIdx.y];
+  frag_stats_body(b.f.affs, b.f.frags, n, b.frag);
+}
+
+__device__ __forceinline__ void frag_decide_body(const uint8_t* __restrict__ affs, const uint64_t* __restrict__ frags, size_t n, const FragWs& w,
                                    double filter_value, long long min_size) {
   for (uint32_t f = blockIdx.x * blockDim.x + threadIdx.x; f < w.id_cap; f += gridDim.x * blockDim.x) {
     const uint32_t c = w.lcnt[f];
@@ -83,16 +88,27 @@
     if (drop) w.lcnt[f] = c | 0x80000000u;
   }
 }
-
-__global__ void frag_filter_kernel(uint64_t* __restrict__ frags, size_t n, FragWs w) {
+__global__ void frag_decide_kernel(const uint8_t* __restrict__ affs, const uint64_t* __restrict__ frags, size_t n, FragWs w,
+                                   double filter_value, long long min_size) { frag_decide_body(affs, frags, n, w, filter_value, min_size); }
+__global__ void frag_decide_batch_kernel(const BatchBlock* __restrict__ tab, size_t n, double filter_value, long long min_size) {
+  const BatchBlock& b = tab[blockIdx.y];
+  frag_decide_body(b.f.affs, b.f.frags, n, b.frag, filter_value, min_size);
+}
+
+__device__ __forceinline__ void frag_filter_body(uint64_t* __restrict__ frags, size_t n, const FragWs& w) {
   for (size_t p = (size_t)blockIdx.x * blockDim.x + threadIdx.x; p < n; p += (size_t)gridDim.x * blockDim.x) {
     const uint64_t f = frags[p];
     if (!f || f >= w.id_cap) continue;
     if (w.lcnt[f] & 0x80000000u) frags[p] = 0;
   }
 }
-
-__global__ void crop_u64_kernel(const uint64_t* __restrict__ in, int H, int W, int oz, int oy, int ox, int cd, int ch,
+__global__ void frag_filter_kernel(uint64_t* __restrict__ frags, size_t n, FragWs w) { frag_filter_body(frags, n, w); }
+__global__ void frag_filter_batch_kernel(const BatchBlock* __restrict__ tab, size_t n) {
+  const BatchBlock& b = tab[blockIdx.y];
+  frag_filter_body(b.f.frags, n, b.frag);
+}
+
+__device__ __forceinline__ void crop_u64_body(const uint64_t* __restrict__ in, int H, int W, int oz, int oy, int ox, int cd, int ch,
                                 int cw, uint64_t* __restrict__ out) {
   const size_t n = (size_t)cd * ch * cw;
   for (size_t i = (size_t)blockIdx.x * blockDim.x + threadIdx.x; i < n; i += (size_t)gridDim.x * blockDim.x) {
@@ -102,13 +118,24 @@
     out[i] = in[((size_t)(z + oz) * H + (y + oy)) * W + (x + ox)];
   }
 }
-
-__global__ void cc26_init_kernel(const uint64_t* __restrict__ x, size_t n, FragWs w) {
+__global__ void crop_u64_kernel(const uint64_t* __restrict__ in, int H, int W, int oz, int oy, int ox, int cd, int ch,
+                                int cw, uint64_t* __restrict__ out) { crop_u64_body(in, H, W, oz, oy, ox, cd, ch, cw, out); }
+__global__ void crop_u64_batch_kernel(const BatchBlock* __restrict__ tab, int H, int W, int oz, int oy, int ox, int cd, int ch, int cw) {
+  const BatchBlock& b = tab[blockIdx.y];
+  crop_u64_body(b.f.frags, H, W, oz, oy, ox, cd, ch, cw, b.crop_tmp);
+}
+
+__device__ __forceinline__ void cc26_init_body(const uint64_t* __restrict__ x, size_t n, const FragWs& w) {
   for (size_t p = (size_t)blockIdx.x * blockDim.x + threadIdx.x; p < n; p += (size_t)gridDim.x * blockDim.x)
     w.par[p] = x[p] ? (int32_t)p : -1;
 }
-
-__global__ void cc26_union_kernel(const uint64_t* __restrict__ x, int D, int H, int W, FragWs w) {
+__global__ void cc26_init_kernel(const uint64_t* __restrict__ x, size_t n, FragWs w) { cc26_init_body(x, n, w); }
+__global__ void cc26_init_batch_kernel(const BatchBlock* __restrict__ tab, size_t n) {
+  const BatchBlock& b = tab[blockIdx.y];
+  cc26_init_body(b.crop_tmp, n, b.frag);
+}
+
+__device__ __forceinline__ void cc26_union_body(const uint64_t* __restrict__ x, int D, int H, int W, const FragWs& w) {
   const size_t n = (size_t)D * H * W;
   for (size_t p = (size_t)blockIdx.x * blockDim.x + threadIdx.x; p < n; p += (size_t)gridDim.x * blockDim.x) {
     const uint64_t v = x[p];
@@ -128,8 +155,13 @@
         }
   }
 }
-
-__global__ __launch_bounds__(1024) void cc26_count_kernel(size_t n, FragWs w) {
+__global__ void cc26_union_kernel(const uint64_t* __restrict__ x, int D, int H, int W, FragWs w) { cc26_union_body(x, D, H, W, w); }
+__global__ void cc26_union_batch_kernel(const BatchBlock* __restrict__ tab, int D, int H, int W) {
+  const BatchBlock& b = tab[blockIdx.y];
+  cc26_union_body(b.crop_tmp, D, H, W, b.frag);
+}
+
+__device__ __forceinline__ void cc26_count_body(size_t n, const FragWs& w) {
   __shared__ uint32_t cnt;
   if (threadIdx.x == 0) cnt = 0;
   __syncthreads();
@@ -138,8 +170,13 @@
   __syncthreads();
   if (threadIdx.x == 0) w.blk[blockIdx.x] = cnt;
 }
-
-__global__ __launch_bounds__(1024) void cc26_scan_kernel(uint32_t nblk, FragWs w, uint64_t* num_out) {
+__global__ __launch_bounds__(1024) void cc26_count_kernel(size_t n, FragWs w) { cc26_count_body(n, w); }
+__global__ __launch_bounds__(1024) void cc26_count_batch_kernel(const BatchBlock* __restrict__ tab, size_t n) {
+  const BatchBlock& b = tab[blockIdx.y];
+  cc26_count_body(n, b.frag);
+}
+
+__device__ __forceinline__ void cc26_scan_body(uint32_t nblk, const FragWs& w, uint64_t* num_out) {
   __shared__ uint32_t sh[1024];
   const uint32_t chunk = (nblk + 1023) / 1024;
   const uint32_t c0 = threadIdx.x * chunk, c1 = min(nblk, c0 + chunk);
@@ -156,8 +193,13 @@
   uint32_t acc = sh[threadIdx.x];
   for (uint32_t i = c0; i < c1; ++i) { const uint32_t c = w.blk[i]; w.blk[i] = acc; acc += c; }
 }
-
-__global__ __launch_bounds__(1024) void cc26_rank_kernel(size_t n, FragWs w) {
+__global__ __launch_bounds__(1024) void cc26_scan_kernel(uint32_t nblk, FragWs w, uint64_t* num_out) { cc26_scan_body(nblk, w, num_out); }
+__global__ __launch_bounds__(1024) void cc26_scan_batch_kernel(const BatchBlock* __restrict__ tab, uint32_t nblk) {
+  const BatchBlock& b = tab[blockIdx.y];
+  cc26_scan_body(nblk, b.frag, b.f.num);
+}
+
+__device__ __forceinline__ void cc26_rank_body(size_t n, const FragWs& w) {
   __shared__ uint32_t sh[1024];
   const size_t p = (size_t)blockIdx.x * 1024 + threadIdx.x;
   const uint32_t flag = (p < n && w.par[p] == (int32_t)p) ? 1u : 0u;
@@ -171,6 +213,11 @@
   }
   if (flag) w.rank[p] = (int32_t)(w.blk[blockIdx.x] + sh[threadIdx.x]);
 }
+__global__ __launch_bounds__(1024) void cc26_rank_kernel(size_t n, FragWs w) { cc26_rank_body(n, w); }
+__global__ __launch_bounds__(1024) void cc26_rank_batch_kernel(const BatchBlock* __restrict__ tab, size_t n) {
+  const BatchBlock& b = tab[blockIdx.y];
+  cc26_rank_body(n, b.frag);
+}
 
 void cc_rank_roots(size_t n, const FragWs& f, uint64_t* num_out, hipStream_t s) {
   const uint32_t nblk = (uint32_t)((n + 1023) / 1024);
@@ -179,11 +226,16 @@
   hipLaunchKernelGGL(cc26_rank_kernel, dim3(nblk), dim3(1024), 0, s, n, f);
 }
 
-__global__ void cc26_write_kernel(const uint64_t* __restrict__ x, size_t n, FragWs w, uint64_t id_offset, uint64_t* __restrict__ out) {
+__device__ __forceinline__ void cc26_write_body(const uint64_t* __restrict__ x, size_t n, const FragWs& w, uint64_t id_offset, uint64_t* __restrict__ out) {
   for (size_t p = (size_t)blockIdx.x * blockDim.x + threadIdx.x; p < n; p += (size_t)gridDim.x * blockDim.x) {
     if (!x[p]) { out[p] = 0; continue; }
     out[p] = id_offset + (uint64_t)w.rank[cc_find(w.par, (int)p)];
   }
+}
+__global__ void cc26_write_kernel(const uint64_t* __restrict__ x, size_t n, FragWs w, uint64_t id_offset, uint64_t* __restrict__ out) { cc26_write_body(x, n, w, id_offset, out); }
+__global__ void cc26_write_batch_kernel(const BatchBlock* __restrict__ tab, size_t n) {
+  const BatchBlock& b = tab[blockIdx.y];
+  cc26_write_body(b.crop_tmp, n, b.frag, b.f.id_offset, b.f.labels);
 }
 
 __global__ void ccaff_init_kernel(size_t n, FragWs w, uint64_t* __restrict__ touched) {
@@ -295,7 +347,7 @@
   }
 }
 
-__global__ void label_stats_kernel(const uint64_t* __restrict__ lab, int D, int H, int W, uint64_t id_offset, uint64_t num,
+__device__ __forceinline__ void label_stats_body(const uint64_t* __restrict__ lab, int D, int H, int W, uint64_t id_offset, uint64_t num,
                                    unsigned long long* __restrict__ size, unsigned long long* __restrict__ sums) {
   const size_t n = (size_t)D * H * W;
   for (size_t p = (size_t)blockIdx.x * blockDim.x + threadIdx.x; p < n; p += (size_t)gridDim.x * blockDim.x) {
@@ -307,6 +359,37 @@
     atomicAdd(&sums[3 * k + 1], (unsigned long long)((p / W) % H));
     atomicAdd(&sums[3 * k + 2], (unsigned long long)(p % W));
   }
+}
+__global__ void label_stats_kernel(const uint64_t* __restrict__ lab, int D, int H, int W, uint64_t id_offset, uint64_t num,
+                                   unsigned long long* __restrict__ size, unsigned long long* __restrict__ sums) { label_stats_body(lab, D, H, W, id_offset, num, size, sums); }
+__global__ void label_stats_batch_kernel(const BatchBlock* __restrict__ tab, int D, int H, int W, uint64_t num) {
+  const BatchBlock& b = tab[blockIdx.y];
+  label_stats_body(b.f.labels, D, H, W, b.f.id_offset, num, (unsigned long long*)b.f.size, (unsigned long long*)b.f.sums);
+}
+
+void batch_post_launch(const BatchBlock* tab, int N, const int64_t shape[3], double filter_value, int64_t min_size, const int64_t crop_offset[3],
+                       const int64_t crop_shape[3], uint64_t stats_num, hipStream_t s) {
+  const size_t n = (size_t)shape[0] * shape[1] * shape[2];
+  const size_t nc = (size_t)crop_shape[0] * crop_shape[1] * crop_shape[2];
+  const int bs = 256;
+  const dim3 grid((unsigned)std::min<size_t>((n + bs - 1) / bs, 4096), N);
+  const dim3 gridc((unsigned)std::min<size_t>((nc + bs - 1) / bs, 4096), N);
+  if (filter_value > 0.0 || min_size > 0) {
+    hipLaunchKernelGGL(frag_stats_batch_kernel, grid, dim3(bs), 0, s, tab, n);
+    hipLaunchKernelGGL(frag_decide_batch_kernel, grid, dim3(bs), 0, s, tab, n, filter_value, (long long)min_size);
+    hipLaunchKernelGGL(frag_filter_batch_kernel, grid, dim3(bs), 0, s, tab, n);
+  }
+  const int cd = (int)crop_shape[0], ch = (int)crop_shape[1], cw = (int)crop_shape[2];
+  hipLaunchKernelGGL(crop_u64_batch_kernel, gridc, dim3(bs), 0, s, tab, (int)shape[1], (int)shape[2], (int)crop_offset[0], (int)crop_offset[1],
+                     (int)crop_offset[2], cd, ch, cw);
+  hipLaunchKernelGGL(cc26_init_batch_kernel, gridc, dim3(bs), 0, s, tab, nc);
+  hipLaunchKernelGGL(cc26_union_batch_kernel, gridc, dim3(bs), 0, s, tab, cd, ch, cw);
+  const uint32_t nblk = (uint32_t)((nc + 1023) / 1024);
+  hipLaunchKernelGGL(cc26_count_batch_kernel, dim3(nblk, N), dim3(1024), 0, s, tab, nc);
+  hipLaunchKernelGGL(cc26_scan_batch_kernel, dim3(1, N), dim3(1024), 0, s, tab, nblk);
+  hipLaunchKernelGGL(cc26_rank_batch_kernel, dim3(nblk, N), dim3(1024), 0, s, tab, nc);
+  hipLaunchKernelGGL(cc26_write_batch_kernel, gridc, dim3(bs), 0, s, tab, nc);
+  hipLaunchKernelGGL(label_stats_batch_kernel, gridc, dim3(bs), 0, s, tab, cd, ch, cw, stats_num);
 }
 
 }
diff --git a/bootstrapper_amd/csrc/seg_ws.hip b/bootstrapper_amd/csrc/seg_ws.hip
--- a/bootstrapper_amd/csrc/seg_ws.hip
+++ b/bootstrapper_amd/csrc/seg_ws.hip
@@ -12,8 +12,8 @@
 constexpr int FLOOD_LDS_HEAP = 1024;
 
 template <bool LDS>
-__global__ __launch_bounds__(WS_T) void ws_seeds_kernel(const uint8_t* __restrict__ affs, int D, int H, int W,
-                                                        int msd, WsScratch s, int compact) {
+__device__ __forceinline__ void ws_seeds_body(const uint8_t* __restrict__ affs, int D, int H, int W, int msd, const WsScratch& s,
+                                              int compact) {
   extern __shared__ __attribute__((aligned(16))) char ws_smem[];
   const int z = blockIdx.x;
   const int n = H * W;
@@ -297,14 +297,28 @@
     else lab[i] = l;
   }
 }
-
-__global__ void ws_offsets_kernel(int D, WsScratch s, uint64_t* max_id) {
+template <bool LDS>
+__global__ __launch_bounds__(WS_T) void ws_seeds_kernel(const uint8_t* __restrict__ affs, int D, int H, int W,
+                                                        int msd, WsScratch s, int compact) {
+  ws_seeds_body<LDS>(affs, D, H, W, msd, s, compact);
+}
+__global__ __launch_bounds__(WS_T) void ws_seeds_batch_kernel(const BatchBlock* __restrict__ tab, int D, int H, int W, int msd, int compact) {
+  const BatchBlock& b = tab[blockIdx.y];
+  ws_seeds_body<true>(b.f.affs, D, H, W, msd, b.ws, compact);
+}
+
+__device__ __forceinline__ void ws_offsets_body(int D, const WsScratch& s, uint64_t* max_id) {
   if (threadIdx.x == 0 && blockIdx.x == 0) {
     uint64_t acc = 0;
     for (int z = 0; z < D; ++z) { s.offs[z] = acc; acc += (uint64_t)s.nseeds[z]; }
     *max_id = acc;
   }
 }
+__global__ void ws_offsets_kernel(int D, WsScratch s, uint64_t* max_id) { ws_offsets_body(D, s, max_id); }
+__global__ void ws_offsets_batch_kernel(const BatchBlock* __restrict__ tab, int D) {
+  const BatchBlock& b = tab[blockIdx.y];
+  ws_offsets_body(D, b.ws, b.f.max_id);
+}
 
 __device__ __forceinline__ uint64_t bcast0(uint64_t v) {
   const uint32_t lo = __builtin_amdgcn_readfirstlane((uint32_t)v), hi = __builtin_amdgcn_readfirstlane((uint32_t)(v >> 32));
@@ -314,8 +328,8 @@
 __device__ __forceinline__ bool flood_smaller(uint64_t a, uint64_t b) { return (int64_t)((a >> 20) - (b >> 20)) < 0; }
 
 template <bool COMPACT>
-__global__ __launch_bounds__(64 * FLOOD_WAVES) void ws_flood_kernel(int D, int H, int W, WsScratch s, uint64_t* heap_spill,
-                                                     size_t spill_stride, uint64_t* __restrict__ frags, int* status) {
+__device__ __forceinline__ void ws_flood_body(int D, int H, int W, const WsScratch& s, uint64_t* heap_spill, size_t spill_stride,
+                                              uint64_t* __restrict__ frags, int* status) {
   __shared__ uint64_t hl_all[FLOOD_WAVES][FLOOD_LDS_HEAP];
   const int lane = threadIdx.x & 63;
   const int wave = __builtin_amdgcn_readfirstlane(threadIdx.x >> 6);
@@ -501,6 +515,15 @@
     out[i] = l ? (uint64_t)l + off : 0ull;
   }
   (void)status;
+}
+template <bool COMPACT>
+__global__ __launch_bounds__(64 * FLOOD_WAVES) void ws_flood_kernel(int D, int H, int W, WsScratch s, uint64_t* heap_spill,
+                                                     size_t spill_stride, uint64_t* __restrict__ frags, int* status) {
+  ws_flood_body<COMPACT>(D, H, W, s, heap_spill, spill_stride, frags, status);
+}
+__global__ __launch_bounds__(64 * FLOOD_WAVES) void ws_flood_batch_kernel(const BatchBlock* __restrict__ tab, int D, int H, int W) {
+  const BatchBlock& b = tab[blockIdx.y];
+  ws_flood_body<true>(D, H, W, b.ws, b.flood_spill, b.flood_spill_stride, b.f.frags, b.status);
 }
 
 constexpr int FLOOD_WIDE_LDS_LEVELS = 13;
@@ -715,6 +738,41 @@
 
 using namespace bsmi;
 
+static size_t ws_seeds_lds_bytes(int H, int W) {
+  const size_t hw16 = ((size_t)H * W + 15) & ~(size_t)15;
+  return (((size_t)H * (W + 2) * 2 + 15) & ~(size_t)15) + (((size_t)H * W * 2 + 15) & ~(size_t)15) + 2 * hw16;
+}
+static bool ws_seeds_use_lds(int H, int W) {
+  return ws_seeds_lds_bytes(H, W) <= 158 * 1024 && (size_t)H * H + (size_t)W * W < 65535 && (H + 1) * (H + 1) + W * W < 65535;
+}
+static bool flood_compact_ok() {
+  static const bool ok = [] { const char* e = getenv("BSMI_FLOOD_COMPACT"); return !(e && e[0] == '0'); }();
+  return ok;
+}
+
+namespace bsmi {
+
+size_t batch_ws_lds_bytes(int H, int W) {
+  return ws_seeds_use_lds(H, W) && flood_compact_ok() && (size_t)H * W < ((size_t)1 << 20) ? ws_seeds_lds_bytes(H, W) : 0;
+}
+
+int batch_ws_launch(const BatchBlock* tab, int N, int D, int H, int W, int msd, hipStream_t s) {
+  const size_t lds = batch_ws_lds_bytes(H, W);
+  if (!lds) BSMI_FAIL(BSMI_ERR_INVALID, "slices of %d x %d are off the LDS / compact path: not served in batches", H, W);
+  static DeviceOnce once;
+  const int rc_once = once.run([&]() -> int {
+    BSMI_HIP(hipFuncSetAttribute((const void*)ws_seeds_batch_kernel, hipFuncAttributeMaxDynamicSharedMemorySize, 158 * 1024));
+    return BSMI_OK;
+  });
+  if (rc_once) return rc_once;
+  hipLaunchKernelGGL(ws_seeds_batch_kernel, dim3(D, N), dim3(WS_T), lds, s, tab, D, H, W, msd, 1);
+  hipLaunchKernelGGL(ws_offsets_batch_kernel, dim3(1, N), dim3(64), 0, s, tab, D);
+  hipLaunchKernelGGL(ws_flood_batch_kernel, dim3((D + FLOOD_WAVES - 1) / FLOOD_WAVES, N), dim3(64 * FLOOD_WAVES), 0, s, tab, D, H, W);
+  return BSMI_OK;
+}
+
+}
+
 static int fragments_xy(bsmi_seg* h, const uint8_t* affs_dev, int D, int H, int W, int min_seed_distance, uint64_t* frags_dev,
                         uint64_t* max_id_dev, uint64_t* seeds_dev, hipStream_t s) {
   if ((size_t)H * W >= ((size_t)1 << 20) && (H > 4096 || W > 4096))
@@ -732,11 +790,9 @@
     wsx.seedlab = h->seedlab;
   }
   {
-    const size_t hw16 = ((size_t)H * W + 15) & ~(size_t)15;
-    const size_t lds = (((size_t)H * (W + 2) * 2 + 15) & ~(size_t)15) + (((size_t)H * W * 2 + 15) & ~(size_t)15) + 2 * hw16;
-    const bool use_lds = lds <= 158 * 1024 && (size_t)H * H + (size_t)W * W < 65535 && (H + 1) * (H + 1) + W * W < 65535;
-    static const bool compact_ok = [] { const char* e = getenv("BSMI_FLOOD_COMPACT"); return !(e && e[0] == '0'); }();
-    compact = use_lds && compact_ok;
+    const size_t lds = ws_seeds_lds_bytes(H, W);
+    const bool use_lds = ws_seeds_use_lds(H, W);
+    compact = use_lds && flood_compact_ok();
     if (use_lds) {
       static DeviceOnce once;
       const int rc_once = once.run([&]() -> int {
diff --git a/bootstrapper_amd/post/engine.py b/bootstrapper_amd/post/engine.py
--- a/bootstrapper_amd/post/engine.py
+++ b/bootstrapper_amd/post/engine.py
@@ -200,6 +200,66 @@
         check(lib.bsmi_seg_status(self._h, self._stream()))
 
 
+class SegBatch:
+
+    def __init__(self, engines):
+        self.engines = list(engines)
+        self.device = self.engines[0].device
+        self._h = C.c_void_p()
+        hs = (C.c_void_p * len(self.engines))(*[e._h.value for e in self.engines])
+        check(lib.bsmi_seg_batch_create(hs, len(self.engines), C.byref(self._h)))
+
+    def __del__(self):
+        h = getattr(self, "_h", None)
+        if h:
+            lib.bsmi_seg_batch_destroy(h)
+            self._h = None
+
+    def __len__(self):
+        return len(self.engines)
+
+    def _stream(self):
+        return C.c_void_p(torch.cuda.current_stream(torch.device("cuda", self.device)).cuda_stream)
+
+    def fragments(self, affs, frags, labels, nums, id_offsets, sizes, sums, min_seed_distance=10, filter_value=0.0, min_size=0,
+                  crop_offset=(0, 0, 0), max_ids=None):
+        n = len(affs)
+        shape, crop = tuple(frags[0].shape), tuple(labels[0].shape)
+        cap = int(sizes[0].numel())
+        if max_ids is None:
+            max_ids = torch.empty(n, dtype=torch.int64, device=affs[0].device)
+        args = (_lib.BatchFragArgs * n)()
+        for i in range(n):
+            _affs3(affs[i], contiguous=True)
+            _frags_like(frags[i], affs[i], contiguous=True)
+            if tuple(frags[i].shape) != shape or tuple(labels[i].shape) != crop or labels[i].dtype != torch.int64 or not labels[i].is_contiguous():
+                raise ValueError("the blocks of a batch share one shape and one crop shape (contiguous int64 labels)")
+            if (sizes[i].dtype != torch.int64 or sums[i].dtype != torch.int64 or sizes[i].numel() != cap or sums[i].numel() != 3 * cap
+                    or nums[i].dtype != torch.int64 or not (sizes[i].is_contiguous() and sums[i].is_contiguous())):
+                raise ValueError("sizes int64 [cap], sums int64 [cap][3] (contiguous, one capacity), nums int64 [1]")
+            args[i] = _lib.BatchFragArgs(affs[i].data_ptr(), frags[i].data_ptr(), max_ids[i:i + 1].data_ptr(), labels[i].data_ptr(),
+                                         nums[i].data_ptr(), int(id_offsets[i]), sizes[i].data_ptr(), sums[i].data_ptr())
+        check(lib.bsmi_seg_batch_fragments_u8(self._h, n, args, _lib.i64x3(shape), 1, int(min_seed_distance), float(filter_value),
+                                              int(min_size), _lib.i64x3(crop_offset), _lib.i64x3(crop), cap, self._stream()))
+        return max_ids
+
+    def rag_graph(self, affs, frags, edges, sums, pair_counts, counts):
+        n = len(affs)
+        shape = tuple(frags[0].shape)
+        args = (_lib.BatchGraphArgs * n)()
+        for i in range(n):
+            _affs3(affs[i], contiguous=True)
+            _frags_like(frags[i], affs[i], contiguous=True)
+            e, s, c, k = edges[i], sums[i], pair_counts[i], counts[i]
+            if (tuple(frags[i].shape) != shape or e.dtype != torch.int64 or s.dtype != torch.int64 or c.dtype != torch.int32 or k.dtype != torch.int64
+                    or not (e.is_contiguous() and s.is_contiguous() and c.is_contiguous() and k.is_contiguous())
+                    or not e.shape[0] == s.shape[0] == c.shape[0] or k.numel() < 3):
+                raise ValueError("one shape; edges int64 [cap][2], sums int64 [cap], pair_counts int32 [cap], counts int64 [>= 3]: contiguous, one capacity")
+            args[i] = _lib.BatchGraphArgs(affs[i].data_ptr(), frags[i].data_ptr(), e.data_ptr(), s.data_ptr(), c.data_ptr(), k.data_ptr(),
+                                          int(e.shape[0]))
+        check(lib.bsmi_seg_batch_rag_graph_u8(self._h, n, args, _lib.i64x3(shape), self._stream()))
+
+
 QUEUE_BINS_FORMULAS = {"n_minus_1": 0, "n": 1}
 
 
diff --git a/bootstrapper_amd/volume.py b/bootstrapper_amd/volume.py
--- a/bootstrapper_amd/volume.py
+++ b/bootstrapper_amd/volume.py
@@ -193,6 +193,17 @@
                                    lab=torch.empty(tuple(min(b, s) for b, s in zip(self.block, self.shape)), dtype=torch.int64,
                                                    device=self.dev)))
         torch.cuda.current_stream(self.dev).synchronize()
+        self._batchers = []
+        self._lane_events = []
+        if (os.environ.get("BSMI_SEG_BATCH", "1") != "0" and self.host_scores and self.fragments_in_xy and self.epsilon == 0
+                and all(v is None for v in self.shift.values())):
+            from .post.engine import SegBatch
+            S = max(1, min(int(os.environ.get("BSMI_SEG_BATCH_STREAMS", "1")), len(self.lanes)))
+            for g in range(S):
+                mine = self.lanes[g::S][:32]
+                self._batchers.append(dict(batch=SegBatch([lane["engine"] for lane in mine]), lanes=mine, stream=mine[0]["stream"],
+                                           max_ids=torch.zeros(len(mine), dtype=torch.int64, device=self.dev)))
+            torch.cuda.current_stream(self.dev).synchronize()
         self.nodes = None
         self.rag_edges = self.rag_scores = None
         self.luts = None
@@ -332,6 +343,74 @@
                 lane["engine"].rag_graph_async(a, f, self.edges[k], self.esums[k], self.scores[k].view(torch.int32), self.counts_dev[k])
             else:
                 lane["engine"].rag_merge_scores_async(a, f, 1.0, self.bins, self.edges[k], self.scores[k], self.counts_dev[k])
+
+    def _batch_stage(self, kind, ks, wait=()):
+        groups = {}
+        for k in ks:
+            groups.setdefault(tuple(sl.stop - sl.start for sl in self._read_slices(k)), []).append(k)
+        pending, self._lane_events = list(wait) + self._lane_events, []
+        waited = set()
+        refused, turn = [], 0
+        for rshape, group in groups.items():
+            wshape = tuple(r - 2 * c for r, c in zip(rshape, self.ctx))
+            i = 0
+            while i < len(group):
+                bt = self._batchers[turn % len(self._batchers)]
+                chunk = group[i:i + len(bt["lanes"])]
+                st = bt["stream"]
+                with torch.cuda.stream(st):
+                    if id(bt) not in waited:
+                        waited.add(id(bt))
+                        for ev in pending:
+                            st.wait_event(ev)
+                    A, F, L = [], [], []
+                    for lane, k in zip(bt["lanes"], chunk):
+                        a = self._buf(lane["a"], rshape, (3,))
+                        a.copy_(self.affs[(slice(None),) + self._read_slices(k)])
+                        f = self._buf(lane["f"], rshape)
+                        if kind == "s":
+                            f.copy_(self.frags[self._read_slices(k)])
+                        A.append(a)
+                        F.append(f)
+                        L.append(self._buf(lane["lab"], wshape))
+                    try:
+                        if kind == "f":
+                            bt["batch"].fragments(A, F, L, [self.nums[k:k + 1] for k in chunk], [self.block_ids[k] * self.nvb for k in chunk],
+                                                  [self.sizes[k] for k in chunk], [self.sums[k] for k in chunk], self.msd, self.filter_fragments,
+                                                  self.remove_debris, self.ctx, max_ids=bt["max_ids"])
+                        else:
+                            bt["batch"].rag_graph(A, F, [self.edges[k] for k in chunk], [self.esums[k] for k in chunk],
+                                                  [self.scores[k].view(torch.int32) for k in chunk], [self.counts_dev[k] for k in chunk])
+                    except _lib.BsmiError as exc:
+                        if exc.code != _lib.ERR_INVALID:
+                            raise
+                        refused.extend(group[i:])
+                        break
+                    if kind == "f":
+                        for k, lab in zip(chunk, L):
+                            b, e = self.boxes[k]
+                            self.frags[tuple(slice(c + lo, c + hi) for c, lo, hi in zip(self.ctx, b, e))].copy_(lab)
+                        done = torch.cuda.Event()
+                        done.record(st)
+                        for k in chunk:
+                            self.frag_done[k] = done
+                i += len(chunk)
+                turn += 1
+        return refused
+
+    def _lanes_stage(self, kind, ks, wait=()):
+        if not ks:
+            return
+        tails = []
+        for bt in self._batchers:
+            ev = torch.cuda.Event()
+            ev.record(bt["stream"])
+            tails.append(ev)
+        for k in ks:
+            (self._launch_fragments if kind == "f" else self._launch_scores)(k, list(wait) + tails)
+            ev = torch.cuda.Event()
+            ev.record(self.lane_of(kind, k)["stream"])
+            self._lane_events.append(ev)
 
     def _collect(self):
         err = self._sync()
@@ -419,7 +498,28 @@
         nb = [self._neighbours(k) for k in range(K)]
         queued, scored = set(), set()
 
+        batched = bool(self._batchers) and not overlap
+        self._lane_events = []
+
+        def fragments_of(ks, wait):
+            if batched:
+                self._lanes_stage("f", self._batch_stage("f", ks, wait), wait)
+            else:
+                for k in ks:
+                    self._launch_fragments(k, wait)
+            queued.update(ks)
+
         def score_what_can_be(candidates, extra=()):
+            if batched:
+                todo = [j for j in candidates if j not in scored and all(i in queued for i in nb[j])]
+                seen, wait = set(), list(extra)
+                for i in sorted(queued):
+                    if id(self.frag_done[i]) not in seen:
+                        seen.add(id(self.frag_done[i]))
+                        wait.append(self.frag_done[i])
+                self._lanes_stage("s", self._batch_stage("s", todo, wait), wait)
+                scored.update(todo)
+                return
             for j in candidates:
                 if j not in scored and all(i in queued for i in nb[j]):
                     self._launch_scores(j, list(extra) + [self.frag_done[i] for i in nb[j]])
@@ -439,9 +539,7 @@
                 err = exc
 
         def launch_inner():
-            for k in inner:
-                self._launch_fragments(k, (ready[K - 1],))
-                queued.add(k)
+            fragments_of(inner, (ready[K - 1],))
         def launch_overlapped():
             import time
             todo_f = list(inner)
@@ -473,11 +571,13 @@
             got = self._exchange(self.affs)
 
             def launch_face():
+                if not overlap:
+                    fragments_of(face, (got,))
+                    return
                 for k in face:
                     self._launch_fragments(k, (got,))
                     queued.add(k)
-                    if overlap:
-                        score_what_can_be([j for j in nb[k] if j in inner_set])
+                    score_what_can_be([j for j in nb[k] if j in inner_set])
             guarded(launch_face)
         guarded(lambda: score_what_can_be(inner))
         if face:
@@ -617,6 +717,18 @@
             self._lane_load = [0] * len(self.lanes)
             for lane in self.lanes:
                 lane["stream"].synchronize()
+            if self._batchers:
+                groups = {}
+                for k in range(len(self.boxes)):
+                    groups.setdefault(tuple(sl.stop - sl.start for sl in self._read_slices(k)), []).append(k)
+                ks = [k for g in groups.values() for k in g[:len(self.lanes)]]
+                self._lane_events = []
+                self._lanes_stage("f", self._batch_stage("f", ks))
+                wait = [ev for ev in {id(self.frag_done[k]): self.frag_done[k] for k in ks}.values()]
+                self._lanes_stage("s", self._batch_stage("s", ks, wait), wait)
+                self._lane_events = []
+                for lane in self.lanes:
+                    lane["stream"].synchronize()
 
     def run(self, ready=None, overlap=False):
         if ready is not None and not overlap:
diff --git a/include/bsmi.h b/include/bsmi.h
--- a/include/bsmi.h
+++ b/include/bsmi.h
@@ -248,6 +248,34 @@
 
 int bsmi_seg_status(bsmi_seg *h, void *stream);
 
+typedef struct bsmi_seg_batch bsmi_seg_batch;
+typedef struct {
+  const uint8_t *affs_dev;
+  uint64_t *frags_dev;
+  uint64_t *max_id_dev;
+  uint64_t *labels_dev;
+  uint64_t *num_labels_dev;
+  uint64_t id_offset;
+  uint64_t *size_dev;
+  uint64_t *sums_dev;
+} bsmi_batch_frag_args;
+typedef struct {
+  const uint8_t *affs_dev;
+  const uint64_t *frags_dev;
+  uint64_t *edges_dev;
+  uint64_t *sums_dev;
+  uint32_t *pair_counts_dev;
+  uint64_t *counts_dev;
+  uint64_t edge_capacity;
+} bsmi_batch_graph_args;
+int bsmi_seg_batch_create(bsmi_seg *const *handles, int n, bsmi_seg_batch **out);
+int bsmi_seg_batch_destroy(bsmi_seg_batch *b);
+int bsmi_seg_batch_fragments_u8(bsmi_seg_batch *b, int n_blocks, const bsmi_batch_frag_args *args, const int64_t shape[3],
+                                int fragments_in_xy, int min_seed_distance, double filter_value, int64_t min_size,
+                                const int64_t crop_offset[3], const int64_t crop_shape[3], uint64_t stats_num, void *stream);
+int bsmi_seg_batch_rag_graph_u8(bsmi_seg_batch *b, int n_blocks, const bsmi_batch_graph_args *args, const int64_t shape[3],
+                                void *stream);
+
 typedef struct bsmi_eval bsmi_eval;
 int bsmi_eval_create(int device, uint64_t pair_capacity, bsmi_eval **out);
 int bsmi_eval_destroy(bsmi_eval *h);
```

Result: faster. 105.7, median of 6 (+8.2%).
